# dimforge/wgsparkl

Measured on AMD Instinct MI355X. Metric: particle-steps/sec, higher is better.
Workload: dtype f32; 1 GPU; wgsparkl3d neo-Hookean elastic cube, 1000000 particles, 128^3-cell domain, h=1, dt=1/1200, 8 particles/cell, floor cuboid (CPIC passes on), free fall; config=c2, particles_per_gpu=1000000, global_particles=1000000, active_blocks_rank0=2700, parallelism=1 GPU

## Files before the change

wgsparkl_amd/csrc/capi_debug.inc:

```

extern "C" {

wgs_status wgs_enqueue_diagnostics(wgs_data *d, uint32_t what, wgs_diagnostics *device_out) {
    WGS_TRY(enter(d, device_out != nullptr));
    return diag_enqueue(d, what, device_out);
}

wgs_status wgs_read_diagnostics(wgs_data *d, uint32_t what, wgs_diagnostics *out) {
    WGS_TRY(enter(d, out != nullptr));
    if (!d->diag_out) WGS_TRY(dev_alloc(d, &d->diag_out, 1));
    if (!d->diag_host) WGS_TRY(d->diag_host.alloc(1));
    WGS_TRY(diag_enqueue(d, what, d->diag_out));
    WGS_TRY(download(d, d->diag_host.get(), d->diag_out, sizeof(wgs_diagnostics)));
    memcpy(out, d->diag_host.get(), sizeof(wgs_diagnostics));
    return WGS_OK;
}

wgs_status wgs_debug_scan(wgs_pipeline *pipeline, const uint32_t *values, uint32_t n, uint32_t *out, uint32_t *total) {
    if (!pipeline || (!values && n) || (!out && n)) return fail(WGS_ERR_INVALID_ARGUMENT, "NULL argument");
    if (n > (1u << 25)) return fail(WGS_ERR_INVALID_ARGUMENT, "n out of range");
    HIP_TRY(hipSetDevice(pipeline->device));
    Dev dev{};
    dev.cap = std::max(1u, n);
    const uint32_t nscan = (dev.cap + SCAN_CHUNK - 1) / SCAN_CHUNK, epoch = 1u;
    Scratch<uint32_t> counters, stamp, acc, active, start;
    Scratch<unsigned long long> chunk_a, chunk_b, group_a, group_b;
    const size_t ngroup = (size_t)nscan * SORT_THREADS;
    if (counters.alloc(CTR_COUNT, true) != WGS_OK || stamp.alloc(dev.cap, true) != WGS_OK || acc.alloc(dev.cap, true) != WGS_OK ||
        active.alloc(dev.cap, true) != WGS_OK || start.alloc(dev.cap, true) != WGS_OK || chunk_a.alloc(nscan, true) != WGS_OK ||
        chunk_b.alloc(nscan, true) != WGS_OK || group_a.alloc(ngroup, true) != WGS_OK || group_b.alloc(ngroup, true) != WGS_OK)
        return fail(WGS_ERR_HIP, "out of device memory");
    dev.counters = counters.ptr; dev.block_stamp = stamp.ptr; dev.block_acc = acc.ptr; dev.active = active.ptr; dev.block_start = start.ptr;
    dev.chunk_a = chunk_a.ptr; dev.chunk_b = chunk_b.ptr; dev.group_a = group_a.ptr; dev.group_b = group_b.ptr;
    std::vector<uint32_t> ones(dev.cap, epoch);
    uint32_t ctr[CTR_COUNT] = {0};
    ctr[CTR_NPHYS] = n;
    hipError_t e = hipMemcpy(dev.counters, ctr, sizeof(ctr), hipMemcpyHostToDevice);
    if (e == hipSuccess) e = hipMemcpy(dev.block_stamp, ones.data(), sizeof(uint32_t) * dev.cap, hipMemcpyHostToDevice);
    if (e == hipSuccess && n) e = hipMemcpy(dev.block_acc, values, sizeof(uint32_t) * n, hipMemcpyHostToDevice);
    if (e == hipSuccess) {
        hipLaunchKernelGGL(k_scan_only, dim3(nscan + std::min((n + 3u) / 4u + 1u, 2048u)), dim3(SORT_THREADS), 0, 0, dev, epoch, nscan);
        e = hipDeviceSynchronize();
    }
    if (e == hipSuccess && n) e = hipMemcpy(out, dev.block_start, sizeof(uint32_t) * n, hipMemcpyDeviceToHost);
    if (e == hipSuccess && total) {
        unsigned long long t = 0;
        std::vector<unsigned long long> ct(nscan);
        e = hipMemcpy(ct.data(), dev.chunk_b, sizeof(unsigned long long) * nscan, hipMemcpyDeviceToHost);
        for (auto v : ct) t += v & 0xffffffffull;
        *total = (uint32_t)t;
    }
    if (e != hipSuccess) return fail(WGS_ERR_HIP, hipGetErrorString(e));
    return WGS_OK;
}

#ifdef WGS_ABLATE
static wgs_status read_and_reset_prof(const void *symbol, unsigned long long *out, size_t rows) {
    const std::vector<unsigned long long> zero(rows * 8, 0ull);
    HIP_TRY(hipDeviceSynchronize());
    HIP_TRY(hipMemcpyFromSymbol(out, symbol, sizeof(unsigned long long) * zero.size()));
    HIP_TRY(hipMemcpyToSymbol(symbol, zero.data(), sizeof(unsigned long long) * zero.size()));
    return WGS_OK;
}
wgs_status wgs_debug_g2p_prof(unsigned long long *out) { return read_and_reset_prof(HIP_SYMBOL(g_g2p_prof), out, WGS_G2P_ROWS); }
wgs_status wgs_debug_p2g_prof(unsigned long long *out) { return read_and_reset_prof(HIP_SYMBOL(g_p2g_prof), out, WGS_P2G_ROWS); }
wgs_status wgs_debug_prof(unsigned long long *out) { return read_and_reset_prof(HIP_SYMBOL(g_prof), out, WGS_PROF_ROWS); }
#endif

}
```

wgsparkl_amd/csrc/host_grid.inc:

```

namespace {

wgs_status alloc_grid(wgs_data *d, bool missing_only = false) {
    Dev &dev = d->dev;
    const size_t hcap = (size_t)dev.hmask + 1, cap = dev.cap, nchunk = (cap + SCAN_CHUNK - 1) / SCAN_CHUNK;
    auto grid_array = [&](auto **ptr, size_t count) {
        return missing_only && *ptr ? WGS_OK : dev_alloc(d, ptr, count, MemGroup::grid);
    };
    WGS_TRY(grid_array(&dev.hkeys, hcap));
    WGS_TRY(grid_array(&dev.hvals, hcap));
    WGS_TRY(grid_array(&dev.block_key, cap));
    if (!(dev.dbg & DBG_NO_EVICTION)) {
        WGS_TRY(grid_array(&dev.block_slot, cap));
        WGS_TRY(grid_array(&dev.free_ids, cap));
    }
    WGS_TRY(grid_array(&dev.block_count, cap));
    WGS_TRY(grid_array(&dev.block_stamp, cap));
    WGS_TRY(grid_array(&dev.links_epoch, cap));
    WGS_TRY(grid_array(&dev.block_acc, cap));
    WGS_TRY(grid_array(&dev.block_dirty, cap));
    WGS_TRY(grid_array(&dev.blk_narr, cap));
    WGS_TRY(grid_array(&dev.block_ident, cap));
    WGS_TRY(grid_array(&dev.blk_arr, cap * BLK_ARR));
    WGS_TRY(grid_array(&dev.active, cap));
    WGS_TRY(grid_array(&dev.block_start, cap));
    WGS_TRY(grid_array(&dev.act_info, cap));
    WGS_TRY(grid_array(&dev.act_cells, cap * NPB));
    WGS_TRY(grid_array(&dev.nbr_plus, cap * 8));
    WGS_TRY(grid_array(&dev.nbr_minus, cap * 8));
    WGS_TRY(grid_array(&dev.nbr_known, cap * 16));
    WGS_TRY(grid_array(&dev.act_src, cap * 8));
    WGS_TRY(grid_array(&dev.cell_head, cap * NPB));
    WGS_TRY(grid_array(&dev.chunk_a, nchunk));
    WGS_TRY(grid_array(&dev.chunk_b, nchunk));
    WGS_TRY(grid_array(&dev.group_a, nchunk * SORT_THREADS));
    WGS_TRY(grid_array(&dev.group_b, nchunk * SORT_THREADS));
    WGS_TRY(grid_array(&dev.cell_start, cap * NPB));
    WGS_TRY(grid_array(&dev.cell_cursor, cap * NPB));
    WGS_TRY(grid_array(&dev.nodes, cap * NPB));
    WGS_TRY(grid_array(&dev.node_cdf, cap * NPB));
    WGS_TRY(grid_array(&dev.slab, cap * Dim<D>::TILE));
    WGS_TRY(grid_array(&dev.slab_epoch, cap));
    WGS_TRY(grid_array(&dev.block_cdf_gen, cap));
    WGS_TRY(grid_array(&dev.block_cpic, cap));
    WGS_TRY(grid_array(&dev.block_cdf_summ, cap));
    WGS_TRY(grid_array(&dev.pcdf_done, cap));
    WGS_TRY(grid_array(&dev.cpic_list, cap * 8));
    dev.visit_cap = dev.npad / 512u + 2u * dev.cap + 16u;
    WGS_TRY(grid_array(&dev.visit_list, (size_t)dev.visit_cap * 8));
    if (dev.sharded) WGS_TRY(grid_array(&dev.halo_list, cap * HALO_ENT));
    if (d->two_way) WGS_TRY(grid_array(&dev.imp_slab, cap * Dim<D>::TILE * (D == 3 ? 2 : 1)));
    if (d->mesh_cdf) {
        WGS_TRY(grid_array(&dev.mesh_min, cap * NPB));
        WGS_TRY(grid_array(&dev.mesh_aff, cap * NPB));
    }
    return WGS_OK;
}

wgs_status enable_impulses(wgs_data *d) {
    if (d->two_way) return WGS_OK;
    d->two_way = true;
    const wgs_status st = alloc_grid(d, true);
    if (st != WGS_OK) d->two_way = false;
    return st;
}

wgs_status clear_table(wgs_data *d, bool ids_too) {
    const Dev &dev = d->dev;
    HIP_TRY(hipMemsetAsync(dev.hkeys, 0xff, sizeof(uint32_t) * ((size_t)dev.hmask + 1), d->stream));
    HIP_TRY(hipMemsetAsync(dev.hvals, 0xff, sizeof(uint32_t) * ((size_t)dev.hmask + 1), d->stream));
    if (!ids_too) return WGS_OK;
    HIP_TRY(hipMemsetAsync(dev.counters + CTR_NPHYS, 0, sizeof(uint32_t), d->stream));
    HIP_TRY(hipMemsetAsync(dev.counters + CTR_NFREE, 0, 3 * sizeof(uint32_t), d->stream));
    return WGS_OK;
}

wgs_status grow_grid(wgs_data *d, uint32_t new_cap) {
    Dev &dev = d->dev;
    HIP_TRY(hipStreamSynchronize(d->stream));
    const Dev old = dev;
    d->mem.regroup(MemGroup::grid, MemGroup::old_grid);
    dev.cap = new_cap;
    dev.hmask = new_cap * 2u - 1u;
    if (alloc_grid(d) != WGS_OK) {
        d->mem.release_group(MemGroup::grid);
        d->mem.regroup(MemGroup::old_grid, MemGroup::grid);
        dev = old;
        d->auto_grow = false;
        hipGetLastError();
        return WGS_OK;
    }
    d->mem.release_group(MemGroup::old_grid);
    WGS_TRY(clear_table(d, true));
    d->sub.prev_sorted = false;
    d->sub.prebinned = false;
    d->cdf_generation++;
    d->seen.ncpic = UINT32_MAX;
    d->seen.nvisit = UINT32_MAX;
    d->stats.grid_grown++;
    return WGS_OK;
}

wgs_status maintain_grid(wgs_data *d) {
    if (!d->seen.watch || !d->seen.watch_pending) return WGS_OK;
    if (hipEventQuery(d->seen.watch_event) != hipSuccess) {
        if (++d->seen.watch_skips < 2u) return WGS_OK;
        HIP_TRY(hipEventSynchronize(d->seen.watch_event));
    }
    d->seen.watch_skips = 0;
    d->seen.watch_pending = false;
    const uint32_t nblocks = d->seen.watch[CTR_NBLOCKS], nphys = d->seen.watch[CTR_NPHYS], cap = d->dev.cap;
    if (d->dev.sharded) d->seen.nv_hint = std::max(d->seen.watch[CTR_NV], d->seen.watch[CTR_NV + CTR_SET]);
    const uint32_t rate = nblocks > d->seen.nblocks && d->seen.nblocks != 0u ? nblocks - d->seen.nblocks : 0u;
    d->seen.nblocks = std::min(nblocks, cap);
    const uint64_t ahead = (uint64_t)nblocks + 3ull * rate;
    if (d->auto_grow && (nblocks > cap / 2u || ahead > cap / 4u * 3u) && cap < (1u << 24)) {
        uint32_t new_cap = cap * 2u;
        while (ahead > new_cap / 4u * 3u && new_cap < (1u << 24)) new_cap *= 2u;
        return grow_grid(d, new_cap);
    }
    if (nphys > cap / 4u * 3u) d->seen.force_rehash = true;
    if (d->seen.watch[CTR_NTOMB] > cap / 2u) d->seen.force_refresh = true;
    return WGS_OK;
}

wgs_status watch_counters(wgs_data *d) {
    if (!d->seen.watch) {
        Pinned<uint32_t> watch;
        Event copied;
        WGS_TRY(watch.alloc(CTR_COUNT));
        WGS_TRY(copied.create(hipEventDisableTiming));
        d->seen.watch = std::move(watch);
        d->seen.watch_event = std::move(copied);
    }
    HIP_TRY(hipMemcpyAsync(d->seen.watch.get(), d->dev.counters, sizeof(uint32_t) * CTR_COUNT, hipMemcpyDeviceToHost, d->stream));
    HIP_TRY(hipEventRecord(d->seen.watch_event, d->stream));
    d->seen.watch_pending = true;
    return WGS_OK;
}

wgs_status fetch_counters(wgs_data *d) {
    uint32_t host[CTR_COUNT];
    HIP_TRY(hipMemcpyAsync(host, d->dev.counters, sizeof(host), hipMemcpyDeviceToHost, d->stream));
    HIP_TRY(hipStreamSynchronize(d->stream));
    d->seen.sync_nblocks = host[CTR_NBLOCKS] < d->dev.cap ? host[CTR_NBLOCKS] : d->dev.cap;
    d->seen.nblocks = d->seen.sync_nblocks;
    const uint32_t last_epoch = (uint32_t)d->substeps;
    d->seen.ncpic = 0;
    for (uint32_t k = 0; k < 8; k++) d->seen.ncpic += std::min(host[ctr_ncpic(k, last_epoch)], d->dev.cap);
    d->seen.ncpic = std::min(d->seen.ncpic, d->dev.cap);
    d->seen.nvisit = 0;
    for (uint32_t k = 0; k < 8; k++) d->seen.nvisit = std::max(d->seen.nvisit, std::min(host[ctr_nvisit(k, last_epoch)], d->dev.visit_cap));
    uint32_t movers = 0u;
    for (int k = 0; k < 16; k++) movers += host[CTR_MOVERS + 32 * k];
    d->stats.movers_total += (uint32_t)(movers - d->seen.movers);
    d->seen.movers = movers;
    d->seen.nphys = host[CTR_NPHYS];
    d->seen.nfree = host[CTR_NFREE];
    d->seen.ntomb = host[CTR_NTOMB];
    d->seen.errors |= host[CTR_ERRORS];
    if (host[CTR_NBLOCKS] > d->dev.cap) d->seen.errors |= ERRBIT_OVERFLOW;
    if (host[CTR_NPHYS] > d->dev.cap / 4u * 3u) d->seen.force_rehash = true;
    if (host[CTR_NTOMB] > d->dev.cap / 2u) d->seen.force_refresh = true;
    return WGS_OK;
}

wgs_status sticky_status(wgs_data *d) {
    if (d->seen.errors & ERRBIT_OVERFLOW)
        return fail(WGS_ERR_GRID_OVERFLOW, "sparse grid overflow: more active blocks than grid_capacity");
    if (d->seen.errors & ERRBIT_SHARD)
        return fail(WGS_ERR_INVALID_ARGUMENT, "sharded run: a message buffer or the particle capacity overflowed, a particle left the decomposition, or the ranks disagree on the uniform-material mode");
    if (d->seen.errors & ERRBIT_KEYRANGE)
        return fail(WGS_ERR_KEY_RANGE, "a particle left the packed block-key range (grid.wgsl:88-95)");
    if (d->seen.errors & ERRBIT_HANDOVER)
        return fail(WGS_ERR_HIP, "internal: a grid-update wave gave up waiting for a block's P2G slab (the sort's block totals and cell runs disagree)");
    if (d->seen.errors & ERRBIT_PCDF)
        return fail(WGS_ERR_HIP, "internal: a near-collider workgroup of P2G gave up waiting for the prologue waves of its launch and computed the particle cdf itself (results intact; the launch lost 0.2 s)");
    if (d->seen.errors & ERRBIT_MATERIAL)
        return fail(WGS_ERR_INVALID_ARGUMENT, "wgs_set_uniform_material: a particle of this wgs_data carries other constants (mass, init_volume, lambda, mu)");
    return WGS_OK;
}

void resolve_timings(wgs_data *d) {
    if (!d->timing.pending) return;
    hipStreamSynchronize(d->stream);
    for (int p = 0; p < WGS_NUM_PASSES; p++) d->timing.ms[p] = 0.f;
    const int pass_of_mark[8] = {WGS_PASS_GRID_SORT,   WGS_PASS_GRID_UPDATE_CDF, WGS_PASS_G2P_CDF,          WGS_PASS_P2G,
                                 WGS_PASS_GRID_UPDATE, WGS_PASS_G2P,             WGS_PASS_PARTICLES_UPDATE, WGS_PASS_INTEGRATE_BODIES};
    d->timing.mark_overhead_ms = 0.f;
    for (int s = 0; s < d->timing.events.used; s++) {
        float ms = 0.f;
        if (hipEventElapsedTime(&ms, d->timing.events.ev[s][9], d->timing.events.ev[s][10]) == hipSuccess) d->timing.mark_overhead_ms += ms;
    }
    if (d->timing.events.used > 0) d->timing.mark_overhead_ms /= (float)d->timing.events.used;
    for (int s = 0; s < d->timing.events.used; s++)
        for (int m = 0; m < 8; m++) {
            if (m == 6 && !d->cpic) continue;
            float ms = 0.f;
            if (hipEventElapsedTime(&ms, d->timing.events.ev[s][m], d->timing.events.ev[s][m + 1]) == hipSuccess)
                d->timing.ms[pass_of_mark[m]] += ms;
        }
    d->timing.pending = false;
}

}
```

wgsparkl_amd/csrc/host_state.h:

```cpp
#pragma once

namespace {

constexpr int D = WGS_DIM;
constexpr int DD = D * D;
using P = Pl<D>;

#define WGS_STR2(x) #x
#define WGS_STR(x) WGS_STR2(x)

thread_local std::string g_last_error;

wgs_status fail(wgs_status code, const std::string &msg) {
    g_last_error = msg;
    return code;
}

#define HIP_TRY(expr)                                                                                   \
    do {                                                                                                \
        hipError_t _e = (expr);                                                                         \
        if (_e != hipSuccess)                                                                           \
            return fail(WGS_ERR_HIP, std::string(#expr) + ": " + hipGetErrorString(_e));                \
    } while (0)
#define WGS_TRY(expr)                          \
// ... 79 lines not shown
        for (int k = 0; k < count; k++) hipEventDestroy(*(&ev[0][0] + k));
        created = false;
    }
};

class DataStream {
    hipStream_t s = nullptr;
    bool owned = false;

public:
    DataStream() = default;
    DataStream(const DataStream &) = delete;
    DataStream &operator=(const DataStream &) = delete;
    ~DataStream() {
        if (s && owned) hipStreamDestroy(s);
    }
    wgs_status create() {
        if (hipStreamCreateWithFlags(&s, hipStreamNonBlocking) != hipSuccess) return fail(WGS_ERR_HIP, "hipStreamCreate failed");
        owned = true;
        return WGS_OK;
    }
    wgs_status borrow(hipStream_t callers) {
        if (s && owned) HIP_TRY(hipStreamDestroy(s));
        s = callers;
        owned = false;
        return WGS_OK;
    }
    hipStream_t exchange(hipStream_t other) { return std::exchange(s, other); }
    operator hipStream_t() const { return s; }
};

enum class MemGroup : uint8_t { fixed, grid, old_grid, rigid, models };
class DeviceMemory {
    struct Block { void *ptr; size_t bytes; MemGroup group; };
    std::vector<Block> blocks;
    uint64_t total = 0;

public:
    wgs_status alloc(void **out, size_t bytes, MemGroup group, hipStream_t zero_on, bool zero) {
        void *p = nullptr;
        HIP_TRY(hipMalloc(&p, bytes));
        blocks.push_back({p, bytes, group});
        total += bytes;
        *out = p;
        if (zero) HIP_TRY(hipMemsetAsync(p, 0, bytes, zero_on));
        return WGS_OK;
    }
    void release(void *p) {
        if (!p) return;
        for (size_t i = 0; i < blocks.size(); i++)
            if (blocks[i].ptr == p) {
                total -= blocks[i].bytes;
                blocks.erase(blocks.begin() + (long)i);
                break;
            }
        hipFree(p);
    }
    void release_group(MemGroup group) {
        for (size_t i = blocks.size(); i-- > 0;)
            if (blocks[i].group == group) release(blocks[i].ptr);
    }
    void release_all() {
        while (!blocks.empty()) release(blocks.back().ptr);
    }
    void regroup(MemGroup from, MemGroup to) {
        for (Block &b : blocks) b.group = b.group == from ? to : b.group;
    }
    uint64_t bytes() const { return total; }
};

template <typename T> struct Scratch {
    T *ptr = nullptr;
    Scratch() = default;
    Scratch(const Scratch &) = delete;
    Scratch &operator=(const Scratch &) = delete;
    ~Scratch() { hipFree(ptr); }
    wgs_status alloc(size_t count, bool zeroed = false) {
        HIP_TRY(hipMalloc((void **)&ptr, sizeof(T) * (count ? count : 1)));
        if (zeroed) HIP_TRY(hipMemset(ptr, 0, sizeof(T) * (count ? count : 1)));
        return WGS_OK;
    }
};

}

namespace { struct DiagAcc; }

struct wgs_pipeline {
    int device = 0;
    int num_cus = 256;
    hipDeviceProp_t props;
};

struct wgs_comm {
    void *comm = nullptr;
    int rank = 0, world = 1;
    int lower = -1, upper = -1;
    int device = 0;
};
struct ShardLink {
    bool attached = false;
    wgs_comm *comm = nullptr;
    bool has_lower = false, has_upper = false;
    uint32_t halo_cap = 0, mig_cap = 0;
    size_t msg_floats = 0;
    float *msg_out[2] = {nullptr, nullptr}, *msg_in[2] = {nullptr, nullptr};
};

struct wgs_data {
    wgs_pipeline *pipeline = nullptr;
    DataStream stream;
    Dev dev{};
    int side = 0;
    bool plastic = false;
    bool cpic = false;
    uint64_t substeps = 0;
    uint32_t capacity = 0;
    uint32_t *shard_counts = nullptr;
    float *static_radius = nullptr;
    float *static_dp = nullptr;
    float *static_phase = nullptr;
    uint32_t *static_flags = nullptr;
    SimParamsDev *sp = nullptr;
    ColliderDev *colliders = nullptr;
    std::vector<ColliderDev> host_colliders;
    std::vector<BodyDev> host_bodies;
    bool bodies_move = false;
    uint32_t moving_mask = 0;
    bool two_way = false;
    bool mesh_cdf = false;
    SimParamsDev host_sp{};
    bool auto_grow = true;
    uint32_t cdf_generation = 1;
    uint32_t rehash_period = REHASH_PERIOD;
    ShardLink *link = nullptr;
    int reduce_impulses = 0;
    int32_t **lockstep_imp_ptrs = nullptr;
    uint32_t lockstep_imp_n = 0;
    DiagAcc *diag_acc = nullptr;
    wgs_diagnostics *diag_out = nullptr;
    Pinned<wgs_diagnostics> diag_host;
    uint32_t *probe_mark = nullptr;
    uint32_t probe_mark_cap = 0, probe_ticket = 0;

    DeviceMemory mem;

    struct Seen {
        Pinned<uint32_t> watch;
        Event watch_event;
        bool watch_pending = false;
        uint32_t watch_skips = 0;
        uint32_t errors = 0;
        uint32_t nblocks = 0;
        uint32_t sync_nblocks = 0;
        uint32_t nv_hint = 0;
        uint32_t ncpic = UINT32_MAX;
        uint32_t nvisit = UINT32_MAX;
        uint32_t movers = 0;
        uint32_t nphys = 0, nfree = 0, ntomb = 0;
        bool force_rehash = false;
        bool force_refresh = false;
    } seen;

    struct Substep {
        bool prev_sorted = false;
        bool needs_compact = false;
        bool prebinned = false;
        bool bodies_pending = false;
        bool in_sharded_step = false;
        int ts_slot = -1;
        uint32_t epoch = 0;
        bool rehash = false;
        bool use_rebin = false;
        bool binned = false;
        bool fused_cdf = false;
        bool gu_fused = false;
        bool shard_fused = false;
        bool arrivals = false;
    } sub;

    struct Stats {
        uint64_t movers_total = 0;
        uint64_t table_rebuilds = 0;
        uint64_t table_refreshes = 0;
        uint32_t grid_grown = 0;
    } stats;

    struct Timing {
        Events events;
        float ms[WGS_NUM_PASSES] = {0};
        float mark_overhead_ms = 0.f;
        bool pending = false;
    } timing;
};

namespace {

template <typename T> wgs_status dev_alloc(wgs_data *d, T **out, size_t count, MemGroup group = MemGroup::fixed, bool zero = true) {
    return d->mem.alloc(reinterpret_cast<void **>(out), sizeof(T) * (count ? count : 1), group, d->stream, zero);
}

wgs_status download(wgs_data *d, void *dst, const void *src, size_t bytes) {
    HIP_TRY(hipMemcpyAsync(dst, src, bytes, hipMemcpyDeviceToHost, d->stream));
    HIP_TRY(hipStreamSynchronize(d->stream));
    return WGS_OK;
}

wgs_status enter(wgs_data *d, bool args_ok = true, const char *what = "NULL argument") {
    if (!d || !args_ok) return fail(WGS_ERR_INVALID_ARGUMENT, what);
    HIP_TRY(hipSetDevice(d->pipeline->device));
    return WGS_OK;
}

int grid_for(const wgs_data *d, int blocks_per_cu) { return d->pipeline->num_cus * blocks_per_cu; }

}
```

wgsparkl_amd/csrc/host_substep.inc:

```

namespace {

wgs_status allreduce_impulses(wgs_data *d);
void launch_bodies_integrate(wgs_data *d);

#ifndef WGS_PCDF_WAVES_MAX_VISITS
#define WGS_PCDF_WAVES_MAX_VISITS 256
#endif
constexpr uint32_t PCDF_WAVES_MAX_VISITS = WGS_PCDF_WAVES_MAX_VISITS;
constexpr uint32_t P2G_SMALL_BUDGET_MIN_PARTICLES = 600000;
#ifndef WGS_REGROUP_ROUNDS
#define WGS_REGROUP_ROUNDS 4u
#endif
#ifndef WGS_GU_WG_PER_CU
#define WGS_GU_WG_PER_CU 8
#endif
#ifndef WGS_PLASTIC_WPE_DENSE
#define WGS_PLASTIC_WPE_DENSE 2
#endif
#ifndef WGS_PLASTIC_WPE
#define WGS_PLASTIC_WPE G2P_WAVES_PER_EU
#endif
constexpr uint32_t P2G_PAIR_MIN_BLOCKS = 8;


struct PackWaves {
    uint32_t blocks, guests;
};
PackWaves pack_waves(const wgs_data *d) {
    return {std::max(64u, std::min(2048u, d->seen.nblocks ? d->seen.nblocks : 2048u)), std::max(1u, std::min(64u, (2u * d->link->mig_cap + 63u) / 64u))};
}

template <int DIM> void launch_regroup(const Dev &dev, hipStream_t s, dim3 g, int side, uint32_t epoch, uint32_t nscan, int have_old, bool cdf, bool summ) {
    const dim3 b(SORT_THREADS);
    if (cdf && dev.sharded && summ) hipLaunchKernelGGL((k_regroup<DIM, true, true, true>), g, b, 0, s, dev, side, epoch, nscan, have_old);
    else if (cdf && dev.sharded) hipLaunchKernelGGL((k_regroup<DIM, true, true>), g, b, 0, s, dev, side, epoch, nscan, have_old);
    else if (cdf && summ) hipLaunchKernelGGL((k_regroup<DIM, true, false, true>), g, b, 0, s, dev, side, epoch, nscan, have_old);
    else if (cdf) hipLaunchKernelGGL((k_regroup<DIM, true, false>), g, b, 0, s, dev, side, epoch, nscan, have_old);
    else if (dev.sharded) hipLaunchKernelGGL((k_regroup<DIM, false, true>), g, b, 0, s, dev, side, epoch, nscan, have_old);
    else hipLaunchKernelGGL((k_regroup<DIM, false, false>), g, b, 0, s, dev, side, epoch, nscan, have_old);
}

enum class P2gShape {
    plain,
    separate,
    cpic_first,
    pair,
};
struct P2gLaunch {
    P2gShape shape;
    bool two_way;
    bool small_budget;
    int gu;
    uint32_t wgs;
    uint32_t ride;
    uint32_t npack, npack_blk, layer_sel;
    uint32_t npro;
};

template <int DIM, bool TW, int WPE> void launch_p2g_pair(Dev &dev, hipStream_t s, int side, uint32_t epoch, const P2gLaunch &p) {
    const dim3 g(p.npro + 2u * p.wgs + p.ride), b(P2GCfg<DIM>::NW * 64);
    dev.pcdf_waves = p.npro;
    if (p.gu == 2) hipLaunchKernelGGL((k_p2g_pair<DIM, TW, WPE, 2>), g, b, 0, s, dev, side, epoch, p.wgs, p.npack, p.npack_blk, p.layer_sel, p.npro);
    else if (p.gu == 3) hipLaunchKernelGGL((k_p2g_pair<DIM, TW, WPE, 3>), g, b, 0, s, dev, side, epoch, p.wgs, p.npack, p.npack_blk, p.layer_sel, p.npro);
    else hipLaunchKernelGGL((k_p2g_pair<DIM, TW, WPE, 0>), g, b, 0, s, dev, side, epoch, p.wgs, p.npack, p.npack_blk, p.layer_sel, p.npro);
    dev.pcdf_waves = 0u;
}

template <int DIM, bool CP, bool TW, bool PC> void launch_p2g_last(Dev &dev, hipStream_t s, int side, int filter, uint32_t epoch, const P2gLaunch &p) {
    const uint32_t npro = PC ? p.npro : 0u;
    const dim3 g(npro + p.wgs + p.ride), b(P2GCfg<DIM>::NW * 64);
    dev.pcdf_waves = npro;
    if (p.gu == 2) hipLaunchKernelGGL((k_p2g<DIM, CP, TW, PC, 2>), g, b, 0, s, dev, side, filter, epoch, p.wgs, p.npack, p.npack_blk, p.layer_sel, npro);
    else if (p.gu == 3) hipLaunchKernelGGL((k_p2g<DIM, CP, TW, PC, 3>), g, b, 0, s, dev, side, filter, epoch, p.wgs, p.npack, p.npack_blk, p.layer_sel, npro);
    else hipLaunchKernelGGL((k_p2g<DIM, CP, TW, PC, 0>), g, b, 0, s, dev, side, filter, epoch, p.wgs, p.npack, p.npack_blk, p.layer_sel, npro);
    dev.pcdf_waves = 0u;
}

template <int DIM> void launch_p2g(Dev &dev, hipStream_t s, int side, uint32_t epoch, const P2gLaunch &p) {
    const dim3 g(p.wgs), b(P2GCfg<DIM>::NW * 64);
    switch (p.shape) {
        case P2gShape::pair:
            if (p.two_way) launch_p2g_pair<DIM, true, 1>(dev, s, side, epoch, p);
            else if (p.small_budget) launch_p2g_pair<DIM, false, 3>(dev, s, side, epoch, p);
            else launch_p2g_pair<DIM, false, 1>(dev, s, side, epoch, p);
            break;
        case P2gShape::cpic_first:
            dev.pcdf_waves = p.npro;
            hipLaunchKernelGGL((k_p2g<DIM, true, true, true, 1>), dim3(p.npro + p.wgs), b, 0, s, dev, side, 2, epoch, p.wgs, 0u, 0u, p.layer_sel, p.npro);
            dev.pcdf_waves = 0u;
            hipLaunchKernelGGL((k_p2g<DIM, false, false, false, 2, true>), dim3(p.wgs + p.ride), b, 0, s, dev, side, 1, epoch, p.wgs, p.npack, p.npack_blk, p.layer_sel, 0u);
            break;
        case P2gShape::separate:
            if (p.gu != 0) hipLaunchKernelGGL((k_p2g<DIM, false, false, false, 1>), g, b, 0, s, dev, side, 1, epoch, p.wgs, 0u, 0u, p.layer_sel, 0u);
            else hipLaunchKernelGGL((k_p2g<DIM, false>), g, b, 0, s, dev, side, 1, epoch, p.wgs, 0u, 0u, p.layer_sel, 0u);
            if (p.two_way) launch_p2g_last<DIM, true, true, true>(dev, s, side, 2, epoch, p);
            else launch_p2g_last<DIM, true, false, true>(dev, s, side, 2, epoch, p);
            break;
        case P2gShape::plain:
            launch_p2g_last<DIM, false, false, false>(dev, s, side, 0, epoch, p);
            break;
    }
}

template <int DIM> void launch_grid_update(const Dev &dev, hipStream_t s, dim3 g, uint32_t epoch, bool slab, bool two_way, uint32_t iface_only) {
    if (!slab && two_way) hipLaunchKernelGGL((k_grid_update<DIM, 0, true>), g, dim3(256), 0, s, dev, epoch, 0u);
    else if (!slab) hipLaunchKernelGGL((k_grid_update<DIM, 0>), g, dim3(256), 0, s, dev, epoch, 0u);
    else if (two_way) hipLaunchKernelGGL((k_grid_update<DIM, 3, true>), g, dim3(256), 0, s, dev, epoch, iface_only);
    else hipLaunchKernelGGL((k_grid_update<DIM, 3>), g, dim3(256), 0, s, dev, epoch, iface_only);
}

enum class G2pShape {
    single,
    two_launches,
    pair,
    pair_dense,
};
struct G2pLaunch {
    G2pShape shape;
    bool shard;
    uint32_t g;
    uint32_t nlist;
};

template <int DIM, int MODEL, bool PL, int NP, class Mark>
void launch_g2p_shape(const Dev &dev, hipStream_t s, int side, uint32_t epoch, const G2pLaunch &p, const Mark &mark) {
    constexpr int WPE = PL ? WGS_PLASTIC_WPE : G2P_WAVES_PER_EU, WPE_DENSE = PL ? WGS_PLASTIC_WPE_DENSE : G2P_WAVES_PER_EU;
    constexpr bool SH = MODEL != 3;
    const dim3 g(p.g), pg(p.g + 8u * p.nlist), t(G2P_THREADS);
    switch (p.shape) {
        case G2pShape::pair_dense:
            if (p.shard) hipLaunchKernelGGL((k_g2p_pair<DIM, MODEL, PL, WPE_DENSE, NP, SH, !PL>), pg, t, 0, s, dev, side, epoch, p.g, p.nlist);
            else hipLaunchKernelGGL((k_g2p_pair<DIM, MODEL, PL, WPE_DENSE, NP, false, !PL>), pg, t, 0, s, dev, side, epoch, p.g, p.nlist);
            break;
        case G2pShape::pair:
            if (p.shard) hipLaunchKernelGGL((k_g2p_pair<DIM, MODEL, PL, WPE, NP, SH, !PL>), pg, t, 0, s, dev, side, epoch, p.g, p.nlist);
            else hipLaunchKernelGGL((k_g2p_pair<DIM, MODEL, PL, WPE, NP, false, !PL>), pg, t, 0, s, dev, side, epoch, p.g, p.nlist);
            break;
        case G2pShape::two_launches:
            hipLaunchKernelGGL((k_g2p_update<DIM, MODEL, PL, 1, NP, false, !PL>), g, t, 0, s, dev, side, epoch);
            mark(6);
            hipLaunchKernelGGL((k_g2p_update<DIM, MODEL, PL, 2, 1, false, !PL>), dim3(8u * p.nlist), t, 0, s, dev, side, epoch);
            break;
        case G2pShape::single:
            if (p.shard) hipLaunchKernelGGL((k_g2p_update<DIM, MODEL, PL, 0, NP, SH, !PL>), g, t, 0, s, dev, side, epoch);
            else hipLaunchKernelGGL((k_g2p_update<DIM, MODEL, PL, 0, NP, false, !PL>), g, t, 0, s, dev, side, epoch);
            break;
    }
}

template <int DIM, int MODEL, bool PL, class Mark>
void launch_g2p_model(const Dev &dev, hipStream_t s, int side, uint32_t epoch, const G2pLaunch &p, const Mark &mark) {
    if (dev.g2p_npass == (uint32_t)G2P_MANY_PASSES) launch_g2p_shape<DIM, MODEL, PL, G2P_MANY_PASSES>(dev, s, side, epoch, p, mark);
    else if (dev.g2p_npass == 2u) launch_g2p_shape<DIM, MODEL, PL, 2>(dev, s, side, epoch, p, mark);
    else launch_g2p_shape<DIM, MODEL, PL, 1>(dev, s, side, epoch, p, mark);
}

enum class G2pVariant { corotated, corotated_plastic, neo_hookean, neo_hookean_plastic, fluid, per_particle };
G2pVariant g2p_variant(const Dev &dev, bool plastic) {
    if (dev.pmodel[0]) return G2pVariant::per_particle;
    if (dev.model == WGS_MODEL_FLUID) return G2pVariant::fluid;
    if (dev.model == WGS_MODEL_NEO_HOOKEAN) return plastic ? G2pVariant::neo_hookean_plastic : G2pVariant::neo_hookean;
    return plastic ? G2pVariant::corotated_plastic : G2pVariant::corotated;
}

template <int DIM, class Mark> void launch_g2p(const Dev &dev, hipStream_t s, int side, uint32_t epoch, bool plastic, const G2pLaunch &p, const Mark &mark) {
    switch (g2p_variant(dev, plastic)) {
        case G2pVariant::corotated: launch_g2p_model<DIM, 0, false>(dev, s, side, epoch, p, mark); break;
        case G2pVariant::corotated_plastic: launch_g2p_model<DIM, 0, true>(dev, s, side, epoch, p, mark); break;
        case G2pVariant::neo_hookean: launch_g2p_model<DIM, 1, false>(dev, s, side, epoch, p, mark); break;
        case G2pVariant::neo_hookean_plastic: launch_g2p_model<DIM, 1, true>(dev, s, side, epoch, p, mark); break;
        case G2pVariant::fluid: launch_g2p_model<DIM, 2, false>(dev, s, side, epoch, p, mark); break;
        case G2pVariant::per_particle: launch_g2p_model<DIM, 3, false>(dev, s, side, epoch, p, mark); break;
    }
}

template <int DIM> void launch_arrivals(const Dev &dev, hipStream_t s, dim3 g, int side, uint32_t epoch, bool plastic) {
    switch (g2p_variant(dev, plastic)) {
        case G2pVariant::corotated: hipLaunchKernelGGL((k_g2p_arrivals<DIM, 0, false>), g, dim3(256), 0, s, dev, side, epoch); break;
        case G2pVariant::corotated_plastic: hipLaunchKernelGGL((k_g2p_arrivals<DIM, 0, true>), g, dim3(256), 0, s, dev, side, epoch); break;
        case G2pVariant::neo_hookean: hipLaunchKernelGGL((k_g2p_arrivals<DIM, 1, false>), g, dim3(256), 0, s, dev, side, epoch); break;
        case G2pVariant::neo_hookean_plastic: hipLaunchKernelGGL((k_g2p_arrivals<DIM, 1, true>), g, dim3(256), 0, s, dev, side, epoch); break;
        default: hipLaunchKernelGGL((k_g2p_arrivals<DIM, 2, false>), g, dim3(256), 0, s, dev, side, epoch); break;
    }
}


enum class SortBin { full, rebin, by_last_g2p };
struct SortLaunch {
    bool refresh, reset_table;
    SortBin bin;
    uint32_t do_bodies;
    uint32_t nscan, nreg;
    int have_old;
    bool cdf, summ;
    uint32_t refresh_wgs, mesh_wgs, p2g_cdf_wgs;
};
SortLaunch plan_sort(const wgs_data *d) {
    const Dev &dev = d->dev;
    SortLaunch p{};
    p.refresh = d->seen.force_refresh && !d->sub.rehash && dev.free_ids != nullptr;
    p.refresh_wgs = std::max(1u, std::min((dev.cap + 255u) / 256u, (uint32_t)grid_for(d, 4)));
    p.reset_table = d->sub.rehash;
    p.bin = d->sub.binned ? SortBin::by_last_g2p : d->sub.use_rebin ? SortBin::rebin : SortBin::full;
    p.do_bodies = d->sub.bodies_pending ? 1u : 0u;
    p.mesh_wgs = (uint32_t)grid_for(d, 1);
    p.nscan = (dev.cap + SCAN_CHUNK - 1) / SCAN_CHUNK;
    p.nreg = std::max(1u, std::min((dev.cap + 3u) / 4u, WGS_REGROUP_ROUNDS * ((uint32_t)grid_for(d, 4) - std::min(p.nscan, (uint32_t)grid_for(d, 2)))));
    p.have_old = d->sub.use_rebin ? 1 : 0;
    p.cdf = d->sub.fused_cdf;
    p.summ = (dev.cdf_moving != 0u || dev.cdf_gen == 0u) && !(dev.dbg & DBG_NO_CDF_SUMM);
    p.p2g_cdf_wgs = std::min((dev.n_rigid * 32u + 255u) / 256u, (uint32_t)grid_for(d, 32));
    return p;
}

enum class P2gLayers { all, boundary, others };

P2gLaunch plan_p2g(const wgs_data *d, P2gLayers layers) {
    const Dev &dev = d->dev;
    const uint32_t n = dev.n;
    const uint32_t NW = (uint32_t)P2GCfg<D>::NW;
    P2gLaunch p{};
    p.two_way = d->two_way;
    p.layer_sel = layers == P2gLayers::boundary ? 1u : layers == P2gLayers::others ? 2u : 0u;
    p.wgs = std::min((uint32_t)grid_for(d, 32), std::max((uint32_t)grid_for(d, 8), (d->seen.nblocks / 2u + 255u) & ~255u));
    p.gu = d->sub.gu_fused ? 2 : d->sub.shard_fused ? 3 : 0;
    const uint32_t gu_wgs = (p.gu == 0 || layers == P2gLayers::boundary) ? 0u : std::min((uint32_t)grid_for(d, 8), std::max((uint32_t)grid_for(d, 1), ((d->seen.nblocks + NW - 1u) / NW + 7u) & ~7u));
    if (d->sub.shard_fused && (d->link->has_lower || d->link->has_upper) && layers != P2gLayers::others) {
        const PackWaves pw = pack_waves(d);
        p.npack_blk = pw.blocks;
        p.npack = (pw.blocks + pw.guests + NW - 1u) / NW;
    }
    p.ride = p.npack + gu_wgs;
    if (d->cpic && !dev.sharded && d->seen.nvisit != UINT32_MAX && d->seen.nvisit != 0u && d->seen.nvisit <= PCDF_WAVES_MAX_VISITS && !(dev.dbg & DBG_NO_PCDF_WAVES))
        p.npro = 8u * ((std::min(d->seen.nvisit + 8u, dev.visit_cap) + NW - 1u) / NW);
    if (d->cpic && !dev.sharded && (dev.dbg & DBG_PCDF_WAVES_UNSIZED)) p.npro = 8u;
    if (!d->cpic) {
        p.shape = P2gShape::plain;
        return p;
    }
    p.small_budget = !d->two_way && n >= P2G_SMALL_BUDGET_MIN_PARTICLES && !(dev.dbg & DBG_NO_P2G_SMALL_BUDGET);
    const bool big_two_way = d->two_way && n >= P2G_SMALL_BUDGET_MIN_PARTICLES;
    const bool small_two_way = d->two_way && n < P2G_SMALL_BUDGET_MIN_PARTICLES;
    const bool many_listed = d->seen.ncpic != UINT32_MAX && d->seen.ncpic >= P2G_PAIR_MIN_BLOCKS;
    if (!big_two_way && (p.small_budget || small_two_way || many_listed) && !(dev.dbg & DBG_P2G_TWO_LAUNCHES))
        p.shape = P2gShape::pair;
    else if (big_two_way && p.gu == 2 && !(dev.dbg & DBG_PLAIN_P2G_FIRST))
        p.shape = P2gShape::cpic_first;
    else
        p.shape = P2gShape::separate;
    return p;
}

G2pLaunch plan_g2p(const wgs_data *d) {
    const Dev &dev = d->dev;
    const uint32_t npass = dev.g2p_npass;
    const uint32_t full = (uint32_t)grid_for(d, 1) * 3u / 2u;
    G2pLaunch p{G2pShape::single, dev.sharded != 0u, ((dev.nv + G2P_THREADS * npass - 1) / (G2P_THREADS * npass) + 7) / 8 * 8, full};
    if (d->cpic && (p.shard || !(dev.dbg & DBG_G2P_TWO_LAUNCHES))) {
        const uint32_t per_run = std::min<uint32_t>(npass, WGS_G2P_LIST_PASSES);
        if (d->seen.nvisit != UINT32_MAX) p.nlist = std::min(full, std::max(8u, 2u * ((d->seen.nvisit + per_run - 1u) / per_run)));
        const bool dense = d->plastic && d->seen.ncpic != UINT32_MAX && d->seen.ncpic * 2u >= std::max(1u, d->seen.sync_nblocks) && !(dev.dbg & DBG_NO_G2P_DENSE);
        p.shape = dense ? G2pShape::pair_dense : G2pShape::pair;
    } else if (d->cpic) {
        p.shape = G2pShape::two_launches;
    }
    return p;
}


struct Mark {
    wgs_data *d;
    void operator()(int m) const {
        static const bool trace = getenv("WGS_TRACE") != nullptr;
        if (d->sub.ts_slot >= 0) hipEventRecord(d->timing.events.ev[d->sub.ts_slot][m], d->stream);
        if (trace) {
            const hipError_t te = hipStreamSynchronize(d->stream);
            fprintf(stderr, "[wgs trace] substep %llu mark %d: %s\n", (unsigned long long)d->substeps, m, hipGetErrorString(te));
        }
    }
};

void catch_up_counters(wgs_data *d) {
    d->dev.ctr_set = (uint32_t)(d->substeps & 1u);
    if (!d->sub.needs_compact) return;
    hipLaunchKernelGGL(k_shard_compacted, dim3(1), dim3(64), 0, d->stream, d->dev);
    d->sub.needs_compact = false;
}

wgs_status begin_substep(wgs_data *d, bool in_sharded_step, int ts_slot = -1) {
    Dev &dev = d->dev;
    wgs_data::Substep &sub = d->sub;
    hipStream_t s = d->stream;
    sub.in_sharded_step = in_sharded_step;
    sub.ts_slot = ts_slot;
    sub.epoch = (uint32_t)(d->substeps + 1);
    const uint32_t nv_now = dev.sharded && d->seen.nv_hint != 0u ? std::min(d->seen.nv_hint, dev.nv) : dev.nv;
    dev.g2p_npass = (D == 3 && nv_now >= G2P_MANY_PASS_MIN_PARTICLES) ? (uint32_t)G2P_MANY_PASSES
                    : (nv_now >= G2P_TWO_PASS_MIN_PARTICLES || (dev.dbg & DBG_G2P_TWO_PASSES)) ? 2u : 1u;
    sub.rehash = d->substeps == 0 || (d->rehash_period != 0u && d->substeps % d->rehash_period == 0) || d->seen.force_rehash;
    if (sub.rehash) {
        d->stats.table_rebuilds++;
        d->seen.force_rehash = false;
        d->cdf_generation++;
    }
    dev.cdf_gen = d->cpic ? d->cdf_generation : 0u;
    dev.cdf_moving = d->moving_mask;
    sub.fused_cdf = d->cpic && dev.n_rigid == 0;
    dev.listed_in_perm = sub.fused_cdf ? 1u : 0u;
    sub.use_rebin = sub.prev_sorted && !sub.rehash && !(dev.dbg & DBG_NO_REBIN);
    sub.binned = sub.use_rebin && sub.prebinned;
    if (sub.prebinned && !sub.binned) {
        HIP_TRY(hipMemsetAsync(dev.block_acc, 0, sizeof(uint32_t) * (size_t)dev.cap, s));
        HIP_TRY(hipMemsetAsync(dev.cell_head, 0, sizeof(uint32_t) * (size_t)dev.cap * NPB, s));
        HIP_TRY(hipMemsetAsync(dev.blk_narr, 0, sizeof(uint32_t) * (size_t)dev.cap, s));
    }
    sub.prebinned = false;
    dev.bin_next = (!d->plastic && !(dev.dbg & (DBG_NO_REBIN | DBG_REBIN_LAUNCH)) && (d->rehash_period == 0u || (d->substeps + 1) % d->rehash_period != 0)) ? 1u : 0u;
    dev.skip_guests = (in_sharded_step && dev.sharded) ? 1u : 0u;
    sub.gu_fused = !in_sharded_step && !dev.sharded && !(dev.dbg & DBG_GU_OWN_LAUNCH);
    const bool attached = in_sharded_step && d->link && d->link->attached;
    sub.shard_fused = attached && dev.n > 0 && !(dev.dbg & DBG_GU_OWN_LAUNCH);
    sub.arrivals = attached;
    catch_up_counters(d);
    return WGS_OK;
}

template <int DIM> wgs_status enqueue_sort(wgs_data *d) {
    Dev &dev = d->dev;
    hipStream_t s = d->stream;
    const Mark mark{d};
    const int side = d->side;
    const uint32_t n = dev.n, epoch = d->sub.epoch;
    const int pgrid = (int)((n + SORT_THREADS - 1) / SORT_THREADS);
    const SortLaunch p = plan_sort(d);
    if (d->sub.ts_slot >= 0) {
        mark(9);
        mark(10);
    }
    mark(0);
    if (p.refresh) {
        WGS_TRY(clear_table(d, false));
        hipLaunchKernelGGL(k_table_refresh, dim3(p.refresh_wgs), dim3(256), 0, s, dev);
        d->stats.table_refreshes++;
    }
    d->seen.force_refresh = false;
    if (p.reset_table) WGS_TRY(clear_table(d, true));
    if (dev.n_rigid > 0)
        hipLaunchKernelGGL(k_rigid_transform<DIM>, dim3(p.mesh_wgs), dim3(256), 0, s, dev);
    if (n > 0) {
        d->sub.bodies_pending = false;
        switch (p.bin) {
            case SortBin::by_last_g2p: if (p.do_bodies) launch_bodies_integrate(d); break;
            case SortBin::rebin: hipLaunchKernelGGL(k_rebin<DIM>, dim3((pgrid + REBIN_K - 1) / REBIN_K), dim3(SORT_THREADS), 0, s, dev, side, epoch, p.do_bodies); break;
            case SortBin::full: hipLaunchKernelGGL(k_bin<DIM>, dim3(pgrid), dim3(SORT_THREADS), 0, s, dev, side, epoch, p.do_bodies); break;
        }
        if (dev.n_rigid > 0) {
            hipLaunchKernelGGL(k_rigid_mark<DIM>, dim3(p.mesh_wgs), dim3(256), 0, s, dev, epoch);
            hipLaunchKernelGGL(k_rigid_touch<DIM>, dim3(p.mesh_wgs), dim3(256), 0, s, dev, epoch);
        }
        launch_regroup<DIM>(dev, s, dim3(p.nscan + p.nreg), side, epoch, p.nscan, p.have_old, p.cdf, p.summ);
    } else {
        HIP_TRY(hipMemsetAsync(dev.counters + CTR_NBLOCKS, 0, sizeof(uint32_t), s));
    }
    mark(1);
    if (dev.n_rigid > 0 && n > 0)
        hipLaunchKernelGGL(k_p2g_cdf<DIM>, dim3(p.p2g_cdf_wgs), dim3(256), 0, s, dev, epoch);
    if (d->cpic && n > 0 && !p.cdf)
        hipLaunchKernelGGL(k_cdf<DIM>, dim3(grid_for(d, 16)), dim3(CDF_THREADS), 0, s, dev, side, epoch);
    mark(2);
    mark(3);
    HIP_TRY(hipGetLastError());
    return WGS_OK;
}

template <int DIM> wgs_status enqueue_p2g(wgs_data *d, P2gLayers layers) {
    if (d->dev.n > 0) launch_p2g<DIM>(d->dev, d->stream, d->side, d->sub.epoch, plan_p2g(d, layers));
    Mark{d}(4);
    HIP_TRY(hipGetLastError());
    return WGS_OK;
}

template <int DIM> wgs_status enqueue_finish(wgs_data *d) {
    Dev &dev = d->dev;
    const wgs_data::Substep &sub = d->sub;
    hipStream_t s = d->stream;
    const Mark mark{d};
    const int side = d->side;
    const uint32_t n = dev.n, epoch = sub.epoch;
    if (n > 0 && !sub.gu_fused)
        launch_grid_update<DIM>(dev, s, dim3(grid_for(d, WGS_GU_WG_PER_CU)), epoch, sub.in_sharded_step, d->two_way, sub.shard_fused ? 1u : 0u);
    mark(5);
    const G2pLaunch g2p = plan_g2p(d);
    if (dev.nv > 0) launch_g2p<DIM>(dev, s, side, epoch, d->plastic, g2p, mark);
    if (!(dev.nv > 0 && g2p.shape == G2pShape::two_launches)) mark(6);
    if (sub.arrivals) {
        const uint32_t arr_most = ((d->link->has_lower ? 1u : 0u) + (d->link->has_upper ? 1u : 0u)) * d->link->mig_cap;
        launch_arrivals<DIM>(dev, s, dim3(std::max(1u, std::min((arr_most + ARR_PER_WG - 1u) / ARR_PER_WG, 1024u))), side, epoch, d->plastic);
    }
    mark(7);
    if (d->bodies_move && dev.n_colliders > 0 && !(sub.in_sharded_step && d->reduce_impulses == 2)) {
        if (sub.in_sharded_step && d->reduce_impulses == 1) WGS_TRY(allreduce_impulses(d));
        if (!sub.in_sharded_step && !dev.sharded && dev.n_rigid == 0 && n > 0 && !(dev.dbg & DBG_BODIES_OWN_LAUNCH) && !dev.bin_next) d->sub.bodies_pending = true;
        else launch_bodies_integrate(d);
    }
    mark(8);
    d->side ^= 1;
    d->substeps++;
    d->sub.prev_sorted = true;
    d->sub.prebinned = dev.bin_next != 0u && dev.nv > 0;
    dev.n = dev.nv;
    if (dev.sharded && !sub.arrivals) d->sub.needs_compact = true;
    HIP_TRY(hipGetLastError());
    return WGS_OK;
}

void launch_bodies_integrate(wgs_data *d) { hipLaunchKernelGGL(k_bodies_integrate<D>, dim3(1), dim3(16), 0, d->stream, d->dev); }

wgs_status enqueue_bodies(wgs_data *d) {
    if (d->bodies_move && d->dev.n_colliders > 0) launch_bodies_integrate(d);
    HIP_TRY(hipGetLastError());
    return WGS_OK;
}

}
```

wgsparkl_amd/csrc/kernels_sort.h:

```cpp
#pragma once
#include "kernels_shard.h"

namespace wgs {

constexpr int SORT_THREADS = 256;
constexpr int TOUCH_SET = 32;

template <int D> __device__ inline void load_cell(const Dev &d, const float *in, uint32_t i, int *cell) {
    const float4 xm = ldq(in, d.npad, Pl<D>::XM, i);
    const bool p2 = d.h_pow2 != 0u;
    cell[0] = assoc_cell(xm.x, d.h, d.inv_h, p2);
    cell[1] = assoc_cell(xm.y, d.h, d.inv_h, p2);
    if constexpr (D == 3) cell[2] = assoc_cell(xm.z, d.h, d.inv_h, p2);
}

__device__ inline void push_mover(const Dev &d, uint32_t cid, uint32_t i) { d.mv_next[i] = atomicExch(&d.cell_head[cid], i + 1u); }
__device__ inline void push_arrival(const Dev &d, uint32_t cid, uint32_t i) {
    const uint32_t pos = atomicAdd(&d.blk_narr[cid >> 6], 1u);
    if (pos < BLK_ARR) d.blk_arr[(size_t)(cid >> 6) * BLK_ARR + pos] = i;
    else push_mover(d, cid, i);
}

__device__ inline void count_blocks(const Dev &d, int lane, uint32_t myid) {
    unsigned long long todo = __ballot(myid != NONE);
// ... 71 lines not shown
        const int slot = tid >> 3, o = tid & 7;
        const uint32_t k0 = s_keys[slot];
        if (k0 != NONE && o < NN) {
            int lb[3] = {0, 0, 0};
            unpack_key<D>(k0, lb);
            int nb[3] = {lb[0] + (o & 1), lb[1] + ((o >> 1) & 1), lb[2] + ((o >> 2) & 1)};
            const uint32_t id = activate_block(d, pack_key<D>(nb), epoch);
            if (o == 0) s_ids[slot] = id;
        }
    }
    __syncthreads();
    uint32_t myid = !valid ? NONE : (myslot != NONE ? s_ids[myslot] : mydirect);
    if (myid >= d.cap) myid = NONE;
    count_blocks(d, lane, myid);
    if (i < slots_end) {
        const uint32_t cid = myid == NONE ? NONE : myid * NPB + local;
        d.cellid[i] = cid;
        if (cid != NONE) push_mover(d, cid, i);
    }
}
template <int D> __global__ __launch_bounds__(SORT_THREADS) void k_bin(Dev d, int side, uint32_t epoch, uint32_t do_bodies) {
    if (do_bodies && blockIdx.x == 0 && threadIdx.x < 16) bodies_integrate_one<D>(d, threadIdx.x);
    bin_body<D>(d, side, epoch, blockIdx.x);
}

#ifndef WGS_REBIN_K
#define WGS_REBIN_K 2
#endif
constexpr int REBIN_K = WGS_REBIN_K;
template <int D> __device__ __forceinline__ void rebin_body(const Dev &d, int side, uint32_t epoch, uint32_t bid) {
    constexpr int BS = Dim<D>::BSHIFT, BW = Dim<D>::BW, NN = Dim<D>::NNBR, K = REBIN_K;
    const float *in = d.buf[side];
    const int tid = threadIdx.x, lane = tid & 63;
    const uint32_t nslots = num_slots(d);
    const uint32_t nprev = d.sharded ? ctr_cur(d, CTR_NPREV) : 0u;
    uint32_t idx[K], old[K];
    bool in_range[K], valid[K];
    float4 xm[K];
#pragma unroll
    for (int k = 0; k < K; k++) {
        idx[k] = (bid * (uint32_t)K + (uint32_t)k) * SORT_THREADS + (uint32_t)tid;
        in_range[k] = idx[k] < nslots;
        valid[k] = in_range[k];
        old[k] = NONE;
        xm[k] = make_float4(0.f, 0.f, 0.f, 0.f);
        if (in_range[k]) {
            if (!d.sharded || idx[k] < nprev) old[k] = d.perm_cell[idx[k]];
            xm[k] = ldq(in, d.npad, Pl<D>::XM, idx[k]);
            if (d.sharded) valid[k] = ldpid<D>(in, d.npad, idx[k]) != 0xffffffffu;
        }
    }
    uint32_t okey[K];
#pragma unroll
    for (int k = 0; k < K; k++) {
        if (old[k] != NONE) old[k] &= ~CELL_LISTED;
        okey[k] = (valid[k] && old[k] != NONE) ? d.block_key[old[k] >> 6] : 0u;
    }
    const bool p2 = d.h_pow2 != 0u;
    uint32_t last_b1 = NONE;
#pragma unroll
    for (int k = 0; k < K; k++) {
        uint32_t myid = NONE, local = 0u, mykey = 0u;
        if (valid[k]) {
            const uint32_t ob = old[k] >> 6;
            int c[3] = {assoc_cell(xm[k].x, d.h, d.inv_h, p2), assoc_cell(xm[k].y, d.h, d.inv_h, p2), D == 3 ? assoc_cell(xm[k].z, d.h, d.inv_h, p2) : 0};
            int nb[3] = {0, 0, 0};
            uint32_t shift = 0;
#pragma unroll
            for (int a = 0; a < D; a++) {
                nb[a] = c[a] >> BS;
                local |= (uint32_t)(c[a] & (BW - 1)) << shift;
                shift += BS;
            }
            int hi[3] = {nb[0] + 1, nb[1] + 1, nb[2] + 1};
            if (!block_in_key_range<D>(nb) || !block_in_key_range<D>(hi)) {
                atomicOr(&d.counters[CTR_ERRORS], ERRBIT_KEYRANGE);
            } else {
                const uint32_t key = pack_key<D>(nb);
                mykey = key;
                myid = (old[k] != NONE && key == okey[k]) ? ob : activate_block(d, key, epoch);
                if (myid >= d.cap) myid = NONE;
            }
        }
        unsigned long long todo = __ballot(myid != NONE);
        while (todo) {
            const int leader = __ffsll((long long)todo) - 1;
            const uint32_t b1 = __shfl(myid, leader);
            const uint32_t k1 = __shfl(mykey, leader);
            const unsigned long long same = __ballot(myid == b1);
            todo &= ~same;
            if (lane == leader) atomicAdd(&d.block_acc[b1], (uint32_t)__popcll(same));
            if (b1 == last_b1) continue;
            last_b1 = b1;
            if (lane < NN) {
                const uint32_t le = d.links_epoch[b1], link = d.nbr_plus[b1 * 8u + lane];
                const uint32_t t1 = le == epoch - 1u ? link : NONE;
                if (t1 != NONE) {
                    d.block_stamp[t1] = epoch;
                } else {
                    int kb[3] = {0, 0, 0};
                    unpack_key<D>(k1, kb);
                    int nb[3] = {kb[0] + (lane & 1), kb[1] + ((lane >> 1) & 1), kb[2] + ((lane >> 2) & 1)};
                    if (block_in_key_range<D>(nb)) activate_block(d, pack_key<D>(nb), epoch);
                }
            }
        }
        if (in_range[k]) {
            const uint32_t cid = myid == NONE ? NONE : myid * NPB + local;
            d.cellid[idx[k]] = (cid != NONE && old[k] != NONE && cid != old[k]) ? (cid | CELL_MOVED) : cid;
            if (old[k] != NONE && cid != old[k]) d.block_dirty[old[k] >> 6] = epoch;
            if (cid != NONE && (old[k] == NONE || (cid >> 6) != (old[k] >> 6))) push_arrival(d, cid, idx[k]);
        }
    }
}
template <int D> __global__ __launch_bounds__(SORT_THREADS) void k_rebin(Dev d, int side, uint32_t epoch, uint32_t do_bodies) {
    if (do_bodies && blockIdx.x == 0 && threadIdx.x < 16) bodies_integrate_one<D>(d, threadIdx.x);
    rebin_body<D>(d, side, epoch, blockIdx.x);
}
#ifdef WGS_ABLATE
constexpr int WGS_PROF_ROWS = 8192;
__device__ unsigned long long g_prof[WGS_PROF_ROWS][8];
#define WGS_PROF_START() if (lane == 0 && id < WGS_PROF_ROWS - 1) g_prof[id][0] = wall_clock64();
#define WGS_PROF(k) if (lane == 0 && id < WGS_PROF_ROWS - 1) g_prof[id][1 + (k)] = wall_clock64();
#define WGS_PROF_END()
#else
#define WGS_PROF_START()
#define WGS_PROF(k)
#define WGS_PROF_END()
#endif
constexpr int SCAN_ITEMS = 16;
constexpr int SCAN_CHUNK = SORT_THREADS * SCAN_ITEMS;
constexpr int RUNCAP = 768;

__device__ inline uint32_t wait_tagged(const unsigned long long *word, uint32_t epoch) {
    unsigned long long v = __hip_atomic_load(word, __ATOMIC_RELAXED, __HIP_MEMORY_SCOPE_AGENT);
    while ((uint32_t)(v >> 32) != epoch) {
        __builtin_amdgcn_s_sleep(8);
        v = __hip_atomic_load(word, __ATOMIC_RELAXED, __HIP_MEMORY_SCOPE_AGENT);
    }
    return (uint32_t)v;
}
__device__ inline void publish_tagged(unsigned long long *word, uint32_t epoch, uint32_t value) {
    __hip_atomic_store(word, ((unsigned long long)epoch << 32) | value, __ATOMIC_RELAXED, __HIP_MEMORY_SCOPE_AGENT);
}

template <bool SHARD = false>
__device__ __forceinline__ void scan_chunk(const Dev &d, uint32_t epoch, uint32_t k, uint32_t nchunks, unsigned long long *s_wave, unsigned long long *s_bcast) {
    const uint32_t nphys = min(d.counters[CTR_NPHYS], d.cap);
    const int tid = threadIdx.x, lane = tid & 63, wave = tid >> 6;
#ifdef WGS_ABLATE
    if (tid == 0 && k == 0) g_prof[WGS_PROF_ROWS - 1][1] = wall_clock64();
#endif
    unsigned long long sum = 0ull;
    const uint32_t first = k * SCAN_CHUNK + (uint32_t)tid * SCAN_ITEMS;
    uint32_t stamp[SCAN_ITEMS], acc[SCAN_ITEMS];
#pragma unroll
    for (int j = 0; j < SCAN_ITEMS; j++) {
        const uint32_t idc = min(first + j, nphys ? nphys - 1u : 0u);
        stamp[j] = d.block_stamp[idc];
        acc[j] = d.block_acc[idc];
    }
#pragma unroll
    for (int j = 0; j < SCAN_ITEMS; j++) {
        const bool act = first + j < nphys && stamp[j] == epoch;
        sum += act ? ((1ull << 32) | (unsigned long long)acc[j]) : 0ull;
    }
    const unsigned long long inc = ((unsigned long long)wave_scan_incl_u32((uint32_t)(sum >> 32)) << 32) | (unsigned long long)wave_scan_incl_u32((uint32_t)sum);
    if (lane == 63) s_wave[wave] = inc;
    __syncthreads();
    unsigned long long wave_off = 0ull, total = 0ull;
#pragma unroll
    for (int w = 0; w < SORT_THREADS / 64; w++) {
        const unsigned long long t = s_wave[w];
        if (w < wave) wave_off += t;
        total += t;
    }
#ifdef WGS_ABLATE
    if (tid == 0 && k == 0) g_prof[WGS_PROF_ROWS - 1][2] = wall_clock64();
#endif
    if (tid == 0) {
        publish_tagged(&d.chunk_a[k], epoch, (uint32_t)(total >> 32));
        publish_tagged(&d.chunk_b[k], epoch, (uint32_t)total);
    }
    unsigned long long part = 0ull;
    for (uint32_t p = (uint32_t)tid; p < k; p += SORT_THREADS)
        part += ((unsigned long long)wait_tagged(&d.chunk_a[p], epoch) << 32) + wait_tagged(&d.chunk_b[p], epoch);
    part = ((unsigned long long)wave_sum_u32((uint32_t)(part >> 32)) << 32) + (unsigned long long)wave_sum_u32((uint32_t)part);
    __syncthreads();
    if (lane == 0) s_wave[wave] = part;
    __syncthreads();
    if (tid == 0) {
        unsigned long long b = 0ull;
        for (int w = 0; w < SORT_THREADS / 64; w++) b += s_wave[w];
        *s_bcast = b;
    }
    __syncthreads();
    const unsigned long long base = *s_bcast;
    const unsigned long long run = base + wave_off + inc - sum;
    publish_tagged(&d.group_a[k * SORT_THREADS + tid], epoch, (uint32_t)(run >> 32));
    publish_tagged(&d.group_b[k * SORT_THREADS + tid], epoch, (uint32_t)run);
    if (tid == 0 && k + 1 == nchunks) {
        d.counters[CTR_NBLOCKS] = (uint32_t)((base + total) >> 32);
        d.counters[CTR_NSORTED] = (uint32_t)(base + total);
    }
#ifdef WGS_ABLATE
    if (tid == 0) g_prof[WGS_PROF_ROWS - 1][0] = wall_clock64();
#endif
    if (k == 0 && tid == 0) d.counters[CTR_NPHYS_SEEN + (epoch & 1u)] = d.counters[CTR_NINSERT];
    if (k == 0 && tid < 16) d.counters[tid < 8 ? ctr_ncpic((uint32_t)tid, epoch + 1u) : ctr_nvisit((uint32_t)tid - 8u, epoch + 1u)] = 0u;
    if (k == 0 && tid == 16) d.counters[ctr_nhalo(epoch + 1u)] = 0u;
    if constexpr (SHARD) {
        if (k == 0 && tid < 4 && d.msg.out[tid >> 1]) reinterpret_cast<uint32_t *>(d.msg.out[tid >> 1])[tid & 1] = 0u;
    }
}

struct GroupLoads {
    uint32_t stamp, acc;
};
__device__ inline GroupLoads block_prefix_loads(const Dev &d, uint32_t id, int lane) {
    GroupLoads g = {0u, 0u};
    if (lane < SCAN_ITEMS) {
        const uint32_t j = min((id & ~(uint32_t)(SCAN_ITEMS - 1)) + (uint32_t)lane, d.cap - 1u);
        g.stamp = d.block_stamp[j];
        g.acc = d.block_acc[j];
    }
    return g;
}
__device__ inline void block_prefix(const Dev &d, uint32_t epoch, uint32_t id, int lane, const GroupLoads &g, uint32_t nphys, uint32_t &start, uint32_t &aidx) {
    const uint32_t gbase = id & ~(uint32_t)(SCAN_ITEMS - 1), j = id & (uint32_t)(SCAN_ITEMS - 1);
    const bool before = lane < (int)j && gbase + (uint32_t)lane < nphys && g.stamp == epoch;
    const uint32_t cnt = (uint32_t)__popcll(__ballot(before));
    uint32_t psum = before ? g.acc : 0u;
    psum = wave_sum_u32(psum);
    const uint32_t grp = id / SCAN_ITEMS;
    aidx = wait_tagged(&d.group_a[grp], epoch) + cnt;
    start = wait_tagged(&d.group_b[grp], epoch) + psum;
}

constexpr uint32_t OUT_CELL_SHIFT = 26, OUT_SRC_MASK = 0x03ffffffu;

constexpr int ARRC = 4;
constexpr int PAR_R = (RUNCAP + 63) / 64;
struct WaveStage {
    uint32_t *s_in;
    uint32_t *s_out;
    uint32_t *s_pid;
    __device__ uint32_t *cnt_stay() const { return s_out + RUNCAP - 64; }
    __device__ uint32_t *cnt_new() const { return s_out + RUNCAP - 128; }
    __device__ uint32_t *place_stay() const { return s_in; }
    __device__ uint32_t *arr_slot() const { return s_in + 64; }
    __device__ uint32_t *place_new() const { return s_in + 128; }
    __device__ uint32_t *hand_cnt() const { return s_out; }
    __device__ uint32_t *hand_slot() const { return s_out + 64; }
    __device__ uint32_t *hand_pid() const { return s_out + 64 + 64 * ARRC; }
};
static_assert(PAR_R % 2 == 0 && RUNCAP <= 1023, "two 16-bit (cell | place << 6) per register; 0xffff = none");
static_assert(RUNCAP >= 64 + 2 * 64 * ARRC, "the hand-over arrays alias the output stage");

template <int D, bool CDF, bool SHARD, bool SUMM>
__device__ __forceinline__ uint32_t regroup_block(const Dev &d, int side, uint32_t epoch_of_launch, uint32_t id, uint32_t nphys, bool have_old, bool no_new_blocks, bool check_keys,
                                              uint32_t *s_in, uint32_t *s_out, uint32_t *s_pid, ColliderDev *cols, bool &cols_staged) {
    constexpr int NN = Dim<D>::NNBR;
    int lane = threadIdx.x & 63;
    asm volatile("" : "+v"(lane));
    uint32_t epoch = epoch_of_launch;
    if constexpr (SUMM) asm volatile("" : "+s"(epoch));
    const float *in = d.buf[side];
    const WaveStage st = {s_in, s_out, s_pid};
    const uint32_t lane_p = (uint32_t)lane;
    const uint32_t idx = id * NPB + lane_p;
    WGS_PROF_START()
    const uint32_t stamp = d.block_stamp[id];
    const uint32_t le = d.links_epoch[id];
    uint32_t cs_old = d.cell_start[idx], ce_old = d.cell_cursor[idx];
    const uint32_t head = d.cell_head[idx];
    const uint32_t bkey = d.block_key[id];
    const uint32_t dirty_at = d.block_dirty[id];
    const uint32_t bstart_old = d.block_start[id], ident = d.block_ident[id];
    const uint32_t narr = d.blk_narr[id];
    uint32_t a_ent = NONE;
    uint32_t cdf_seen = 0u, cdf_class = 0u, cdf_summ = 0u;
    if constexpr (CDF) {
        cdf_seen = d.block_cdf_gen[id];
        cdf_class = d.block_cpic[id];
        if constexpr (SUMM) cdf_summ = d.block_cdf_summ[id];
    }
    uint32_t link = NONE;
    if (lane < 16) link = d.nbr_known[id * 16u + lane_p];
    const GroupLoads grp = block_prefix_loads(d, id, lane);
    if (stamp != epoch) {
        {
            if (d.free_ids != nullptr && lane == 0 && (epoch & (EVICT_AGE - 1u)) == 0u && stamp != 0u && epoch - stamp > EVICT_AGE && bkey != NONE &&
                d.counters[CTR_NTOMB] <= d.cap / 2u) {
                const uint32_t hs = d.block_slot[id];
                d.hkeys[hs] = KEY_TOMB;
                d.hvals[hs] = NONE;
                d.block_key[id] = NONE;
                if constexpr (CDF) d.block_cdf_gen[id] = 0u;
                d.free_ids[atomicAdd(&d.counters[CTR_NFREE], 1u)] = id;
                atomicAdd(&d.counters[CTR_NTOMB], 1u);
            }
        }
        return 0u;
    }
    const bool old_ok = have_old && le == epoch - 1u;
    if (!old_ok) {
        cs_old = ce_old = 0u;
        link = NONE;
    }
    uint32_t link_stamp = 0u, link_cnt = 0u, link_key = NONE;
    if (link != NONE) {
        link_stamp = d.block_stamp[link];
        link_cnt = d.block_acc[link];
        if (check_keys) link_key = d.block_key[link];
    }
    const bool links_valid = old_ok;
    const uint32_t run0 = lane_value(cs_old, 0), run1 = lane_value(ce_old, 63);
    const uint32_t runlen = run1 - run0;
    const bool in_lds = runlen <= (uint32_t)RUNCAP;
    const uint32_t narr_in = min(narr, BLK_ARR);
    const bool any_arr = __ballot(head != 0u) != 0ull || narr != 0u;
    uint32_t a_cell = NONE, a_epid = 0u;
    if ((uint32_t)lane < narr_in) {
        a_ent = d.blk_arr[(size_t)id * BLK_ARR + (uint32_t)lane];
        a_cell = cell_of(d.cellid[a_ent]);
        a_epid = ldpid<D>(in, d.npad, a_ent);
        if ((a_cell >> 6) != id) a_cell = NONE;
    } else {
        a_ent = NONE;
    }
    const bool clean = dirty_at != epoch;
    const bool need_ids = !clean || any_arr;
    uint32_t n_moved = 0u;
    const bool par = old_ok && need_ids && in_lds && __ballot(head != 0u) == 0ull && runlen + narr_in <= (uint32_t)RUNCAP;
    if (in_lds && need_ids) {
        const bool want_cells = !clean || par;
#pragma unroll
        for (int half = 0; half < 2; half++) {
            if (half == 1 && runlen <= 64u * (uint32_t)(PAR_R / 2)) break;
            uint32_t ce[PAR_R / 2], pe[PAR_R / 2];
#pragma unroll
            for (int r = 0; r < PAR_R / 2; r++) {
                const uint32_t t = (uint32_t)lane + 64u * (uint32_t)(half * (PAR_R / 2) + r);
                ce[r] = NONE;
                pe[r] = 0u;
                if (t < runlen) {
                    if (want_cells) ce[r] = d.cellid[run0 + t];
                    pe[r] = ldpid<D>(in, d.npad, run0 + t);
                }
            }
#pragma unroll
            for (int r = 0; r < PAR_R / 2; r++) {
                const uint32_t t = (uint32_t)lane + 64u * (uint32_t)(half * (PAR_R / 2) + r);
                if (t < runlen) {
                    if (want_cells) {
                        s_in[t] = ce[r];
                        n_moved += (ce[r] != NONE && (ce[r] & CELL_MOVED) != 0u && (cell_of(ce[r]) >> 6) == id) ? 1u : 0u;
                    }
                    s_pid[t] = pe[r];
                }
            }
        }
    }
    uint32_t res = NONE;
    int b[3] = {0, 0, 0};
    unpack_key<D>(bkey, b);
    if (lane < 16) {
        const uint32_t o = lane & 7u;
        const bool minus = lane >= 8;
        uint32_t known = NONE;
        if ((int)o < NN) {
            const int sgn = minus ? -1 : 1;
            int nb[3] = {b[0] + sgn * (int)(o & 1u), b[1] + sgn * (int)((o >> 1) & 1u), b[2] + sgn * (int)((o >> 2) & 1u)};
            if (check_keys && link != NONE && link_key != pack_key<D>(nb)) link = NONE;
            if (link != NONE) {
                known = link;
                res = link_stamp == epoch ? link : NONE;
            } else if (!(links_valid && no_new_blocks)) {
                if (block_in_key_range<D>(nb)) known = hmap_lookup(d, pack_key<D>(nb));
                if (known != NONE && d.block_stamp[known] == epoch) res = known;
                if (res != NONE) link_cnt = d.block_acc[res];
            }
        }
        if (res == NONE) link_cnt = 0u;
        (minus ? d.nbr_minus : d.nbr_plus)[id * 8u + o] = res;
        d.nbr_known[id * 16u + lane] = known;
    }
    WGS_PROF(0)
    auto new_cell_of = [&](uint32_t i) {
// ... 110 lines not shown
                uint32_t parts = 1u;
                uint32_t mine = 0u;
#pragma unroll 1
                for (int it = 0; it <= ROUNDS; it++) {
                    if (it == 1) {
                        uint32_t bits = 0u;
                        const int t0[3] = {lane & (BW - 1), (lane >> BS) & (BW - 1), D == 3 ? (lane >> (2 * BS)) : 0};
#pragma unroll
                        for (int o = 0; o < NN; o++) {
                            bool in = mine != 0u;
#pragma unroll
                            for (int k = 0; k < D; k++)
                                if ((o >> k) & 1) in = in && t0[k] < TW - BW;
                            bits |= __ballot(in) != 0ull ? (1u << o) : 0u;
                        }
                        publish_summ(bits);
                        any = (bits & 1u) != 0u;
                        parts = 0u;
                        if (!any && bcount > 0u) {
                            const uint32_t nb = lane >= 1 && lane < NN ? res : NONE;
                            const unsigned long long t_start = wall_clock64();
                            for (;;) {
                                uint32_t w = 0u;
                                if (nb != NONE) w = __hip_atomic_load(&d.block_cdf_summ[nb], __ATOMIC_RELAXED, __HIP_MEMORY_SCOPE_AGENT);
                                const bool have = nb != NONE && (w >> 8) == (epoch & SUMM_TAG);
                                any = __ballot(have && ((w >> lane) & 1u) != 0u) != 0ull;
                                parts = (uint32_t)__ballot(nb != NONE && !have);
                                if (any || parts == 0u || (d.dbg & DBG_CDF_SUMM_NO_WAIT) || wall_clock64() - t_start > 400ull) break;
                                __builtin_amdgcn_s_sleep(8);
                            }
                            if (any) parts = 0u;
                        }
                        if (parts == 0u) break;
                        mine = 0u;
                    }
                    int t[3], o = 0;
                    bool active = true;
                    if (it == 0) {
                        t[0] = lane & (BW - 1); t[1] = (lane >> BS) & (BW - 1); t[2] = D == 3 ? (lane >> (2 * BS)) : 0;
                    } else {
                        const int n = lane + 64 * (it - 1);
                        t[0] = n % TW; t[1] = (n / TW) % TW; t[2] = D == 3 ? n / (TW * TW) : 0;
                        o = (t[0] >= BW ? 1 : 0) | (t[1] >= BW ? 2 : 0) | (t[2] >= BW ? 4 : 0);
                        active = n < TILE && ((parts >> o) & 1u) != 0u;
                    }
                    if (active) {
                        float pt[D];
#pragma unroll
                        for (int k = 0; k < D; k++) pt[k] = (float)(b[k] * BW + t[k]) * d.h;
                        const NodeCdf c = node_cdf_eval<D>(cols, d.n_colliders, d.h, pt, near);
                        if (it == 0) d.node_cdf[(size_t)id * NPB + (uint32_t)lane] = c;
                        mine |= c.affinities;
                    }
                }
                if (parts != 0u) any = __ballot(mine != 0u) != 0ull;
            }
        }
        if (lane == 0) {
            d.block_cpic[id] = any ? 1u : 0u;
            if (d.cdf_gen != 0u) d.block_cdf_gen[id] = (near & d.cdf_moving) == 0u ? (d.cdf_gen | (bcount > 0u ? CDF_FULL : 0u)) : 0u;
            if (any && bcount > 0u) d.cpic_list[(size_t)(id & 7u) * d.cap + atomicAdd(&d.counters[ctr_ncpic(id & 7u, epoch)], 1u)] = id;
        }
        listed = any && bcount > 0u;
        pc_flag = any ? CELL_LISTED : 0u;
    }
    WGS_PROF(3)
    uint32_t a_slot[ARRC], a_pid[ARRC];
#pragma unroll
    for (int k = 0; k < ARRC; k++) { a_slot[k] = NONE; a_pid[k] = NONE; }
    uint32_t n_stay = ce_old - cs_old, n_arr = 0, n_in = 0;
    uint32_t ckp[PAR_R / 2];
    uint32_t a_ck = NONE;
    uint32_t *s_cnt = st.cnt_stay(), *s_cnt2 = st.cnt_new();
    uint32_t par_new = 0u;
    uint32_t par_nst = 0u;
    if (par) {
        __hip_atomic_store(&s_cnt[lane], 0u, __ATOMIC_RELAXED, __HIP_MEMORY_SCOPE_WAVEFRONT);
        __hip_atomic_store(&s_cnt2[lane], 0u, __ATOMIC_RELAXED, __HIP_MEMORY_SCOPE_WAVEFRONT);
#pragma unroll
        for (int r = 0; r < PAR_R; r++) {
            const uint32_t t = (uint32_t)lane + 64u * (uint32_t)r;
            uint32_t ck = 0xffffu;
            if (t < runlen) {
                const uint32_t e = __hip_atomic_load(&s_in[t], __ATOMIC_RELAXED, __HIP_MEMORY_SCOPE_WAVEFRONT);
                const uint32_t c = cell_of(e);
                if ((c >> 6) == id) {
                    const bool came = (e & CELL_MOVED) != 0u;
                    ck = (c & 63u) | (__hip_atomic_fetch_add(came ? &s_cnt2[c & 63u] : &s_cnt[c & 63u], 1u, __ATOMIC_RELAXED, __HIP_MEMORY_SCOPE_WAVEFRONT) << 6);
                    par_new |= came ? (1u << r) : 0u;
                }
            }
            if (r & 1) ckp[r / 2] |= ck << 16;
            else ckp[r / 2] = ck;
        }
        if (a_cell != NONE) a_ck = (a_cell & 63u) | (__hip_atomic_fetch_add(&s_cnt2[a_cell & 63u], 1u, __ATOMIC_RELAXED, __HIP_MEMORY_SCOPE_WAVEFRONT) << 6);
        par_nst = __hip_atomic_load(&s_cnt[lane], __ATOMIC_RELAXED, __HIP_MEMORY_SCOPE_WAVEFRONT);
        n_stay = par_nst + __hip_atomic_load(&s_cnt2[lane], __ATOMIC_RELAXED, __HIP_MEMORY_SCOPE_WAVEFRONT);
        n_arr = 0;
    } else {
        uint32_t *s_acnt = st.hand_cnt(), *s_aslot = st.hand_slot(), *s_apid = st.hand_pid();
        auto hand_over = [&](uint32_t c, uint32_t slot, uint32_t pid) {
            const uint32_t k = __hip_atomic_fetch_add(&s_acnt[c & 63u], 1u, __ATOMIC_RELAXED, __HIP_MEMORY_SCOPE_WAVEFRONT);
            if (k < (uint32_t)ARRC) {
                __hip_atomic_store(&s_aslot[(c & 63u) * ARRC + k], slot, __ATOMIC_RELAXED, __HIP_MEMORY_SCOPE_WAVEFRONT);
                __hip_atomic_store(&s_apid[(c & 63u) * ARRC + k], pid, __ATOMIC_RELAXED, __HIP_MEMORY_SCOPE_WAVEFRONT);
            }
        };
        if (!clean || narr_in != 0u) {
            __hip_atomic_store(&s_acnt[lane], 0u, __ATOMIC_RELAXED, __HIP_MEMORY_SCOPE_WAVEFRONT);
            if (!clean) {
                n_stay = 0;
                for (uint32_t i = cs_old; i < ce_old; i++) {
                    const uint32_t c = new_cell_of(i);
                    if (c == idx) n_stay++;
                    else if ((c >> 6) == id) hand_over(c, i, pid_of_old(i));
                }
            }
            if (a_cell != NONE) hand_over(a_cell, a_ent, a_epid);
            n_in = __hip_atomic_load(&s_acnt[lane], __ATOMIC_RELAXED, __HIP_MEMORY_SCOPE_WAVEFRONT);
#pragma unroll
            for (int k = 0; k < ARRC; k++)
                if ((uint32_t)k < n_in) {
                    a_slot[k] = __hip_atomic_load(&s_aslot[lane * ARRC + k], __ATOMIC_RELAXED, __HIP_MEMORY_SCOPE_WAVEFRONT);
                    a_pid[k] = __hip_atomic_load(&s_apid[lane * ARRC + k], __ATOMIC_RELAXED, __HIP_MEMORY_SCOPE_WAVEFRONT);
                }
            n_arr = n_in;
        }
        for (uint32_t a = head; a != 0u;) {
            const uint32_t nxt = d.mv_next[a - 1u], p = ldpid<D>(in, d.npad, a - 1u);
#pragma unroll
            for (int k = 0; k < ARRC; k++)
                if (n_arr == (uint32_t)k) { a_slot[k] = a - 1u; a_pid[k] = p; }
            n_arr++;
            a = nxt;
        }
    }
    if (n_arr > 1u && n_arr <= (uint32_t)ARRC) {
#pragma unroll
        for (int pass = 0; pass < ARRC; pass++)
#pragma unroll
            for (int k = pass & 1; k + 1 < ARRC; k += 2)
                if (a_pid[k] > a_pid[k + 1]) {
                    const uint32_t tp = a_pid[k], ts = a_slot[k];
                    a_pid[k] = a_pid[k + 1]; a_slot[k] = a_slot[k + 1];
                    a_pid[k + 1] = tp; a_slot[k + 1] = ts;
                }
    }
    const uint32_t total = n_stay + n_arr;
    const uint32_t inc = wave_scan_incl_u32(total);
    const uint32_t btotal = lane_value(inc, 63);
    const uint32_t lstart = inc - total;
    WGS_PROF(2)
    const bool out_lds = btotal <= (uint32_t)RUNCAP;
    uint32_t bstart = 0, aidx = 0;
    auto fetch_bstart = [&]() { block_prefix(d, epoch, id, lane, grp, nphys, bstart, aidx); };
    if (!out_lds) fetch_bstart();
    const bool fast_clean = old_ok && clean && !any_arr;
    bool keep_perm = false;
    if (fast_clean) {
        if (out_lds) fetch_bstart();
        keep_perm = bstart == bstart_old && ident == (((epoch - 1u) << 1) | (pc_flag != 0u ? 1u : 0u));
    }
    uint32_t *s_lst = st.place_stay(), *s_av = st.arr_slot(), *s_new = st.place_new();
    if (par) {
        __hip_atomic_store(&s_lst[lane], lstart, __ATOMIC_RELAXED, __HIP_MEMORY_SCOPE_WAVEFRONT);
        __hip_atomic_store(&s_new[lane], lstart + par_nst, __ATOMIC_RELAXED, __HIP_MEMORY_SCOPE_WAVEFRONT);
        if (a_ck != NONE) {
            __hip_atomic_store(&s_av[lane], a_ent, __ATOMIC_RELAXED, __HIP_MEMORY_SCOPE_WAVEFRONT);
            __hip_atomic_store(&s_pid[runlen + (uint32_t)lane], a_epid, __ATOMIC_RELAXED, __HIP_MEMORY_SCOPE_WAVEFRONT);
        }
#pragma unroll
        for (int r = 0; r < PAR_R; r++) {
            const uint32_t ck = (ckp[r / 2] >> (16 * (r & 1))) & 0xffffu;
            if (ck != 0xffffu) {
                const uint32_t pos = __hip_atomic_load(((par_new >> r) & 1u) ? &s_new[ck & 63u] : &s_lst[ck & 63u], __ATOMIC_RELAXED, __HIP_MEMORY_SCOPE_WAVEFRONT) + (ck >> 6);
                __hip_atomic_store(&s_out[pos], ((ck & 63u) << OUT_CELL_SHIFT) | ((uint32_t)lane + 64u * (uint32_t)r), __ATOMIC_RELAXED, __HIP_MEMORY_SCOPE_WAVEFRONT);
            }
        }
        if (a_ck != NONE) {
            const uint32_t pos = __hip_atomic_load(&s_new[a_ck & 63u], __ATOMIC_RELAXED, __HIP_MEMORY_SCOPE_WAVEFRONT) + (a_ck >> 6);
            __hip_atomic_store(&s_out[pos], ((a_ck & 63u) << OUT_CELL_SHIFT) | (runlen + (uint32_t)lane), __ATOMIC_RELAXED, __HIP_MEMORY_SCOPE_WAVEFRONT);
        }
        constexpr int NEWC = 4;
        auto lds = [&](const uint32_t *ptr) { return *ptr; };
        bool ordered = true;
        {
            uint32_t pk = 0u, pv = 0u;
#pragma unroll 4
            for (uint32_t m = 0; m < par_nst; m++) {
                const uint32_t v = lds(&s_out[lstart + m]) & OUT_SRC_MASK, k = lds(&s_pid[v]);
                ordered = ordered && (m == 0u || pk < k || (pk == k && pv < v));
                pk = k;
                pv = v;
            }
        }
        const bool quick = ordered && !(d.dbg & DBG_CELL_INSERTION_SORT);
        for (uint32_t base = par_nst; quick && base < total; base += (uint32_t)NEWC) {
            const uint32_t par_nst = base, n_new = min((uint32_t)NEWC, total - base);
            uint32_t nk[NEWC], nv[NEWC], rk[NEWC];
#pragma unroll
            for (int k = 0; k < NEWC; k++) {
                nk[k] = nv[k] = NONE;
                if ((uint32_t)k < n_new) {
                    nv[k] = lds(&s_out[lstart + par_nst + (uint32_t)k]) & OUT_SRC_MASK;
                    nk[k] = lds(&s_pid[nv[k]]);
                }
            }
#pragma unroll
            for (int pass = 0; pass < NEWC; pass++)
#pragma unroll
                for (int k = pass & 1; k + 1 < NEWC; k += 2)
                    if (nk[k] > nk[k + 1] || (nk[k] == nk[k + 1] && nv[k] > nv[k + 1])) {
                        const uint32_t tk = nk[k], tv = nv[k];
                        nk[k] = nk[k + 1]; nv[k] = nv[k + 1];
                        nk[k + 1] = tk; nv[k + 1] = tv;
                    }
            uint32_t lo[NEWC], hi[NEWC];
#pragma unroll
            for (int k = 0; k < NEWC; k++) { lo[k] = 0u; hi[k] = (uint32_t)k < n_new ? par_nst : 0u; }
            for (;;) {
                bool more = false;
                uint32_t mid[NEWC], mv[NEWC], mk[NEWC];
#pragma unroll
                for (int k = 0; k < NEWC; k++) {
                    mid[k] = (lo[k] + hi[k]) >> 1;
                    mv[k] = lo[k] < hi[k] ? (lds(&s_out[lstart + mid[k]]) & OUT_SRC_MASK) : 0u;
                }
#pragma unroll
                for (int k = 0; k < NEWC; k++) mk[k] = lo[k] < hi[k] ? lds(&s_pid[mv[k]]) : 0u;
#pragma unroll
                for (int k = 0; k < NEWC; k++)
                    if (lo[k] < hi[k]) {
                        if (mk[k] < nk[k] || (mk[k] == nk[k] && mv[k] < nv[k])) lo[k] = mid[k] + 1u;
                        else hi[k] = mid[k];
                        more = more || lo[k] < hi[k];
                    }
                if (!more) break;
            }
#pragma unroll
            for (int k = 0; k < NEWC; k++) rk[k] = lo[k];
            for (uint32_t t = par_nst; t > rk[0]; t--) {
                const uint32_t at = t - 1u;
                uint32_t up = 0u;
#pragma unroll
                for (int k = 0; k < NEWC; k++) up += ((uint32_t)k < n_new && rk[k] <= at) ? 1u : 0u;
                s_out[lstart + at + up] = lds(&s_out[lstart + at]);
            }
#pragma unroll
            for (int k = 0; k < NEWC; k++)
                if ((uint32_t)k < n_new)
                    s_out[lstart + rk[k] + (uint32_t)k] = ((uint32_t)lane << OUT_CELL_SHIFT) | nv[k];
        }
        uint32_t kprev = 0u, vprev = 0u;
        if (!quick && total > 1u) {
            vprev = __hip_atomic_load(&s_out[lstart], __ATOMIC_RELAXED, __HIP_MEMORY_SCOPE_WAVEFRONT) & OUT_SRC_MASK;
            kprev = __hip_atomic_load(&s_pid[vprev], __ATOMIC_RELAXED, __HIP_MEMORY_SCOPE_WAVEFRONT);
        }
        for (uint32_t m = 1; m < (quick ? 0u : total); m++) {
            const uint32_t e = __hip_atomic_load(&s_out[lstart + m], __ATOMIC_RELAXED, __HIP_MEMORY_SCOPE_WAVEFRONT);
            const uint32_t ve = e & OUT_SRC_MASK, ke = __hip_atomic_load(&s_pid[ve], __ATOMIC_RELAXED, __HIP_MEMORY_SCOPE_WAVEFRONT);
            if (kprev < ke || (kprev == ke && vprev < ve)) {
                kprev = ke;
                vprev = ve;
                continue;
            }
            uint32_t j = m;
            while (j > 0u) {
                const uint32_t q = __hip_atomic_load(&s_out[lstart + j - 1u], __ATOMIC_RELAXED, __HIP_MEMORY_SCOPE_WAVEFRONT);
                const uint32_t vq = q & OUT_SRC_MASK, kq = __hip_atomic_load(&s_pid[vq], __ATOMIC_RELAXED, __HIP_MEMORY_SCOPE_WAVEFRONT);
                if (kq < ke || (kq == ke && vq < ve)) break;
                __hip_atomic_store(&s_out[lstart + j], q, __ATOMIC_RELAXED, __HIP_MEMORY_SCOPE_WAVEFRONT);
                j--;
            }
            if (j != m) __hip_atomic_store(&s_out[lstart + j], e, __ATOMIC_RELAXED, __HIP_MEMORY_SCOPE_WAVEFRONT);
        }
    }
    uint32_t out = lstart;
    auto emit = [&](uint32_t src) {
        if (out_lds) {
            __hip_atomic_store(&s_out[out], ((uint32_t)lane << OUT_CELL_SHIFT) | src, __ATOMIC_RELAXED, __HIP_MEMORY_SCOPE_WAVEFRONT);
        } else {
            d.perm[bstart + out] = src;
            d.perm_cell[bstart + out] = idx | pc_flag;
        }
        out++;
    };
    uint32_t arr_slot = NONE, arr_pid = 0, arr_k = 0;
    bool have_last = false;
    uint32_t last_pid = 0, last_slot = 0;
    const bool cached = n_arr <= (uint32_t)ARRC;
    const bool coop_ok = in_lds && out_lds;
    const bool coop_me = !par && !cached && coop_ok && total <= 64u;
    auto next_arrival = [&]() {
        arr_slot = NONE;
        if (cached) {
#pragma unroll
            for (int k = 0; k < ARRC; k++)
                if (arr_k == (uint32_t)k && (uint32_t)k < n_arr) { arr_slot = a_slot[k]; arr_pid = a_pid[k]; }
            arr_k++;
            return;
        }
        unsigned long long best = ~0ull;
        const unsigned long long last_key = ((unsigned long long)last_pid << 32) | last_slot;
        for (uint32_t a = head; a != 0u; a = d.mv_next[a - 1u]) {
            const unsigned long long key = ((unsigned long long)ldpid<D>(in, d.npad, a - 1u) << 32) | (a - 1u);
            if (have_last && key <= last_key) continue;
            if (key < best) best = key;
        }
        if (n_in != 0u) {
            if (!clean)
                for (uint32_t i = run0; i < run1; i++) {
                    if ((i >= cs_old && i < ce_old) || new_cell_of(i) != idx) continue;
                    const unsigned long long key = ((unsigned long long)pid_of_old(i) << 32) | i;
                    if (have_last && key <= last_key) continue;
                    if (key < best) best = key;
                }
            for (uint32_t t = 0; t < narr_in; t++) {
                const uint32_t sl = d.blk_arr[(size_t)id * BLK_ARR + t];
                if (cell_of(d.cellid[sl]) != idx) continue;
                const unsigned long long key = ((unsigned long long)ldpid<D>(in, d.npad, sl) << 32) | sl;
                if (have_last && key <= last_key) continue;
                if (key < best) best = key;
            }
        }
        if (best != ~0ull) {
            arr_slot = (uint32_t)best;
            arr_pid = (uint32_t)(best >> 32);
        }
    };
    if (n_arr && !coop_me) next_arrival();
    for (uint32_t i = cs_old; i < ((coop_me || par || keep_perm) ? cs_old : ce_old); i++) {
        if (!stays_here(i)) continue;
        if (arr_slot != NONE) {
            const uint32_t ps = pid_of_old(i);
            while (arr_slot != NONE && arr_pid < ps) {
                emit(arr_slot);
                have_last = true;
                last_pid = arr_pid;
                last_slot = arr_slot;
                next_arrival();
            }
        }
        emit(i);
    }
    while (arr_slot != NONE) {
        emit(arr_slot);
        have_last = true;
        last_pid = arr_pid;
        last_slot = arr_slot;
        next_arrival();
    }
    for (unsigned long long slow = __ballot(coop_me); slow != 0ull; slow &= slow - 1ull) {
        const int c = __ffsll((long long)slow) - 1;
        const uint32_t c_idx = id * NPB + (uint32_t)c;
        const uint32_t c_cs = __shfl(cs_old, c), c_ce = __shfl(ce_old, c), c_head = __shfl(head, c), c_lstart = __shfl(lstart, c), c_total = __shfl(total, c);
        uint32_t cnt = 0u;
        for (uint32_t t0 = 0; t0 < runlen; t0 += 64u) {
            const uint32_t t = t0 + (uint32_t)lane, i = run0 + t;
            const bool m = t < runlen && (clean ? (i >= c_cs && i < c_ce) : new_cell_of(i) == c_idx);
            const unsigned long long mm = __ballot(m);
            if (m) {
                const uint32_t at = c_lstart + cnt + (uint32_t)__popcll(mm & ((1ull << lane) - 1ull));
                if (at < c_lstart + c_total) __hip_atomic_store(&s_out[at], i, __ATOMIC_RELAXED, __HIP_MEMORY_SCOPE_WAVEFRONT);
            }
            cnt += (uint32_t)__popcll(mm);
        }
        {
            const bool m = a_cell == c_idx;
            const unsigned long long mm = __ballot(m);
            if (m) {
                const uint32_t at = c_lstart + cnt + (uint32_t)__popcll(mm & ((1ull << lane) - 1ull));
                if (at < c_lstart + c_total) __hip_atomic_store(&s_out[at], a_ent, __ATOMIC_RELAXED, __HIP_MEMORY_SCOPE_WAVEFRONT);
            }
            cnt += (uint32_t)__popcll(mm);
        }
        if (lane == 0)
            for (uint32_t a = c_head; a != 0u && cnt < c_total; a = d.mv_next[a - 1u]) {
                __hip_atomic_store(&s_out[c_lstart + cnt], a - 1u, __ATOMIC_RELAXED, __HIP_MEMORY_SCOPE_WAVEFRONT);
                cnt++;
            }
        unsigned long long key = ~0ull;
        if ((uint32_t)lane < c_total) {
            const uint32_t sl = __hip_atomic_load(&s_out[c_lstart + (uint32_t)lane], __ATOMIC_RELAXED, __HIP_MEMORY_SCOPE_WAVEFRONT);
            const uint32_t pd = (sl >= run0 && sl < run1) ? pid_of_old(sl) : ldpid<D>(in, d.npad, sl);
            key = ((unsigned long long)pd << 32) | sl;
        }
        uint32_t rank = 0u;
        for (uint32_t m = 0; m < c_total; m++) rank += __shfl(key, (int)m) < key ? 1u : 0u;
        if ((uint32_t)lane < c_total)
            __hip_atomic_store(&s_out[c_lstart + rank], ((uint32_t)c << OUT_CELL_SHIFT) | (uint32_t)key, __ATOMIC_RELAXED, __HIP_MEMORY_SCOPE_WAVEFRONT);
    }
    WGS_PROF(4)
    if (out_lds && !fast_clean) fetch_bstart();
    WGS_PROF(5)
    if (out_lds && !keep_perm)
        for (uint32_t t = lane; t < btotal; t += 64) {
            const uint32_t v = __hip_atomic_load(&s_out[t], __ATOMIC_RELAXED, __HIP_MEMORY_SCOPE_WAVEFRONT);
            uint32_t src = v & OUT_SRC_MASK;
            if (par) src = src < runlen ? run0 + src : __hip_atomic_load(&s_av[src - runlen], __ATOMIC_RELAXED, __HIP_MEMORY_SCOPE_WAVEFRONT);
            d.perm[bstart + t] = src;
            d.perm_cell[bstart + t] = (id * NPB + (v >> OUT_CELL_SHIFT)) | pc_flag;
        }
    d.cell_start[idx] = bstart + lstart;
    d.cell_cursor[idx] = bstart + lstart + total;
    const bool direct = fast_clean && !(d.dbg & DBG_NO_DIRECT_RUNS);
    d.act_cells[(size_t)aidx * NPB + lane] = direct ? make_uint2(cs_old, ce_old) : make_uint2(bstart + lstart, bstart + lstart + total);
    if (head != 0u) d.cell_head[idx] = 0u;
    if (lane == 0 && narr != 0u) d.blk_narr[id] = 0u;
    if (d.n_rigid != 0u) {
        d.mesh_min[idx] = ~0ull;
        d.mesh_aff[idx] = 0u;
    }
    if (lane >= 8 && lane < 16) d.act_src[aidx * 8u + (uint32_t)(lane & 7)] = link_cnt > 0u ? res : NONE;
    if (lane == 63) {
        d.active[aidx] = id;
        d.act_info[aidx] = make_uint4(id, bkey, btotal, pc_flag | (direct ? CELL_DIRECT : 0u));
        d.block_start[id] = bstart;
        d.block_count[id] = btotal;
        d.links_epoch[id] = epoch;
        d.block_ident[id] = (fast_clean && bstart == bstart_old) ? ((epoch << 1) | (pc_flag != 0u ? 1u : 0u)) : 0u;
    }
    if (listed) {
        append_visits(d, id, bstart, btotal, lane, epoch);
        if (lane == 0) d.pcdf_done[id] = 0u;
    }
    if constexpr (SHARD) {
        const IfaceMasks im = iface_masks<D>(d, b[0]);
        if ((im.send_lo | im.send_hi) != 0u) {
            uint32_t e = 0u;
            if (lane == 0) e = atomicAdd(&d.counters[ctr_nhalo(epoch)], 1u);
            e = __shfl(e, 0);
            if (e < d.cap) {
                uint32_t *ent = d.halo_list + (size_t)e * HALO_ENT;
                if (lane == 0) { ent[0] = id; ent[1] = bkey; }
                if (lane >= 8 && lane < 16) ent[2 + (lane & 7)] = link_cnt > 0u ? res : NONE;
            }
        }
    }
    WGS_PROF(6)
    WGS_PROF_END()
    uint32_t movers = 0u;
    if (have_old) {
        if (par) {
            movers = wave_sum_u32(n_moved) + narr_in;
        } else {
            movers = wave_sum_u32(n_arr);
        }
    }
    return movers;
}

#ifndef WGS_REGROUP_WPE
#define WGS_REGROUP_WPE 4
#endif
template <int D, bool CDF, bool SHARD = false, bool SUMM = false> __global__ __launch_bounds__(SORT_THREADS, WGS_REGROUP_WPE) void k_regroup(Dev d, int side, uint32_t epoch, uint32_t nscan, int have_old) {
    __shared__ unsigned long long s_wave[SORT_THREADS / 64];
    __shared__ unsigned long long s_bcast;
    __shared__ uint32_t s_in[SORT_THREADS / 64][RUNCAP], s_out[SORT_THREADS / 64][RUNCAP], s_pid[SORT_THREADS / 64][RUNCAP];
    if (blockIdx.x < nscan) {
        __builtin_amdgcn_s_setprio(3);
        scan_chunk<SHARD>(d, epoch, blockIdx.x, nscan, s_wave, &s_bcast);
        return;
    }
    __shared__ ColliderDev s_cols[SUMM ? 16 : 1];
    bool cols_staged = false;
    const uint32_t nphys = min(d.counters[CTR_NPHYS], d.cap);
    const uint32_t wave = ((blockIdx.x - nscan) * SORT_THREADS + threadIdx.x) >> 6;
    const uint32_t nwaves = ((gridDim.x - nscan) * SORT_THREADS) >> 6;
    const int w = SUMM ? __builtin_amdgcn_readfirstlane((int)(threadIdx.x >> 6)) : (int)(threadIdx.x >> 6);
    const bool no_new_blocks = d.counters[CTR_NINSERT] == d.counters[CTR_NPHYS_SEEN + ((epoch - 1u) & 1u)];
    const bool check_keys = ((epoch - 1u) & (EVICT_AGE - 1u)) == 0u;
    uint32_t movers = 0u;
    for (uint32_t id = wave; id < nphys; id += nwaves)
        movers += regroup_block<D, CDF, SHARD, SUMM>(d, side, epoch, id, nphys, have_old != 0, no_new_blocks, check_keys, s_in[w], s_out[w], s_pid[w], s_cols, cols_staged);
    if ((threadIdx.x & 63u) == 0u) s_wave[w] = movers;
    __syncthreads();
    if (threadIdx.x == 0) {
        const unsigned long long m = s_wave[0] + s_wave[1] + s_wave[2] + s_wave[3];
        if (m != 0ull) atomicAdd(&d.counters[CTR_MOVERS + 32u * (blockIdx.x & 15u)], (uint32_t)m);
    }
}

__global__ __launch_bounds__(256) void k_table_refresh(Dev d) {
    const uint32_t nphys = min(d.counters[CTR_NPHYS], d.cap);
    if (blockIdx.x == 0 && threadIdx.x == 0) d.counters[CTR_NTOMB] = 0u;
    for (uint32_t id = blockIdx.x * 256u + threadIdx.x; id < nphys; id += gridDim.x * 256u) {
        const uint32_t key = d.block_key[id];
        if (key == NONE) continue;
        uint32_t slot = hash_key(key) & d.hmask;
        for (uint32_t probe = 0; probe <= d.hmask; ++probe) {
            if (atomicCAS(&d.hkeys[slot], NONE, key) == NONE) {
                d.hvals[slot] = id;
                d.block_slot[id] = slot;
                break;
            }
            slot = (slot + 1u) & d.hmask;
        }
    }
}

__global__ __launch_bounds__(SORT_THREADS) void k_scan_only(Dev d, uint32_t epoch, uint32_t nscan) {
    __shared__ unsigned long long s_wave[SORT_THREADS / 64];
    __shared__ unsigned long long s_bcast;
    if (blockIdx.x < nscan) {
        scan_chunk(d, epoch, blockIdx.x, nscan, s_wave, &s_bcast);
        return;
    }
    const uint32_t nphys = min(d.counters[CTR_NPHYS], d.cap);
    const int lane = threadIdx.x & 63;
    const uint32_t wave = ((blockIdx.x - nscan) * SORT_THREADS + threadIdx.x) >> 6;
    const uint32_t nwaves = ((gridDim.x - nscan) * SORT_THREADS) >> 6;
    for (uint32_t id = wave; id < nphys; id += nwaves) {
        const GroupLoads g = block_prefix_loads(d, id, lane);
        uint32_t start = 0, aidx = 0;
        block_prefix(d, epoch, id, lane, g, nphys, start, aidx);
        if (lane == 0) {
            d.block_start[id] = start;
            d.active[aidx] = id;
        }
    }
}

}
```

wgsparkl_amd/csrc/kernels_transfer.h:

```cpp
#pragma once
#include "kernels_bodies.h"
#include "kernels_shard.h"

namespace wgs {

constexpr int P2G_J = 4;
#ifndef WGS_P2G_ROW_PAD
#define WGS_P2G_ROW_PAD 2
#endif
#ifdef WGS_ABLATE
constexpr int WGS_P2G_ROWS = 8192;
__device__ unsigned long long g_p2g_prof[WGS_P2G_ROWS][8];
#define P2G_PROF(k)                                                                                               \
    if (threadIdx.x == 0) {                                                                                       \
        if (filter != 2 && a < WGS_P2G_ROWS / 2) g_p2g_prof[a][k] = wall_clock64();                               \
        if (filter == 2 && a < WGS_P2G_ROWS / 16) g_p2g_prof[WGS_P2G_ROWS / 2 + (P2G_BLK & 7u) * (WGS_P2G_ROWS / 16) + a][k] = wall_clock64(); \
    }
#else
#define P2G_PROF(k)
#endif
template <int D> struct P2GCfg;
template <> struct P2GCfg<3> {
    static constexpr int NW = 3;
    static constexpr int NSXY = 9;
// ... 57 lines not shown
        for (int o = 0; o < NN; o++) {
            const uint32_t src = (uint32_t)__builtin_amdgcn_readlane((int)mysrc, o);
            const int tt[3] = {l[0] + BW * (o & 1), l[1] + BW * ((o >> 1) & 1), l[2] + BW * ((o >> 2) & 1)};
            const bool in_tile = tt[0] < TW && tt[1] < TW && (D == 2 || tt[2] < TW);
            rs[o] = slab_rsrc(&d.slab[(size_t)(src != NONE ? src : 0u) * TILE], src != NONE ? TILE * 16u : 0u);
            off[o] = in_tile ? slab_pos<D>(o, l) * 16u : 0x7ffffff0u;
            part[o] = ld_agent(rs[o], off[o]);
        }
        float4 sum = make_float4(0.f, 0.f, 0.f, 0.f);
#pragma unroll
        for (int o = 0; o < NN; o++) {
            sum.x += part[o].x; sum.y += part[o].y; sum.z += part[o].z; sum.w += part[o].w;
        }
        if constexpr (TWOWAY) {
            constexpr int IMPQ = D == 3 ? 2 : 1;
            float isum[6] = {0.f, 0.f, 0.f, 0.f, 0.f, 0.f};
#pragma unroll
            for (int o = 0; o < NN; o++) {
                const uint32_t src = (uint32_t)__builtin_amdgcn_readlane((int)mysrc, o);
                if (src == NONE || d.block_cpic[src] == 0u) continue;
                const __amdgpu_buffer_rsrc_t ri = slab_rsrc(&d.imp_slab[(size_t)src * TILE * IMPQ], TILE * IMPQ * 16u);
                const uint32_t io = off[o] < TILE * 16u ? off[o] * IMPQ : 0x7ffffff0u;
                const float4 a = ld_agent(ri, io);
                isum[0] += a.x; isum[1] += a.y; isum[2] += a.z;
                if constexpr (D == 3) {
                    const float4 bq = ld_agent(ri, io + 16u);
                    isum[3] += bq.x; isum[4] += bq.y; isum[5] += bq.z;
                }
            }
            const uint32_t cl = d.node_cdf[(size_t)b * NPB + (uint32_t)lane].closest_id;
            if (cl < 16u) {
                constexpr int NI = D == 3 ? 6 : 3;
#pragma unroll
                for (int k = 0; k < NI; k++) {
                    const int32_t v = flt2int(isum[k]);
                    if (v != 0) atomicAdd(&s_body_imp[cl * 8u + k], v);
                }
            }
        }
        const float4 nv = node_velocity<D>(sum, g, dt, lim);
#pragma unroll
        for (int o = 0; o < NN; o++) st_plain(rs[o], off[o], nv);
        d.nodes[b * NPB + (uint32_t)lane] = nv;
        if (lane == 0 && !d.bin_next) d.block_acc[b] = 0u;
    }
    if constexpr (TWOWAY) {
        __syncthreads();
        for (uint32_t i = threadIdx.x; i < 128u; i += blockDim.x) {
            const int32_t v = s_body_imp[i];
            if (v != 0) atomicAdd(&d.impulses[i], v);
        }
    }
}

template <int D> __device__ __forceinline__ void pcdf_waves(const Dev &d, int side, uint32_t epoch, uint32_t wave_of_list, uint32_t waves_per_list, uint32_t k, int lane, NodeCdf *tile) {
    if (!pcdf_waves_on(d, epoch, (uint32_t)P2GCfg<D>::NW)) return;
    const uint32_t nvis = min(d.counters[ctr_nvisit(k, epoch)], d.visit_cap);
    const uint2 *vl = d.visit_list + (size_t)k * d.visit_cap;
    const uint32_t nsorted = min(d.nv, d.counters[CTR_NSORTED]);
    float *buf = d.buf[side];
    uint32_t staged = NONE;
    for (uint32_t v = wave_of_list; v < nvis; v += waves_per_list) {
        const uint2 e = vl[v];
        const uint32_t b = (uint32_t)__builtin_amdgcn_readfirstlane((int)e.x);
        const uint32_t j = e.y * 64u + (uint32_t)lane;
        uint32_t cid = NONE, src = 0u;
        if (j < nsorted) {
            cid = d.perm_cell[j];
            src = d.perm[j];
        }
        const uint32_t bkey = d.block_key[b];
        const ParticleCdfIn in = particle_cdf_fetch<D>(d, buf, src);
        if (b != staged) {
            __builtin_amdgcn_fence(__ATOMIC_RELEASE, "wavefront");
            __builtin_amdgcn_wave_barrier();
            stage_node_cdf_tile<D, 64>(d, b, tile, lane);
            __builtin_amdgcn_fence(__ATOMIC_RELEASE, "wavefront");
            __builtin_amdgcn_wave_barrier();
            __builtin_amdgcn_fence(__ATOMIC_ACQUIRE, "wavefront");
            staged = b;
        }
        int bc[3] = {0, 0, 0};
        unpack_key<D>(bkey, bc);
        const bool mine = cid != NONE && ((cid & ~CELL_LISTED) >> 6) == b;
        if (mine) particle_cdf_update<D, true>(d, buf, src, in, tile, bc, epoch);
        const uint32_t done = (uint32_t)__popcll(__ballot(mine));
        asm volatile("s_waitcnt vmcnt(0)" ::: "memory");
        if (lane == 0 && done != 0u) __hip_atomic_fetch_add(&d.pcdf_done[b], done, __ATOMIC_RELAXED, __HIP_MEMORY_SCOPE_AGENT);
    }
}

template <int D, bool CPIC, bool TWOWAY = false, bool PCDF = false, int GU = 0, bool GUTW = TWOWAY>
__global__ __launch_bounds__(P2GCfg<D>::NW * 64) void k_p2g(Dev d, int side, int filter, uint32_t epoch, uint32_t nblk, uint32_t npack, uint32_t npack_blk, uint32_t layer_sel, uint32_t npro) {
    using Cfg = P2GCfg<D>;
    constexpr int TILE = Dim<D>::TILE;
    __shared__ float4 s_tile[Cfg::NW][TILE];
    if constexpr (PCDF) {
        if (blockIdx.x < npro) {
            const uint32_t w = threadIdx.x >> 6;
            pcdf_waves<D>(d, side, epoch, (blockIdx.x >> 3) * (uint32_t)Cfg::NW + w, (npro >> 3) * (uint32_t)Cfg::NW, blockIdx.x & 7u, (int)(threadIdx.x & 63u),
                          reinterpret_cast<NodeCdf *>(s_tile[w]));
            return;
        }
    }
    const uint32_t wg = blockIdx.x - (PCDF ? npro : 0u), nwg = gridDim.x - (PCDF ? npro : 0u);
    if constexpr (GU == 2) {
        if (wg >= nblk) {
            gu_waves<D, GUTW>(d, epoch, (wg - nblk) * Cfg::NW + (threadIdx.x >> 6), (nwg - nblk) * Cfg::NW, (int)(threadIdx.x & 63u));
            return;
        }
    }
    if constexpr (GU == 3) {
        if (wg >= nblk) {
            const uint32_t t = wg - nblk, w = threadIdx.x >> 6;
            const int lane = (int)(threadIdx.x & 63u);
            if (t < npack) pack_face_body<D, true>(d, side, epoch, t * Cfg::NW + w, npack_blk, npack * Cfg::NW, lane);
            else gu_waves<D, GUTW, true>(d, epoch, (t - npack) * Cfg::NW + w, (nwg - nblk - npack) * Cfg::NW, lane);
            return;
        }
    }
    constexpr int BW = Dim<D>::BW, BS = Dim<D>::BSHIFT, TW = Dim<D>::TW;
    constexpr int NT = Cfg::NW * 64;
    constexpr int SLOTS = P2G_J * NPB;
    constexpr int ROW = NPB + WGS_P2G_ROW_PAD;
    constexpr int KS = (SLOTS + NT - 1) / NT;
    constexpr int NQ = Cfg::NQ;
    __shared__ float4 s_q[NQ][P2G_J * ROW];
    __shared__ uint32_t s_aff[CPIC ? P2G_J * ROW : 1];
    __shared__ uint32_t s_cs[NPB], s_cn[NPB];
    constexpr int IMPQ = D == 3 ? 2 : 1;
    __shared__ float4 s_nrm[TWOWAY ? P2G_J * ROW : 1];
    __shared__ NodeCdf s_ncdf[PCDF ? TILE : 1];
    __shared__ float4 s_imp[TWOWAY ? Cfg::NW : 1][TWOWAY ? IMPQ : 1][TWOWAY ? TILE : 1];
    __shared__ ColliderMotion s_colm[TWOWAY ? 16 : 1];

#define P2G_CPIC CPIC
#define P2G_TWOWAY TWOWAY
#define P2G_PCDF PCDF
#define P2G_HANDOVER (GU != 0)
#define P2G_GUESTS_INLAUNCH (GU == 3)
#define P2G_BLK wg
#define P2G_NBLK nblk
#include "p2g_body.inc"
#undef P2G_CPIC
#undef P2G_TWOWAY
#undef P2G_PCDF
#undef P2G_BLK
#undef P2G_NBLK
#undef P2G_HANDOVER
#undef P2G_GUESTS_INLAUNCH
}

template <int D, bool TWOWAY, int WPE = 1, int GU = 0>
__global__ __launch_bounds__(P2GCfg<D>::NW * 64, WPE) void k_p2g_pair(Dev d, int side, uint32_t epoch, uint32_t half, uint32_t npack, uint32_t npack_blk, uint32_t layer_sel, uint32_t npro) {
    using Cfg = P2GCfg<D>;
    constexpr int TILE = Dim<D>::TILE;
    __shared__ float4 s_tile[Cfg::NW][TILE];
    if (blockIdx.x < npro) {
        static_assert(sizeof(NodeCdf) == sizeof(float4), "a wave's accumulation tile doubles as its node-cdf tile");
        const uint32_t w = threadIdx.x >> 6;
        pcdf_waves<D>(d, side, epoch, (blockIdx.x >> 3) * (uint32_t)Cfg::NW + w, (npro >> 3) * (uint32_t)Cfg::NW, blockIdx.x & 7u, (int)(threadIdx.x & 63u),
                      reinterpret_cast<NodeCdf *>(s_tile[w]));
        return;
    }
    const uint32_t wg = blockIdx.x - npro, nwg = gridDim.x - npro;
    if constexpr (GU == 2) {
        if (wg >= 2u * half) {
            gu_waves<D, TWOWAY>(d, epoch, (wg - 2u * half) * Cfg::NW + (threadIdx.x >> 6), (nwg - 2u * half) * Cfg::NW, (int)(threadIdx.x & 63u));
            return;
        }
    }
    if constexpr (GU == 3) {
        if (wg >= 2u * half) {
            const uint32_t t = wg - 2u * half, w = threadIdx.x >> 6;
            const int lane = (int)(threadIdx.x & 63u);
            if (t < npack) pack_face_body<D, true>(d, side, epoch, t * Cfg::NW + w, npack_blk, npack * Cfg::NW, lane);
            else gu_waves<D, TWOWAY, true>(d, epoch, (t - npack) * Cfg::NW + w, (nwg - 2u * half - npack) * Cfg::NW, lane);
            return;
        }
    }
    constexpr int BW = Dim<D>::BW, BS = Dim<D>::BSHIFT, TW = Dim<D>::TW;
    constexpr int NT = Cfg::NW * 64;
    constexpr int SLOTS = P2G_J * NPB;
    constexpr int ROW = NPB + WGS_P2G_ROW_PAD;
    constexpr int KS = (SLOTS + NT - 1) / NT;
    constexpr int NQ = Cfg::NQ;
    __shared__ float4 s_q[NQ][P2G_J * ROW];
    __shared__ uint32_t s_aff[P2G_J * ROW];
    __shared__ uint32_t s_cs[NPB], s_cn[NPB];
    constexpr int IMPQ = D == 3 ? 2 : 1;
    __shared__ float4 s_nrm[TWOWAY ? P2G_J * ROW : 1];
    __shared__ NodeCdf s_ncdf[TILE];
    __shared__ float4 s_imp[TWOWAY ? Cfg::NW : 1][TWOWAY ? IMPQ : 1][TWOWAY ? TILE : 1];
    __shared__ ColliderMotion s_colm[TWOWAY ? 16 : 1];
#define P2G_HANDOVER (GU != 0)
#define P2G_GUESTS_INLAUNCH (GU == 3)
#define P2G_NBLK half
    if (wg >= half) {
        const int filter = 1;
#define P2G_CPIC false
#define P2G_TWOWAY false
#define P2G_PCDF false
#define P2G_BLK (wg - half)
#include "p2g_body.inc"
#undef P2G_CPIC
#undef P2G_TWOWAY
#undef P2G_PCDF
#undef P2G_BLK
    } else {
        const int filter = 2;
#define P2G_CPIC true
#define P2G_TWOWAY TWOWAY
#define P2G_PCDF true
#define P2G_BLK wg
#include "p2g_body.inc"
#undef P2G_CPIC
#undef P2G_TWOWAY
#undef P2G_PCDF
#undef P2G_BLK
    }
#undef P2G_NBLK
#undef P2G_HANDOVER
#undef P2G_GUESTS_INLAUNCH
}


template <int D> __device__ inline float4 gather_slabs(const Dev &d, uint32_t b, uint32_t ln) {
    constexpr int BW = Dim<D>::BW, BS = Dim<D>::BSHIFT, TW = Dim<D>::TW, TILE = Dim<D>::TILE, NN = Dim<D>::NNBR;
    const int l[3] = {(int)(ln & (BW - 1)), (int)((ln >> BS) & (BW - 1)), D == 3 ? (int)(ln >> (2 * BS)) : 0};
    float4 sum = make_float4(0.f, 0.f, 0.f, 0.f);
#pragma unroll
    for (int o = 0; o < NN; o++) {
        const int tt[3] = {l[0] + BW * (o & 1), l[1] + BW * ((o >> 1) & 1), l[2] + BW * ((o >> 2) & 1)};
        const bool in_tile = tt[0] < TW && tt[1] < TW && (D == 2 || tt[2] < TW);
        if (!in_tile) continue;
        const uint32_t src = d.nbr_minus[b * 8u + o];
        if (src == NONE || d.block_count[src] == 0) continue;
        const float4 p = d.slab[(size_t)src * TILE + slab_pos<D>(o, l)];
        sum.x += p.x; sum.y += p.y; sum.z += p.z; sum.w += p.w;
    }
    return sum;
}

template <int D, int PHASE, bool TWOWAY = false> __global__ __launch_bounds__(256) void k_grid_update(Dev d, uint32_t epoch, uint32_t iface_only) {
    constexpr int BW = Dim<D>::BW, BS = Dim<D>::BSHIFT, TW = Dim<D>::TW, TILE = Dim<D>::TILE, NN = Dim<D>::NNBR;
    const uint32_t B = min(d.counters[CTR_NBLOCKS], d.cap);
    const uint32_t total = B * NPB;
    const float dt = d.sp->dt;
    const float lim = d.h / dt;
    float g[3] = {d.sp->gravity[0], d.sp->gravity[1], d.sp->gravity[2]};
    if (d.sharded && blockIdx.x == 0 && threadIdx.x == 0) d.counters[CTR_NLEAVE] = 0;
    __shared__ int32_t s_body_imp[TWOWAY ? 128 : 1];
    if constexpr (TWOWAY) {
        if (threadIdx.x < 128) s_body_imp[threadIdx.x] = 0;
        __syncthreads();
    }
    for (uint32_t t = blockIdx.x * 256 + threadIdx.x; t < total; t += gridDim.x * 256) {
        const uint32_t b = d.active[t >> 6], ln = t & 63u;
        const uint32_t node = b * NPB + ln;
        if constexpr (PHASE == 3) {
            if (iface_only) {
                int kc[3] = {0, 0, 0};
                unpack_key<D>(d.block_key[b], kc);
                const IfaceMasks im = iface_masks<D>(d, kc[0]);
                if ((im.recv | im.send_lo | im.send_hi) == 0u) continue;
            }
        }
        if (ln == 0u && !d.bin_next) d.block_acc[b] = 0u;
        int l[3];
        l[0] = ln & (BW - 1);
        l[1] = (ln >> BS) & (BW - 1);
        l[2] = D == 3 ? (ln >> (2 * BS)) : 0;
        float4 sum = make_float4(0.f, 0.f, 0.f, 0.f);
        float4 recv = make_float4(0.f, 0.f, 0.f, 0.f);
        if constexpr (PHASE == 3) {
            int bc[3] = {0, 0, 0};
            unpack_key<D>(d.block_key[b], bc);
            const uint32_t rmask = iface_masks<D>(d, bc[0]).recv;
            if (rmask != 0u) {
                int tag, q;
                halo_slot<D>(ln, tag, q);
                const int face = iface_recv_face(d, bc[0]);
                uint32_t mine = NONE;
#pragma unroll
                for (int tt = 0; tt < HaloCfg<D>::NTAG; tt++) {
                    if (!((rmask >> tt) & 1u)) continue;
                    const uint32_t slot = rec_find_wave<D>(d, face, d.block_key[b], (uint32_t)tt, epoch, (int)(threadIdx.x & 63u));
                    if (tt == tag) mine = slot;
                }
                if (mine != NONE) recv = msg_halo<D>(d.msg.in[face])[(size_t)mine * HaloCfg<D>::REC_F4 + 1 + q];
            }
        }
        float isum[6] = {0.f, 0.f, 0.f, 0.f, 0.f, 0.f};
        uint32_t srcs[NN];
        int tis[NN];
#pragma unroll
        for (int o = 0; o < NN; o++) {
            srcs[o] = NONE;
            int tt[3] = {l[0] + BW * (o & 1), l[1] + BW * ((o >> 1) & 1), l[2] + BW * ((o >> 2) & 1)};
            bool in_tile = tt[0] < TW && tt[1] < TW && (D == 2 || tt[2] < TW);
            if (!in_tile) continue;
            const uint32_t src = d.act_src[(t >> 6) * 8u + o];
            if (src == NONE) continue;
            int ti = (int)slab_pos<D>(o, l);
            srcs[o] = src;
            tis[o] = ti;
            {
                float4 p = d.slab[(size_t)src * TILE + ti];
                sum.x += p.x; sum.y += p.y; sum.z += p.z; sum.w += p.w;
            }
            if constexpr (TWOWAY) {
                if (d.block_cpic[src] != 0u) {
                    constexpr int IMPQ = D == 3 ? 2 : 1;
                    const float4 a = d.imp_slab[((size_t)src * TILE + ti) * IMPQ];
                    isum[0] += a.x; isum[1] += a.y; isum[2] += a.z;
                    if constexpr (D == 3) {
                        const float4 bq = d.imp_slab[((size_t)src * TILE + ti) * IMPQ + 1];
                        isum[3] += bq.x; isum[4] += bq.y; isum[5] += bq.z;
                    }
                }
            }
        }
        if constexpr (TWOWAY) {
            const uint32_t cl = d.node_cdf[node].closest_id;
            if (cl < 16u) {
                constexpr int NI = D == 3 ? 6 : 3;
#pragma unroll
                for (int k = 0; k < NI; k++) {
                    const int32_t v = flt2int(isum[k]);
                    if (v != 0) atomicAdd(&s_body_imp[cl * 8u + k], v);
                }
            }
        }
        if constexpr (PHASE == 3) {
            sum.x += recv.x; sum.y += recv.y; sum.z += recv.z; sum.w += recv.w;
        }
        const float4 nv = node_velocity<D>(sum, g, dt, lim);
#pragma unroll
        for (int o = 0; o < NN; o++)
            if (srcs[o] != NONE) d.slab[(size_t)srcs[o] * TILE + tis[o]] = nv;
        d.nodes[node] = nv;
    }
    if constexpr (TWOWAY) {
        __syncthreads();
        if (threadIdx.x < 128) {
            const int32_t v = s_body_imp[threadIdx.x];
            if (v != 0) atomicAdd(&d.impulses[threadIdx.x], v);
        }
    }
}

constexpr int G2P_THREADS = 64;
#ifdef WGS_ABLATE
constexpr int WGS_G2P_ROWS = 16384;
__device__ unsigned long long g_g2p_prof[WGS_G2P_ROWS][8];
#define G2P_PROF(k)                                                                                                   \
    if (threadIdx.x == 0) {                                                                                           \
        if (G2P_CMODE != 2 && chunk < WGS_G2P_ROWS / 2) g_g2p_prof[chunk][k] = wall_clock64();                        \
        if (G2P_CMODE == 2 && run * npass + (uint32_t)pass < WGS_G2P_ROWS / 4)                                        \
            g_g2p_prof[WGS_G2P_ROWS / 2 + run * npass + (uint32_t)pass][k] = wall_clock64();                          \
    }
#define G2P_PROF_LIST(k, v) if (threadIdx.x == 0 && G2P_CMODE == 2 && blockIdx.x < WGS_G2P_ROWS / 4) g_g2p_prof[WGS_G2P_ROWS * 3 / 4 + blockIdx.x][k] = (v);
#else
#define G2P_PROF(k)
#define G2P_PROF_LIST(k, v)
#endif
#ifndef G2P_WAVES_PER_EU
#define G2P_WAVES_PER_EU 3
#endif

#define G2P_DONE continue;
#define G2P_BIN BIN
#ifndef WGS_G2P_TWO_PASS_MIN
#define WGS_G2P_TWO_PASS_MIN 1500000
// ... 61 lines not shown
```

wgsparkl_amd/csrc/layout.h:

```cpp
#pragma once
#include <hip/hip_runtime.h>
#include <stdint.h>

#include <initializer_list>

#ifndef WGS_DIM
#define WGS_DIM 3
#endif

#ifdef WGS_ABLATE
#define WGS_ABLATE_AND(cond) &&(cond)
#else
#define WGS_ABLATE_AND(cond)
#endif

namespace wgs {

constexpr uint32_t NONE = 0xffffffffu;
constexpr uint32_t PID_DEAD = 0xffffffffu;
constexpr int NPB = 64;
constexpr uint32_t BLK_ARR = 64;

template <int D> struct Dim;
template <> struct Dim<3> {
    static constexpr int BW = 4, BSHIFT = 2, TW = 6, TILE = 216, NBH = 27, DD = 9, NNBR = 8, ANG = 3;
};
template <> struct Dim<2> {
    static constexpr int BW = 8, BSHIFT = 3, TW = 10, TILE = 100, NBH = 9, DD = 4, NNBR = 4, ANG = 1;
};

template <int D> struct Pl;
template <> struct Pl<3> {
    static constexpr int XM = 0;
    static constexpr int CV0 = 1;
    static constexpr int CV1 = 2;
    static constexpr int CV2 = 3;
    static constexpr int F0 = 4;
    static constexpr int F1 = 5;
    static constexpr int F2 = 6;
    static constexpr int NBASE = 7;
    static constexpr int DP0 = 7;
    static constexpr int DP1 = 8;
    static constexpr int DP2 = 9;
    static constexpr int CDF0 = 10;
    static constexpr int CDF1 = 11;
    static constexpr int NQ = 12;
};
template <> struct Pl<2> {
    static constexpr int XM = 0;
    static constexpr int CV0 = 1;
    static constexpr int CV2 = 2;
    static constexpr int F0 = 3;
    static constexpr int NBASE = 4;
    static constexpr int DP0 = 4;
    static constexpr int DP1 = 5;
    static constexpr int DP2 = 6;
    static constexpr int CDF0 = 7;
    static constexpr int CDF1 = 8;
    static constexpr int NQ = 9;
};
template <int D> constexpr size_t buffer_floats(uint32_t npad) { return ((size_t)Pl<D>::NQ * 4 + 2) * npad; }

struct SimParamsDev {
    float gravity[3];
    float dt;
};

struct ColliderDev {
    uint32_t shape_type;
    float shape[4];
    float rot[4];
    float trans[3];
    float scale;
    float linvel[3];
    float angvel[3];
    float com[3];
};

struct ColliderMotion {
    float linvel[3];
    float angvel[3];
    float com[3];
};

struct BodyDev {
    float inv_mass[3];
    float inv_inertia_local[9];
    float local_com[3];
    float inv_inertia_world[9];
};

struct NodeCdf {
    float distance;
    uint32_t affinities;
    uint32_t closest_id;
    uint32_t pad;
};

enum { CTR_NBLOCKS = 0, CTR_ERRORS = 1, CTR_NPHYS = 2,
       CTR_NSORTED = 3,
       CTR_N = 4, CTR_NV = 5,
       CTR_NPREV = 6,
       CTR_NLEAVE = 7,
       CTR_TICKET = 10,
       CTR_NFREE = 11,
       CTR_NINSERT = 12,
       CTR_NTOMB = 13,
       CTR_NPHYS_SEEN = 8,
       CTR_NVISIT = 64,
       CTR_NCPIC = 320,
       CTR_NHALO = 576,
       CTR_MOVERS = 640,
       CTR_COUNT = 1152 };
constexpr uint32_t CTR_PARITY = 16;
__host__ __device__ inline uint32_t ctr_ncpic(uint32_t k, uint32_t epoch) { return (uint32_t)CTR_NCPIC + 32u * k + CTR_PARITY * (epoch & 1u); }
__host__ __device__ inline uint32_t ctr_nvisit(uint32_t k, uint32_t epoch) { return (uint32_t)CTR_NVISIT + 32u * k + CTR_PARITY * (epoch & 1u); }
__host__ __device__ inline uint32_t ctr_nhalo(uint32_t epoch) { return (uint32_t)CTR_NHALO + CTR_PARITY * (epoch & 1u); }
enum { ERRBIT_OVERFLOW = 1u, ERRBIT_KEYRANGE = 2u, ERRBIT_SHARD = 4u, ERRBIT_MATERIAL = 8u, ERRBIT_HANDOVER = 16u,
       ERRBIT_PCDF = 32u };
constexpr uint32_t CELL_LISTED = 0x80000000u;
constexpr uint32_t CELL_DIRECT = 0x40000000u;
constexpr uint32_t CELL_MOVED = 0x80000000u;
__device__ inline uint32_t cell_of(uint32_t entry) { return entry == NONE ? NONE : (entry & ~CELL_MOVED); }
constexpr uint32_t HALO_ENT = 12;

struct ShardMsg {
    float *out[2];
    const float *in[2];
    uint32_t halo_cap, mig_cap;
};

struct Dev {
    uint32_t n;
    uint32_t nv;
    uint32_t sharded;
    int shard_lo, shard_hi;
    uint32_t shard_has_lo, shard_has_hi;
    uint32_t ctr_set;
    uint32_t skip_guests;
    ShardMsg msg;
    uint32_t npad;
    float *buf[2];
    uint32_t *perm;
    uint32_t *perm_cell;
    uint32_t *cellid;
    uint32_t *mv_next;
    uint32_t *hkeys;
    uint32_t *hvals;
    uint32_t hmask;
    uint32_t cap;
    uint32_t *block_key;
    uint32_t *block_slot;
    uint32_t *free_ids;
    uint32_t *block_stamp;
    uint32_t *links_epoch;
    uint32_t *block_acc;
    uint32_t *block_ident;
    uint32_t *blk_narr;
    uint32_t *blk_arr;
    uint32_t *block_dirty;
    uint32_t *block_count;
    uint32_t *block_start;
    uint32_t *active;
    uint4 *act_info;
    uint2 *act_cells;
    uint32_t *nbr_plus;
    uint32_t *nbr_minus;
    uint32_t *act_src;
    uint32_t *nbr_known;
    uint32_t *cell_head;
    uint32_t *cell_start;
    uint32_t *cell_cursor;
    unsigned long long *chunk_a, *chunk_b;
    unsigned long long *group_a, *group_b;
    float4 *nodes;
    NodeCdf *node_cdf;
    float4 *slab;
    uint32_t *slab_epoch;
    uint32_t *block_cdf_gen;
    uint32_t *block_cpic;
    uint32_t *block_cdf_summ;
    uint32_t *cpic_list;
    uint2 *visit_list;
    uint32_t *halo_list;
    uint32_t *pcdf_done;
    uint32_t pcdf_waves;
    uint32_t visit_cap;
    uint32_t cdf_gen;
    uint32_t cdf_moving;
    uint32_t listed_in_perm;
    uint32_t g2p_npass;
    uint32_t bin_next;
    uint32_t *counters;
    const SimParamsDev *sp;
    ColliderDev *colliders;
    uint32_t n_colliders;
    BodyDev *bodies;
    int32_t *impulses;
    float4 *imp_slab;
    uint32_t *leavers;
    uint32_t leavers_cap;
    uint32_t n_rigid, n_rvtx;
    float *rp_local, *rp_world;
    uint4 *rp_ids;
    float *rv_local, *rv_world;
    uint32_t *rv_collider;
    uint32_t *rp_needs;
    unsigned long long *mesh_min;
    uint32_t *mesh_aff;
    float h;
    float inv_h;
    uint32_t h_pow2;
    uint32_t uniform;
    float uni_mass, uni_vol, uni_lambda, uni_mu;
    uint32_t uni_dp;
    float uni_dpv[6], uni_max_stretch;
    int model;
    uint32_t dbg;
    float fluid_gamma;
    uint8_t *pmodel[2];
};

enum DebugSwitch : uint32_t {
    DBG_CDF_SUMM_NO_WAIT = 1u << 1,
    DBG_NO_PCDF_WAVES = 1u << 2,
    DBG_PCDF_WAVES_UNSIZED = 1u << 3,
    DBG_ABLATE_G2P_BYTES_ONLY = 1u << 6,
    DBG_NO_REBIN = 1u << 7,
    DBG_ABLATE_P2G_NO_ACCUM = 1u << 8,
    DBG_ABLATE_P2G_NO_LOADS = 1u << 9,
    DBG_NO_EVICTION = 1u << 10,
    DBG_NO_CDF_SUMM = 1u << 11,
    DBG_G2P_TWO_LAUNCHES = 1u << 12,
    DBG_P2G_TWO_LAUNCHES = 1u << 13,
    DBG_NO_G2P_DENSE = 1u << 14,
    DBG_NO_P2G_SMALL_BUDGET = 1u << 15,
    DBG_NO_UNIFORM = 1u << 16,
    DBG_G2P_TWO_PASSES = 1u << 17,
    DBG_GU_OWN_LAUNCH = 1u << 18,
    DBG_BODIES_OWN_LAUNCH = 1u << 19,
    DBG_REBIN_LAUNCH = 1u << 20,
    DBG_ABLATE_NO_BLOCK_CDF = 1u << 21,
    DBG_SHARD_SPLIT_LAYERS = 1u << 22,
    DBG_CELL_INSERTION_SORT = 1u << 24,
    DBG_NO_DIRECT_RUNS = 1u << 25,
    DBG_PLAIN_P2G_FIRST = 1u << 26,
};

constexpr uint32_t or_of_distinct_bits(std::initializer_list<uint32_t> bits) {
    uint32_t all = 0u;
    for (const uint32_t b : bits) {
        if (b == 0u || (b & (b - 1u)) != 0u || (all & b) != 0u) return 0u;
        all |= b;
    }
    return all;
}
constexpr uint32_t WGS_LAUNCH_SHAPE_SWITCHES = or_of_distinct_bits({
    DBG_CDF_SUMM_NO_WAIT, DBG_NO_PCDF_WAVES, DBG_PCDF_WAVES_UNSIZED, DBG_NO_REBIN, DBG_NO_EVICTION, DBG_NO_CDF_SUMM,
    DBG_G2P_TWO_LAUNCHES, DBG_P2G_TWO_LAUNCHES, DBG_NO_G2P_DENSE, DBG_NO_P2G_SMALL_BUDGET, DBG_NO_UNIFORM, DBG_G2P_TWO_PASSES,
    DBG_GU_OWN_LAUNCH, DBG_BODIES_OWN_LAUNCH, DBG_REBIN_LAUNCH, DBG_SHARD_SPLIT_LAYERS, DBG_CELL_INSERTION_SORT,
    DBG_NO_DIRECT_RUNS, DBG_PLAIN_P2G_FIRST});
constexpr uint32_t WGS_ABLATION_SWITCHES = or_of_distinct_bits({
    DBG_ABLATE_G2P_BYTES_ONLY, DBG_ABLATE_P2G_NO_ACCUM, DBG_ABLATE_P2G_NO_LOADS, DBG_ABLATE_NO_BLOCK_CDF});
static_assert(WGS_LAUNCH_SHAPE_SWITCHES != 0u && WGS_ABLATION_SWITCHES != 0u && (WGS_LAUNCH_SHAPE_SWITCHES & WGS_ABLATION_SWITCHES) == 0u,
              "WGS_DEBUG switches must be distinct single bits");

constexpr uint32_t CTR_SET = 16;
__device__ inline uint32_t &ctr_cur(const Dev &d, uint32_t which) { return d.counters[which + CTR_SET * d.ctr_set]; }
__device__ inline uint32_t &ctr_next(const Dev &d, uint32_t which) { return d.counters[which + CTR_SET * (d.ctr_set ^ 1u)]; }
__device__ inline uint32_t num_slots(const Dev &d) { return d.sharded ? ctr_cur(d, CTR_N) : d.n; }
__device__ inline uint32_t num_valid(const Dev &d) { return d.sharded ? ctr_cur(d, CTR_NV) : d.nv; }
__device__ inline uint32_t g2p_waves_per_xcd(const Dev &d, uint32_t npass) {
    const uint32_t span = 64u * npass;
    return ((num_valid(d) + span - 1u) / span + 7u) >> 3;
}

template <int D> __host__ __device__ constexpr int slab_region_base(int o) {
    int base = 0;
    for (int r = 0; r < o; r++) {
        int sz = 1;
        for (int k = 0; k < D; k++) sz *= ((r >> k) & 1) ? 2 : Dim<D>::BW;
        base += sz;
    }
    return base;
}
template <int D> __device__ inline uint32_t slab_pos(int o, const int *l) {
    constexpr int BW = Dim<D>::BW;
    const int ex = (o & 1) ? 2 : BW, ey = (o & 2) ? 2 : BW;
    int base = 0;
#pragma unroll
    for (int r = 0; r < (1 << D); r++)
        if (r == o) base = slab_region_base<D>(r);
    return (uint32_t)(base + l[0] + ex * (l[1] + (D == 3 ? ey * l[2] : 0)));
}
template <int D> __host__ __device__ constexpr uint32_t slab_tile_of(uint32_t p) {
    constexpr int BW = Dim<D>::BW, TW = Dim<D>::TW;
    int o = 0;
    for (int r = 1; r < (1 << D); r++)
        if (p >= (uint32_t)slab_region_base<D>(r)) o = r;
    const uint32_t q = p - (uint32_t)slab_region_base<D>(o);
    const uint32_t sx = (o & 1) ? 1u : (uint32_t)Dim<D>::BSHIFT, sy = (o & 2) ? 1u : (uint32_t)Dim<D>::BSHIFT;
    const uint32_t lx = q & ((1u << sx) - 1u), ly = (q >> sx) & ((1u << sy) - 1u), lz = D == 3 ? q >> (sx + sy) : 0u;
    const uint32_t tx = lx + ((o & 1) ? BW : 0), ty = ly + ((o & 2) ? BW : 0), tz = lz + ((o & 4) ? BW : 0);
    return tx + TW * ty + (D == 3 ? TW * TW * tz : 0u);
}
template <int D> struct SlabTileMap {
    uint8_t t[Dim<D>::TILE];
    constexpr SlabTileMap() : t{} {
        for (int p = 0; p < Dim<D>::TILE; p++) t[p] = (uint8_t)slab_tile_of<D>((uint32_t)p);
    }
};
__constant__ SlabTileMap<WGS_DIM> g_slab_tile_map = SlabTileMap<WGS_DIM>();
template <int D> __host__ __device__ constexpr uint32_t slab_pos_of_tile(uint32_t t) {
    constexpr uint32_t BW = Dim<D>::BW, TW = Dim<D>::TW, BS = Dim<D>::BSHIFT;
    const uint32_t tz = D == 3 ? t / (TW * TW) : 0u, r = D == 3 ? t - tz * (TW * TW) : t, ty = r / TW, tx = r - ty * TW;
    const uint32_t ox = tx >= BW ? 1u : 0u, oy = ty >= BW ? 1u : 0u, oz = tz >= BW ? 1u : 0u;
    const uint32_t o = ox | (oy << 1) | (oz << 2);
    unsigned long long bases = 0ull;
    for (int q = 0; q < (1 << D); q++) bases |= (unsigned long long)slab_region_base<D>(q) << (8 * q);
    const uint32_t sx = ox ? 1u : BS, sy = oy ? 1u : BS;
    return (uint32_t)((bases >> (8u * o)) & 0xffull) + (tx - ox * BW) + (((ty - oy * BW) + ((tz - oz * BW) << sy)) << sx);
}
template <int D> constexpr bool slab_pos_of_tile_inverts_the_map() {
    static_assert(slab_region_base<D>((1 << D) - 1) < 256, "the region bases are packed a byte each");
    for (int p = 0; p < Dim<D>::TILE; p++)
        if (slab_pos_of_tile<D>(slab_tile_of<D>((uint32_t)p)) != (uint32_t)p) return false;
    return true;
}
static_assert(slab_pos_of_tile_inverts_the_map<2>() && slab_pos_of_tile_inverts_the_map<3>(), "slab_pos_of_tile is the inverse of slab_tile_of at every node");

__device__ inline float4 ldq(const float *base, uint32_t npad, int q, uint32_t i) {
    uint32_t off = ((uint32_t)q * npad + i) * 16u;
    asm volatile("" : "+v"(off));
    return *reinterpret_cast<const float4 *>(reinterpret_cast<const char *>(base) + off);
}
__device__ inline void stq(float *base, uint32_t npad, int q, uint32_t i, float4 v) {
    uint32_t off = ((uint32_t)q * npad + i) * 16u;
    asm volatile("" : "+v"(off));
    *reinterpret_cast<float4 *>(reinterpret_cast<char *>(base) + off) = v;
}
__device__ inline float4 ldq_stream(const float *base, uint32_t npad, int q, uint32_t i) {
    typedef float v4f __attribute__((ext_vector_type(4)));
    uint32_t off = ((uint32_t)q * npad + i) * 16u;
    asm volatile("" : "+v"(off));
    const v4f nv = __builtin_nontemporal_load(reinterpret_cast<const v4f *>(reinterpret_cast<const char *>(base) + off));
    return make_float4(nv.x, nv.y, nv.z, nv.w);
}
typedef uint32_t wgs_v4u __attribute__((ext_vector_type(4)));
constexpr int WGS_CPOL_SC1 = 16;
__device__ inline __amdgpu_buffer_rsrc_t slab_rsrc(float4 *slab_of_block, uint32_t bytes) {
    return __builtin_amdgcn_make_buffer_rsrc(slab_of_block, 0, bytes, 0x00020000);
}
__device__ inline void st_agent(__amdgpu_buffer_rsrc_t r, uint32_t byte_off, const float4 v) {
    const wgs_v4u u = {__float_as_uint(v.x), __float_as_uint(v.y), __float_as_uint(v.z), __float_as_uint(v.w)};
    __builtin_amdgcn_raw_buffer_store_b128(u, r, byte_off, 0, WGS_CPOL_SC1);
}
__device__ inline void st_plain(__amdgpu_buffer_rsrc_t r, uint32_t byte_off, const float4 v) {
    const wgs_v4u u = {__float_as_uint(v.x), __float_as_uint(v.y), __float_as_uint(v.z), __float_as_uint(v.w)};
    __builtin_amdgcn_raw_buffer_store_b128(u, r, byte_off, 0, 0);
}
__device__ inline float4 ld_agent(__amdgpu_buffer_rsrc_t r, uint32_t byte_off) {
    const wgs_v4u u = __builtin_amdgcn_raw_buffer_load_b128(r, byte_off, 0, WGS_CPOL_SC1);
    return make_float4(__uint_as_float(u.x), __uint_as_float(u.y), __uint_as_float(u.z), __uint_as_float(u.w));
}
__device__ __forceinline__ uint32_t wave_max_u32(uint32_t v) {
    v = max(v, (uint32_t)__builtin_amdgcn_update_dpp(0, (int)v, 0x111, 0xf, 0xf, true));
    v = max(v, (uint32_t)__builtin_amdgcn_update_dpp(0, (int)v, 0x112, 0xf, 0xf, true));
    v = max(v, (uint32_t)__builtin_amdgcn_update_dpp(0, (int)v, 0x114, 0xf, 0xf, true));
    v = max(v, (uint32_t)__builtin_amdgcn_update_dpp(0, (int)v, 0x118, 0xf, 0xf, true));
    v = max(v, (uint32_t)__builtin_amdgcn_update_dpp(0, (int)v, 0x142, 0xa, 0xf, false));
    v = max(v, (uint32_t)__builtin_amdgcn_update_dpp(0, (int)v, 0x143, 0xc, 0xf, false));
    return (uint32_t)__builtin_amdgcn_readlane((int)v, 63);
}
__device__ __forceinline__ uint32_t wave_scan_incl_u32(uint32_t v) {
    v += (uint32_t)__builtin_amdgcn_update_dpp(0, (int)v, 0x111, 0xf, 0xf, true);
    v += (uint32_t)__builtin_amdgcn_update_dpp(0, (int)v, 0x112, 0xf, 0xf, true);
    v += (uint32_t)__builtin_amdgcn_update_dpp(0, (int)v, 0x114, 0xf, 0xf, true);
    v += (uint32_t)__builtin_amdgcn_update_dpp(0, (int)v, 0x118, 0xf, 0xf, true);
    v += (uint32_t)__builtin_amdgcn_update_dpp(0, (int)v, 0x142, 0xa, 0xf, false);
    v += (uint32_t)__builtin_amdgcn_update_dpp(0, (int)v, 0x143, 0xc, 0xf, false);
    return v;
}
__device__ __forceinline__ uint32_t wave_sum_u32(uint32_t v) { return (uint32_t)__builtin_amdgcn_readlane((int)wave_scan_incl_u32(v), 63); }
__device__ __forceinline__ uint32_t lane_value(uint32_t v, int uniform_lane) { return (uint32_t)__builtin_amdgcn_readlane((int)v, uniform_lane); }
template <int D> __device__ inline uint32_t ldpid(const float *base, uint32_t npad, uint32_t i) {
    uint32_t off = ((uint32_t)Pl<D>::NQ * 4u * npad + i) * 4u;
    asm volatile("" : "+v"(off));
    return *reinterpret_cast<const uint32_t *>(reinterpret_cast<const char *>(base) + off);
}
template <int D> __host__ __device__ inline const uint32_t *pid_plane(const float *base, uint32_t npad) {
    return reinterpret_cast<const uint32_t *>(base + (size_t)Pl<D>::NQ * 4 * npad);
}
template <int D> __host__ __device__ inline uint32_t *pid_plane(float *base, uint32_t npad) {
    return const_cast<uint32_t *>(pid_plane<D>(static_cast<const float *>(base), npad));
}
template <int D> __device__ inline uint32_t ldstamp(const float *base, uint32_t npad, uint32_t i) {
    uint32_t off = (((uint32_t)Pl<D>::NQ * 4u + 1u) * npad + i) * 4u;
    asm volatile("" : "+v"(off));
    return *reinterpret_cast<const uint32_t *>(reinterpret_cast<const char *>(base) + off);
}
template <int D> __device__ inline void ststamp(float *base, uint32_t npad, uint32_t i, uint32_t e) {
    uint32_t off = (((uint32_t)Pl<D>::NQ * 4u + 1u) * npad + i) * 4u;
    asm volatile("" : "+v"(off));
    *reinterpret_cast<uint32_t *>(reinterpret_cast<char *>(base) + off) = e;
}
template <int D> __device__ inline __amdgpu_buffer_rsrc_t particle_rsrc(float *base, uint32_t npad) {
    return __builtin_amdgcn_make_buffer_rsrc(base, 0, ((uint32_t)Pl<D>::NQ * 4u + 2u) * npad * 4u, 0x00020000);
}
__device__ inline uint32_t quad_off(uint32_t npad, int q, uint32_t i) { return ((uint32_t)q * npad + i) * 16u; }
template <int D> __device__ inline uint32_t *stamp_ptr(float *base, uint32_t npad, uint32_t i) {
    return reinterpret_cast<uint32_t *>(base) + ((size_t)((uint32_t)Pl<D>::NQ * 4u + 1u) * npad + i);
}
template <int D> __device__ inline void stpid(float *base, uint32_t npad, uint32_t i, uint32_t pid) {
    uint32_t off = ((uint32_t)Pl<D>::NQ * 4u * npad + i) * 4u;
// ... 17 lines not shown
```

wgsparkl_amd/csrc/p2g_body.inc:

```
    const float *in = d.buf[side];
    const uint32_t npad = d.npad;
    const float h = d.h, inv_h = d.inv_h;
    const int tid0 = threadIdx.x;
    const int sz = D == 3 ? (tid0 >> 6) : 0;

    const bool pcdf_thru = P2G_PCDF && pcdf_waves_on(d, epoch, (uint32_t)Cfg::NW);
    bool s_pcdf_timed_out = false;
    if constexpr (P2G_TWOWAY) {
        for (uint32_t i = (uint32_t)tid0; i < min(d.n_colliders, 16u) * 9u; i += (uint32_t)NT)
            reinterpret_cast<float *>(s_colm)[i] = reinterpret_cast<const float *>(&d.colliders[i / 9u].linvel)[i % 9u];
        __syncthreads();
    }
    int tmap[(TILE + NT - 1) / NT];
#pragma unroll
    for (int kk = 0; kk < (TILE + NT - 1) / NT; kk++) tmap[kk] = tid0 + kk * NT < TILE ? (int)g_slab_tile_map.t[tid0 + kk * NT] : 0;
    uint32_t pending = NONE;
    const uint32_t B = min(d.counters[filter == 2 ? ctr_ncpic(P2G_BLK & 7u, epoch) : (uint32_t)CTR_NBLOCKS], d.cap);
    for (uint32_t a = filter == 2 ? P2G_BLK >> 3 : P2G_BLK; a < B; a += filter == 2 ? P2G_NBLK >> 3 : P2G_NBLK) {
        int tid = tid0;
        asm volatile("" : "+v"(tid));
        const int cell = tid & 63;
        int lc[3];
        lc[0] = cell & (BW - 1);
        lc[1] = (cell >> BS) & (BW - 1);
        lc[2] = D == 3 ? (cell >> (2 * BS)) : 0;
        const int tnode0 = lc[0] + TW * lc[1] + (D == 3 ? TW * TW * (lc[2] + sz) : 0);
        P2G_PROF(0)
        uint32_t b = 0u, cnt = 0u, cs = 0u, cn = 0u, key = 0u;
        bool skip = false;
        bool direct = false;
        if (filter == 2) {
            b = d.cpic_list[(size_t)(P2G_BLK & 7u) * d.cap + a];
            cnt = d.block_count[b];
            key = d.block_key[b];
            cs = d.cell_start[b * NPB + cell];
            cn = d.cell_cursor[b * NPB + cell] - cs;
        } else {
            const uint4 info = d.act_info[a];
            const uint2 cr = d.act_cells[(size_t)a * NPB + cell];
            b = info.x;
            key = info.y;
            cnt = info.z;
            cs = cr.x;
            cn = cr.y - cr.x;
            direct = (info.w & CELL_DIRECT) != 0u;
            if (filter == 1) skip = d.listed_in_perm ? (info.w & CELL_LISTED) != 0u : d.block_cpic[b] != 0u;
        }
        if (layer_sel != 0u) {
            int kb[3] = {0, 0, 0};
            unpack_key<D>(key, kb);
            if (shard_boundary_layer(d, kb[0]) != (layer_sel == 1u)) skip = true;
        }
        if constexpr (P2G_HANDOVER) {
            if (cnt == 0 && filter != 2 && tid == 0) __hip_atomic_store(&d.slab_epoch[b], epoch, __ATOMIC_RELAXED, __HIP_MEMORY_SCOPE_AGENT);
        }
        if (cnt == 0 || skip) continue;
#ifdef WGS_ABLATE
        if (!P2G_CPIC) { P2G_PROF(6) }
#endif
        int bc[3] = {0, 0, 0};
        unpack_key<D>(key, bc);
        __syncthreads();
        if constexpr (P2G_PCDF) {
          stage_node_cdf_tile<D, NT>(d, b, s_ncdf, tid);
          bool own_prologue = !pcdf_thru;
          if (pcdf_thru) {
            if (tid == 0) {
                const unsigned long long t_start = wall_clock64();
                uint32_t gave_up = 0u;
                while (__hip_atomic_load(&d.pcdf_done[b], __ATOMIC_RELAXED, __HIP_MEMORY_SCOPE_AGENT) != cnt) {
                    if (s_pcdf_timed_out || wall_clock64() - t_start > 20000000ull) {
                        atomicOr(&d.counters[CTR_ERRORS], ERRBIT_PCDF);
                        gave_up = 1u;
                        s_pcdf_timed_out = true;
                        break;
                    }
                    __builtin_amdgcn_s_sleep(4);
                }
                s_cs[0] = gave_up;
            }
            __syncthreads();
            own_prologue = s_cs[0] != 0u;
            __syncthreads();
          }
          if (own_prologue) {
            __syncthreads();
            const uint32_t bstart = d.block_start[b];
            {
                const uint32_t jend = bstart + cnt;
                uint32_t j = bstart + (uint32_t)tid;
                uint32_t src0 = j < jend ? d.perm[j] : NONE;
                uint32_t src1 = j + (uint32_t)NT < jend ? d.perm[j + (uint32_t)NT] : NONE;
                ParticleCdfIn in0 = {make_float4(0.f, 0.f, 0.f, 0.f), 0u, 0u};
                if (src0 != NONE) in0 = particle_cdf_fetch<D>(d, d.buf[side], src0);
#pragma unroll 1
                while (src0 != NONE) {
                    const uint32_t src2 = j + 2u * (uint32_t)NT < jend ? d.perm[j + 2u * (uint32_t)NT] : NONE;
                    ParticleCdfIn in1 = {make_float4(0.f, 0.f, 0.f, 0.f), 0u, 0u};
                    if (src1 != NONE) in1 = particle_cdf_fetch<D>(d, d.buf[side], src1);
                    particle_cdf_update<D, P2G_GUESTS_INLAUNCH>(d, d.buf[side], src0, in0, s_ncdf, bc, epoch);
                    src0 = src1;
                    in0 = in1;
                    src1 = src2;
                    j += (uint32_t)NT;
                }
            }
            __threadfence_block();
            __syncthreads();
          }
        }
        if (P2G_CPIC) { P2G_PROF(6) }
        if (tid < NPB) {
            s_cs[cell] = cs;
            s_cn[cell] = cn;
        }
        for (int n = cell; n < TILE; n += 64) s_tile[sz][n] = make_float4(0.f, 0.f, 0.f, 0.f);
        if constexpr (P2G_TWOWAY) {
            for (int n = cell; n < TILE; n += 64)
                for (int q = 0; q < IMPQ; q++) s_imp[sz][q][n] = make_float4(0.f, 0.f, 0.f, 0.f);
        }
        const uint32_t maxc = wave_max_u32(cn);
#ifdef WGS_ABLATE
        if (!P2G_CPIC && maxc != 0xfffffffeu) { P2G_PROF(7) }
#endif
        float cpos[D];
#pragma unroll
        for (int k = 0; k < D; k++) cpos[k] = (float)(bc[k] * BW + lc[k]) * h;
        uint32_t naff[Cfg::NSXY];
        unsigned long long ncol = 0ull;
        if constexpr (P2G_CPIC) {
#pragma unroll
            for (int s = 0; s < 9; s++) {
                int t[3] = {lc[0] + s % 3, lc[1] + s / 3, lc[2] + sz};
                int o = (t[0] >= BW ? 1 : 0) | (t[1] >= BW ? 2 : 0) | (t[2] >= BW ? 4 : 0);
                int ln = (t[0] & (BW - 1)) + ((t[1] & (BW - 1)) << BS) + (D == 3 ? ((t[2] & (BW - 1)) << (2 * BS)) : 0);
                if constexpr (P2G_PCDF) {
                    const NodeCdf nc = s_ncdf[tnode0 + (s % 3) + TW * (s / 3)];
                    naff[s] = nc.affinities;
                    if constexpr (P2G_TWOWAY) {
                        if (nc.closest_id < 16u) ncol |= ((unsigned long long)nc.closest_id << (4 * s)) | (1ull << (36 + s));
                    }
                } else {
                    uint32_t nb = d.nbr_plus[b * 8u + o];
                    naff[s] = nb != NONE ? d.node_cdf[(size_t)nb * NPB + ln].affinities : 0u;
                    if constexpr (P2G_TWOWAY) {
                        const uint32_t cl = nb != NONE ? d.node_cdf[(size_t)nb * NPB + ln].closest_id : NONE;
                        if (cl < 16u) ncol |= ((unsigned long long)cl << (4 * s)) | (1ull << (36 + s));
                    }
                }
            }
        }
        if (P2G_CPIC) { P2G_PROF(7) }
        float acc[Cfg::NSXY][D + 1];
#pragma unroll
        for (int s = 0; s < 9; s++)
#pragma unroll
            for (int k = 0; k <= D; k++) acc[s][k] = 0.f;

        float4 pre[KS][NQ];
        float4 pre_nrm[P2G_TWOWAY ? KS : 1];
        uint32_t pre_aff[KS];
        bool pre_ok[KS];
        __syncthreads();
        P2G_PROF(1)
        auto fetch_round = [&](uint32_t r0) {
#pragma unroll
            for (int k = 0; k < KS; k++) {
                const int sl = tid + k * NT;
                pre_ok[k] = false;
                if (sl < SLOTS) {
// ... 221 lines not shown
```

wgsparkl_amd/pipeline.py:

```python
from __future__ import annotations

import ctypes as C
from dataclasses import dataclass
from typing import Dict, Optional, Sequence

import numpy as np

from . import _ffi
from .models import MODEL_COROTATED
from .solver import Collider, ParticleSet, SimulationParams

F32 = np.float32


@dataclass
class FixedSum:
    fixed: np.ndarray
    exponent: int
    value: np.ndarray

    def __float__(self):
        return float(self.value[0])


# ... 153 lines not shown
    u[:, off("has_plasticity")] = hp.astype(np.uint32)
    o = off("plasticity"); raw[:, o:o + 6] = ps.dp
    u[:, off("has_phase")] = hph.astype(np.uint32)
    o = off("phase"); raw[:, o:o + 2] = ps.phase
    return raw


def _offset_words(struct, path: str) -> int:
    off = 0
    cur = struct
    for name in path.split("."):
        fld = getattr(cur, name)
        off += fld.offset
        cur = dict((f[0], f[1]) for f in cur._fields_)[name]
    return off // 4


def _unpack_particles(T, raw: np.ndarray, D: int, plastic: Optional[np.ndarray]) -> ParticleSet:
    u = raw.view(np.uint32)
    off = lambda path: _offset_words(T.Particle, path)
    sl = lambda path, k: raw[:, off(path):off(path) + k].copy()
    n = raw.shape[0]
    return ParticleSet(
        dim=D, pos=sl("position", D), vel=sl("dynamics.velocity", D), def_grad=sl("dynamics.def_grad", D * D),
        affine=sl("dynamics.affine", D * D), cdf_normal=sl("dynamics.cdf.normal", D),
        cdf_rigid_vel=sl("dynamics.cdf.rigid_vel", D), cdf_dist=raw[:, off("dynamics.cdf.signed_distance")].copy(),
        cdf_affinity=u[:, off("dynamics.cdf.affinity")].copy(), init_volume=raw[:, off("dynamics.init_volume")].copy(),
        init_radius=raw[:, off("dynamics.init_radius")].copy(), mass=raw[:, off("dynamics.mass")].copy(),
        lambda_=raw[:, off("model.lambda_")].copy(), mu=raw[:, off("model.mu")].copy(), dp=sl("plasticity", 6),
        dp_state=plastic if plastic is not None else np.tile(np.array([1, 1, 0], F32), (n, 1)),
        phase=sl("phase", 2), has_plasticity=u[:, off("has_plasticity")] != 0, has_phase=u[:, off("has_phase")] != 0)


def _is_dynamic(c: Collider) -> bool:
    return any(float(v) != 0.0 for v in list(c.inv_mass) + list(c.inv_inertia_local))


def _fill_collider(T, dst, c: Collider, D: int):
    dst.shape_type = int(c.shape_type)
    sh = list(c.shape) + [0.0] * (4 - len(c.shape))
    dst.shape = (C.c_float * 4)(*sh)
    if D == 2:
        ang = F32(c.rotation[0])
        dst.pose.rotation = (C.c_float * 4)(float(np.cos(ang)), float(np.sin(ang)), 0.0, 0.0)
    else:
        dst.pose.rotation = (C.c_float * 4)(*c.rotation)
    t = list(c.translation) + [0.0] * (3 - len(c.translation))
    dst.pose.translation = (C.c_float * 3)(*t)
    dst.pose.scale = c.scale
    dst.velocity.linear = (C.c_float * 3)(*(list(c.linvel)[:D] + [0.0] * (3 - D)))
    dst.velocity.angular = (C.c_float * 3)(*((list(c.angvel) + [0.0, 0.0, 0.0])[:3]))
    com = list(c.com) if c.com is not None else list(c.translation)
    dst.com = (C.c_float * 3)(*(com + [0.0] * (3 - len(com))))


class DataHandle:

    def __init__(self, pipeline: MpmPipeline, colliders: Sequence[Collider]):
        self.pipeline, self.lib, self.T, self.dim = pipeline, pipeline.lib, pipeline.T, pipeline.dim
        self.n_colliders = len(colliders)
        self._h = None

    def _sim_params(self, params: SimulationParams):
        sp = self.T.SimParams()
        sp.gravity = (C.c_float * self.dim)(*params.gravity)
        sp.dt = params.dt
        return sp

    def _collider_array(self, colliders: Sequence[Collider]):
        cols = (self.T.Collider * max(1, len(colliders)))()
        for i, c in enumerate(colliders):
            _fill_collider(self.T, cols[i], c, self.dim)
        return cols

    def set_constitutive_model(self, model: int):
        _ffi.check(self.lib, self.lib.wgs_set_constitutive_model(self._h, int(model)))

    def set_fluid_eos(self, gamma: float):
        _ffi.check(self.lib, self.lib.wgs_set_fluid_eos(self._h, float(gamma)))

    def set_sim_params(self, params: SimulationParams):
        _ffi.check(self.lib, self.lib.wgs_set_sim_params(self._h, C.byref(self._sim_params(params))))

    def set_colliders(self, colliders: Sequence[Collider]):
        n = len(colliders)
        tmp = self._collider_array(colliders)
        poses = (self.T.Pose * max(1, n))()
        vels = (self.T.Velocity * max(1, n))()
        coms = (C.c_float * (3 * max(1, n)))()
        for i in range(n):
            poses[i] = tmp[i].pose
            vels[i] = tmp[i].velocity
            for k in range(3):
                coms[3 * i + k] = tmp[i].com[k]
        _ffi.check(self.lib, self.lib.wgs_set_collider_poses(self._h, poses, coms, n))
        _ffi.check(self.lib, self.lib.wgs_set_body_velocities(self._h, vels, n))
        self.set_body_mass_properties(colliders)

    def set_rigid_particles(self, rb: dict):
        pts = np.ascontiguousarray(rb["local_pts"], F32)
        ids = np.ascontiguousarray(rb["ids"], np.uint32)
        vtx = np.ascontiguousarray(rb["local_vtx"], F32)
        vcol = np.ascontiguousarray(rb["vtx_collider"], np.uint32)
        fp, up = C.POINTER(C.c_float), C.POINTER(C.c_uint32)
        _ffi.check(self.lib, self.lib.wgs_set_rigid_particles(
            self._h, pts.ctypes.data_as(fp), ids.ctypes.data_as(C.c_void_p), len(pts), vtx.ctypes.data_as(fp),
            vcol.ctypes.data_as(up), len(vtx)))

    def _set_mesh_samples(self, colliders: Sequence[Collider], cell_width: float):
        from .sampling import build_rigid_particles
        rb = build_rigid_particles(colliders, self.dim, float(cell_width))
        if rb is not None:
            self.set_rigid_particles(rb)

    def set_body_mass_properties(self, colliders: Sequence[Collider]):
        n = len(colliders)
        mp = (self.T.MassProperties * max(1, n))()
        for i, c in enumerate(colliders):
            im = (list(c.inv_mass) + [0.0] * 3)[:3]
            ii = (list(c.inv_inertia_local) + [0.0] * 9)[:9]
            mp[i].inv_mass = (C.c_float * 3)(*im)
            mp[i].inv_inertia_local = (C.c_float * 9)(*ii)
        _ffi.check(self.lib, self.lib.wgs_set_body_mass_properties(self._h, mp, n))

    def read_body_poses(self):
        n, D = self.n_colliders, self.dim
        poses = (self.T.Pose * max(1, n))()
        vels = (self.T.Velocity * max(1, n))()
        coms = (C.c_float * (3 * max(1, n)))()
        _ffi.check(self.lib, self.lib.wgs_read_body_poses(self._h, poses, vels, coms, n))
        out = []
        for i in range(n):
            out.append(dict(rotation=np.array(list(poses[i].rotation)[:(2 if D == 2 else 4)], np.float64),
                            translation=np.array(list(poses[i].translation)[:D], np.float64),
                            linvel=np.array(list(vels[i].linear)[:D], np.float64),
                            angvel=np.array(list(vels[i].angular)[:(1 if D == 2 else 3)], np.float64),
                            com=np.array([coms[3 * i + k] for k in range(D)], np.float64)))
        return out

    def sync(self):
        _ffi.check(self.lib, self.lib.wgs_sync(self._h))

    def diagnostics(self, what: int = _ffi.DIAG_PARTICLES) -> Diagnostics:
        return read_diagnostics(self.lib, self._h, self.dim, what)

    def enqueue_diagnostics(self, device_ptr: int, what: int = _ffi.DIAG_PARTICLES):
        _ffi.check(self.lib, self.lib.wgs_enqueue_diagnostics(self._h, int(what), C.c_void_p(int(device_ptr))))

    def stats(self):
        s = self.T.Stats()
        _ffi.check(self.lib, self.lib.wgs_get_stats(self._h, C.byref(s)))
        return {k: int(getattr(s, k)) for k, _ in s._fields_}

    def close(self):
        if getattr(self, "_h", None):
            self.lib.wgs_data_destroy(self._h)
            self._h = None

    def __del__(self):
        try:
            self.close()
        except Exception:
            pass


class MpmData(DataHandle):

    def __init__(self, pipeline: MpmPipeline, params: SimulationParams, particles: ParticleSet,
                 colliders: Sequence[Collider], cell_width: float, grid_capacity: int,
                 model: int = MODEL_COROTATED):
        super().__init__(pipeline, colliders)
        if particles.dim != self.dim:
            raise ValueError("particle dimension does not match the pipeline")
        self.n = particles.n
        raw = _pack_particles(self.T, particles)
        h = C.c_void_p()
        _ffi.check(self.lib, self.lib.wgs_data_create(
            pipeline._h, C.byref(self._sim_params(params)), raw.ctypes.data_as(C.POINTER(self.T.Particle)), self.n,
            self._collider_array(colliders), len(colliders), float(cell_width), int(grid_capacity), C.byref(h)))
        self._h = h
        if model != MODEL_COROTATED:
            self.set_constitutive_model(model)
        if any(_is_dynamic(c) for c in colliders):
            self.set_body_mass_properties(colliders)
        self._set_mesh_samples(colliders, cell_width)

    @classmethod
    def new(cls, pipeline, params, particles, colliders, cell_width, grid_capacity, model=MODEL_COROTATED):
        if not isinstance(particles, ParticleSet):
            particles = ParticleSet.from_particles(particles)
        return cls(pipeline, params, particles, colliders, cell_width, grid_capacity, model)

    @classmethod
    def from_scene(cls, pipeline, scene, **overrides):
        sc = {"model": MODEL_COROTATED, **scene, **overrides}
        return cls.new(pipeline, sc["params"], sc["particles"], sc["colliders"], sc["cell_width"], sc["grid_capacity"], sc["model"])

    def set_particle_models(self, models):
        if models is None:
            _ffi.check(self.lib, self.lib.wgs_set_particle_models(self._h, None))
            return
        m = np.ascontiguousarray(models, np.uint8).reshape(-1)
        if m.shape[0] != self.n:
            raise ValueError("set_particle_models: one entry per particle")
        _ffi.check(self.lib, self.lib.wgs_set_particle_models(self._h, m.ctypes.data_as(C.POINTER(C.c_uint8))))

    def read_particle_models(self) -> np.ndarray:
        out = np.zeros(self.n, np.uint8)
        _ffi.check(self.lib, self.lib.wgs_read_particle_models(self._h, out.ctypes.data_as(C.POINTER(C.c_uint8))))
        return out

    def read_positions(self) -> np.ndarray:
        out = np.zeros((self.n, self.dim), F32)
        _ffi.check(self.lib, self.lib.wgs_read_positions(self._h, out.ctypes.data_as(C.POINTER(C.c_float))))
        return out

    def device_ptrs(self):
        v = _ffi.DevicePtrs()
        _ffi.check(self.lib, self.lib.wgs_get_device_ptrs(self._h, C.byref(v)))
        return v

    def read_particles(self) -> ParticleSet:
        T = self.T
        words = C.sizeof(T.Particle) // 4
        raw = np.zeros((self.n, words), F32)
        plastic = np.zeros((self.n, 3), F32)
        _ffi.check(self.lib, self.lib.wgs_read_particles(
            self._h, raw.ctypes.data_as(C.POINTER(T.Particle)), plastic.ctypes.data_as(C.POINTER(T.PlasticState))))
        return _unpack_particles(T, raw, self.dim, plastic)

    def prep_vertex_buffer(self, mode: int = 0, base_color=None) -> np.ndarray:
        inst = np.zeros((self.n, 24), F32)
        inst[:, 16:20] = 1.0 if base_color is None else np.asarray(base_color, F32).reshape(self.n, 4)
        _ffi.check(self.lib, self.lib.wgs_prep_vertex_buffer(self._h, int(mode), inst.ctypes.data_as(C.c_void_p)))
        return inst

    def set_plastic_state(self, dp_state: np.ndarray):
        st = np.ascontiguousarray(dp_state, F32).reshape(self.n, 3)
        _ffi.check(self.lib, self.lib.wgs_set_plastic_state(self._h, st.ctypes.data_as(C.POINTER(self.T.PlasticState))))

    def read_grid(self):
        T, D = self.T, self.dim
        cnt = C.c_size_t(0)
        _ffi.check(self.lib, self.lib.wgs_read_grid(self._h, None, 0, C.byref(cnt)))
        m = cnt.value
        words = C.sizeof(T.NodeRecord) // 4
        raw = np.zeros((max(m, 1), words), np.int32)
        if m:
            _ffi.check(self.lib, self.lib.wgs_read_grid(self._h, raw.ctypes.data_as(C.POINTER(T.NodeRecord)), m, C.byref(cnt)))
        raw = raw[:m]
        cells = raw[:, :D].copy()
        fl = raw.view(F32)
        vm = fl[:, D:2 * D + 1].copy()
        dist = fl[:, 2 * D + 1].copy()
        aff = raw.view(np.uint32)[:, 2 * D + 2].copy()
        closest = raw.view(np.uint32)[:, 2 * D + 3].copy()
        order = np.lexsort(cells.T[::-1]) if m else np.zeros(0, np.int64)
        return cells[order], vm[order], dist[order], aff[order], closest[order]

    def read_blocks(self, with_sorted_ids: bool = True):
        T, D = self.T, self.dim
        cnt = C.c_size_t(0)
        _ffi.check(self.lib, self.lib.wgs_read_blocks(self._h, None, 0, C.byref(cnt), None))
        m = cnt.value
        raw = np.zeros((max(m, 1), D + 2), np.int32)
        ids = np.zeros(max(self.n, 1), np.uint32)
        _ffi.check(self.lib, self.lib.wgs_read_blocks(
            self._h, raw.ctypes.data_as(C.POINTER(T.BlockRecord)), m, C.byref(cnt),
            ids.ctypes.data_as(C.POINTER(C.c_uint32)) if with_sorted_ids else None))
        raw = raw[:m]
        vid = raw[:, :D].copy()
        order = np.lexsort(vid.T[::-1]) if m else np.zeros(0, np.int64)
        u = raw.view(np.uint32)
        return vid[order], u[:, D][order].copy(), u[:, D + 1][order].copy(), ids[:self.n]

    def particle_fields(self) -> ParticleFields:
        words = np.zeros((self.n, C.sizeof(self.T.ParticleField) // 4), np.uint32)
        _ffi.check(self.lib, self.lib.wgs_read_particle_fields(self._h, words.ctypes.data_as(C.POINTER(self.T.ParticleField))))
        return particle_fields_from_words(words, self.dim)

    def particle_fields_device(self, out_ptr: int):
        _ffi.check(self.lib, self.lib.wgs_read_particle_fields_device(self._h, C.c_void_p(int(out_ptr))))

    def sample_grid(self, points) -> GridSamples:
        D = self.dim
        pts = np.ascontiguousarray(points, F32).reshape(-1, D)
        n = pts.shape[0]
        words = np.zeros((n, C.sizeof(self.T.GridSample) // 4), np.uint32)
        _ffi.check(self.lib, self.lib.wgs_sample_grid(self._h, pts.ctypes.data_as(C.POINTER(C.c_float)), n,
                                                      words.ctypes.data_as(C.POINTER(self.T.GridSample))))
        return grid_samples_from_words(words, D)

    def sample_grid_device(self, points_ptr: int, n: int, out_ptr: int):
        _ffi.check(self.lib, self.lib.wgs_sample_grid_device(self._h, C.c_void_p(int(points_ptr)), int(n), C.c_void_p(int(out_ptr))))

    def _window_args(self, lo, dims):
        D = self.dim
        lo = np.ascontiguousarray(lo, np.int32).reshape(D)
        dims = np.ascontiguousarray(dims, np.uint32).reshape(D)
        return lo, dims, lo.ctypes.data_as(C.POINTER(C.c_int32)), dims.ctypes.data_as(C.POINTER(C.c_uint32))

    def grid_window(self, lo, dims):
        D = self.dim
        lo, dims, plo, pdims = self._window_args(lo, dims)
        total = int(np.prod(dims.astype(np.uint64)))
        ok = bool(np.all(dims >= 1)) and total < 2 ** 31
# ... 15 lines not shown
```

Measured before the change: 5.649 billion particle-steps/s.

## Compact P2G work list to particle-bearing blocks and size CPIC workgroups separately

Adds a third prefix-scan channel during block sorting that counts active blocks holding particles, and writes act_info/act_cells compacted by that rank so P2G iterates only over blocks with particles (CTR_NP2G) rather than all active blocks. The plain P2G launch is sized from the bearing-block count, and the CPIC half gets its own workgroup count derived from ncpic instead of mirroring the plain half. This cuts empty-block iterations and idle workgroups, at the cost of extra scan work, extra tagged publishes and buffers, and a split between active-index and p2g-rank indexing.

```diff
diff --git a/wgsparkl_amd/csrc/capi_debug.inc b/wgsparkl_amd/csrc/capi_debug.inc
--- a/wgsparkl_amd/csrc/capi_debug.inc
+++ b/wgsparkl_amd/csrc/capi_debug.inc
@@ -24,14 +24,16 @@
     dev.cap = std::max(1u, n);
     const uint32_t nscan = (dev.cap + SCAN_CHUNK - 1) / SCAN_CHUNK, epoch = 1u;
     Scratch<uint32_t> counters, stamp, acc, active, start;
-    Scratch<unsigned long long> chunk_a, chunk_b, group_a, group_b;
+    Scratch<unsigned long long> chunk_a, chunk_b, group_a, group_b, chunk_c, group_c;
     const size_t ngroup = (size_t)nscan * SORT_THREADS;
     if (counters.alloc(CTR_COUNT, true) != WGS_OK || stamp.alloc(dev.cap, true) != WGS_OK || acc.alloc(dev.cap, true) != WGS_OK ||
         active.alloc(dev.cap, true) != WGS_OK || start.alloc(dev.cap, true) != WGS_OK || chunk_a.alloc(nscan, true) != WGS_OK ||
-        chunk_b.alloc(nscan, true) != WGS_OK || group_a.alloc(ngroup, true) != WGS_OK || group_b.alloc(ngroup, true) != WGS_OK)
+        chunk_b.alloc(nscan, true) != WGS_OK || group_a.alloc(ngroup, true) != WGS_OK || group_b.alloc(ngroup, true) != WGS_OK ||
+        chunk_c.alloc(nscan, true) != WGS_OK || group_c.alloc(ngroup, true) != WGS_OK)
         return fail(WGS_ERR_HIP, "out of device memory");
     dev.counters = counters.ptr; dev.block_stamp = stamp.ptr; dev.block_acc = acc.ptr; dev.active = active.ptr; dev.block_start = start.ptr;
     dev.chunk_a = chunk_a.ptr; dev.chunk_b = chunk_b.ptr; dev.group_a = group_a.ptr; dev.group_b = group_b.ptr;
+    dev.chunk_c = chunk_c.ptr; dev.group_c = group_c.ptr;
     std::vector<uint32_t> ones(dev.cap, epoch);
     uint32_t ctr[CTR_COUNT] = {0};
     ctr[CTR_NPHYS] = n;
@@ -54,6 +56,27 @@
     return WGS_OK;
 }
 
+wgs_status wgs_debug_p2g_list(wgs_data *d, uint32_t *records, uint32_t *active, size_t capacity, size_t *nlist, size_t *nactive) {
+    WGS_TRY(enter(d, nlist && nactive));
+    WGS_TRY(fetch_counters(d));
+    uint32_t np2g = 0;
+    WGS_TRY(download(d, &np2g, d->dev.counters + CTR_NP2G, sizeof(uint32_t)));
+    *nlist = std::min(np2g, d->dev.cap);
+    *nactive = d->seen.sync_nblocks;
+    if (capacity < *nlist || capacity < *nactive) return fail(WGS_ERR_INVALID_ARGUMENT, "capacity too small; *nlist and *nactive hold the required sizes");
+    if (records && *nlist) WGS_TRY(download(d, records, d->dev.act_info, sizeof(uint4) * *nlist));
+    if (active && *nactive) {
+        std::vector<uint32_t> ids(*nactive), counts(d->dev.cap);
+        WGS_TRY(download(d, ids.data(), d->dev.active, sizeof(uint32_t) * *nactive));
+        WGS_TRY(download(d, counts.data(), d->dev.block_count, sizeof(uint32_t) * counts.size()));
+        for (size_t a = 0; a < *nactive; a++) {
+            active[2 * a] = ids[a];
+            active[2 * a + 1] = ids[a] < d->dev.cap ? counts[ids[a]] : 0u;
+        }
+    }
+    return WGS_OK;
+}
+
 #ifdef WGS_ABLATE
 static wgs_status read_and_reset_prof(const void *symbol, unsigned long long *out, size_t rows) {
     const std::vector<unsigned long long> zero(rows * 8, 0ull);
diff --git a/wgsparkl_amd/csrc/host_grid.inc b/wgsparkl_amd/csrc/host_grid.inc
--- a/wgsparkl_amd/csrc/host_grid.inc
+++ b/wgsparkl_amd/csrc/host_grid.inc
@@ -35,6 +35,8 @@
     WGS_TRY(grid_array(&dev.chunk_b, nchunk));
     WGS_TRY(grid_array(&dev.group_a, nchunk * SORT_THREADS));
     WGS_TRY(grid_array(&dev.group_b, nchunk * SORT_THREADS));
+    WGS_TRY(grid_array(&dev.chunk_c, nchunk));
+    WGS_TRY(grid_array(&dev.group_c, nchunk * SORT_THREADS));
     WGS_TRY(grid_array(&dev.cell_start, cap * NPB));
     WGS_TRY(grid_array(&dev.cell_cursor, cap * NPB));
     WGS_TRY(grid_array(&dev.nodes, cap * NPB));
@@ -113,6 +115,7 @@
     if (d->dev.sharded) d->seen.nv_hint = std::max(d->seen.watch[CTR_NV], d->seen.watch[CTR_NV + CTR_SET]);
     const uint32_t rate = nblocks > d->seen.nblocks && d->seen.nblocks != 0u ? nblocks - d->seen.nblocks : 0u;
     d->seen.nblocks = std::min(nblocks, cap);
+    d->seen.nbear = std::min(d->seen.watch[CTR_NP2G], cap);
     const uint64_t ahead = (uint64_t)nblocks + 3ull * rate;
     if (d->auto_grow && (nblocks > cap / 2u || ahead > cap / 4u * 3u) && cap < (1u << 24)) {
         uint32_t new_cap = cap * 2u;
@@ -145,6 +148,7 @@
     HIP_TRY(hipStreamSynchronize(d->stream));
     d->seen.sync_nblocks = host[CTR_NBLOCKS] < d->dev.cap ? host[CTR_NBLOCKS] : d->dev.cap;
     d->seen.nblocks = d->seen.sync_nblocks;
+    d->seen.nbear = std::min(host[CTR_NP2G], d->dev.cap);
     const uint32_t last_epoch = (uint32_t)d->substeps;
     d->seen.ncpic = 0;
     for (uint32_t k = 0; k < 8; k++) d->seen.ncpic += std::min(host[ctr_ncpic(k, last_epoch)], d->dev.cap);
diff --git a/wgsparkl_amd/csrc/host_state.h b/wgsparkl_amd/csrc/host_state.h
--- a/wgsparkl_amd/csrc/host_state.h
+++ b/wgsparkl_amd/csrc/host_state.h
@@ -255,6 +255,7 @@
         uint32_t watch_skips = 0;
         uint32_t errors = 0;
         uint32_t nblocks = 0;
+        uint32_t nbear = 0;
         uint32_t sync_nblocks = 0;
         uint32_t nv_hint = 0;
         uint32_t ncpic = UINT32_MAX;
diff --git a/wgsparkl_amd/csrc/host_substep.inc b/wgsparkl_amd/csrc/host_substep.inc
--- a/wgsparkl_amd/csrc/host_substep.inc
+++ b/wgsparkl_amd/csrc/host_substep.inc
@@ -53,17 +53,18 @@
     bool small_budget;
     int gu;
     uint32_t wgs;
+    uint32_t ncpic_wgs;
     uint32_t ride;
     uint32_t npack, npack_blk, layer_sel;
     uint32_t npro;
 };
 
 template <int DIM, bool TW, int WPE> void launch_p2g_pair(Dev &dev, hipStream_t s, int side, uint32_t epoch, const P2gLaunch &p) {
-    const dim3 g(p.npro + 2u * p.wgs + p.ride), b(P2GCfg<DIM>::NW * 64);
+    const dim3 g(p.npro + p.ncpic_wgs + p.wgs + p.ride), b(P2GCfg<DIM>::NW * 64);
     dev.pcdf_waves = p.npro;
-    if (p.gu == 2) hipLaunchKernelGGL((k_p2g_pair<DIM, TW, WPE, 2>), g, b, 0, s, dev, side, epoch, p.wgs, p.npack, p.npack_blk, p.layer_sel, p.npro);
-    else if (p.gu == 3) hipLaunchKernelGGL((k_p2g_pair<DIM, TW, WPE, 3>), g, b, 0, s, dev, side, epoch, p.wgs, p.npack, p.npack_blk, p.layer_sel, p.npro);
-    else hipLaunchKernelGGL((k_p2g_pair<DIM, TW, WPE, 0>), g, b, 0, s, dev, side, epoch, p.wgs, p.npack, p.npack_blk, p.layer_sel, p.npro);
+    if (p.gu == 2) hipLaunchKernelGGL((k_p2g_pair<DIM, TW, WPE, 2>), g, b, 0, s, dev, side, epoch, p.ncpic_wgs, p.wgs, p.npack, p.npack_blk, p.layer_sel, p.npro);
+    else if (p.gu == 3) hipLaunchKernelGGL((k_p2g_pair<DIM, TW, WPE, 3>), g, b, 0, s, dev, side, epoch, p.ncpic_wgs, p.wgs, p.npack, p.npack_blk, p.layer_sel, p.npro);
+    else hipLaunchKernelGGL((k_p2g_pair<DIM, TW, WPE, 0>), g, b, 0, s, dev, side, epoch, p.ncpic_wgs, p.wgs, p.npack, p.npack_blk, p.layer_sel, p.npro);
     dev.pcdf_waves = 0u;
 }
 
@@ -223,7 +224,8 @@
     P2gLaunch p{};
     p.two_way = d->two_way;
     p.layer_sel = layers == P2gLayers::boundary ? 1u : layers == P2gLayers::others ? 2u : 0u;
-    p.wgs = std::min((uint32_t)grid_for(d, 32), std::max((uint32_t)grid_for(d, 8), (d->seen.nblocks / 2u + 255u) & ~255u));
+    p.wgs = std::min((uint32_t)grid_for(d, 32), std::max((uint32_t)grid_for(d, 8), (d->seen.nbear / 2u + 255u) & ~255u));
+    p.ncpic_wgs = d->seen.ncpic == UINT32_MAX ? p.wgs : std::min(p.wgs, std::max(256u, (2u * d->seen.ncpic + 7u) & ~7u));
     p.gu = d->sub.gu_fused ? 2 : d->sub.shard_fused ? 3 : 0;
     const uint32_t gu_wgs = (p.gu == 0 || layers == P2gLayers::boundary) ? 0u : std::min((uint32_t)grid_for(d, 8), std::max((uint32_t)grid_for(d, 1), ((d->seen.nblocks + NW - 1u) / NW + 7u) & ~7u));
     if (d->sub.shard_fused && (d->link->has_lower || d->link->has_upper) && layers != P2gLayers::others) {
@@ -362,6 +364,7 @@
         launch_regroup<DIM>(dev, s, dim3(p.nscan + p.nreg), side, epoch, p.nscan, p.have_old, p.cdf, p.summ);
     } else {
         HIP_TRY(hipMemsetAsync(dev.counters + CTR_NBLOCKS, 0, sizeof(uint32_t), s));
+        HIP_TRY(hipMemsetAsync(dev.counters + CTR_NP2G, 0, sizeof(uint32_t), s));
     }
     mark(1);
     if (dev.n_rigid > 0 && n > 0)
diff --git a/wgsparkl_amd/csrc/kernels_sort.h b/wgsparkl_amd/csrc/kernels_sort.h
--- a/wgsparkl_amd/csrc/kernels_sort.h
+++ b/wgsparkl_amd/csrc/kernels_sort.h
@@ -247,6 +247,9 @@
     if (tid == 0 && k == 0) g_prof[WGS_PROF_ROWS - 1][1] = wall_clock64();
 #endif
     unsigned long long sum = 0ull;
+    __shared__ uint32_t s_bear[SORT_THREADS / 64], s_bear_before;
+    const bool full_list = SHARD || (d.dbg & DBG_P2G_FULL_LIST) != 0u;
+    uint32_t bear = 0u;
     const uint32_t first = k * SCAN_CHUNK + (uint32_t)tid * SCAN_ITEMS;
     uint32_t stamp[SCAN_ITEMS], acc[SCAN_ITEMS];
 #pragma unroll
@@ -259,16 +262,24 @@
     for (int j = 0; j < SCAN_ITEMS; j++) {
         const bool act = first + j < nphys && stamp[j] == epoch;
         sum += act ? ((1ull << 32) | (unsigned long long)acc[j]) : 0ull;
+        bear += (act && (full_list || acc[j] != 0u)) ? 1u : 0u;
     }
     const unsigned long long inc = ((unsigned long long)wave_scan_incl_u32((uint32_t)(sum >> 32)) << 32) | (unsigned long long)wave_scan_incl_u32((uint32_t)sum);
-    if (lane == 63) s_wave[wave] = inc;
+    const uint32_t bear_inc = wave_scan_incl_u32(bear);
+    if (lane == 63) {
+        s_wave[wave] = inc;
+        s_bear[wave] = bear_inc;
+    }
     __syncthreads();
     unsigned long long wave_off = 0ull, total = 0ull;
+    uint32_t bear_off = 0u, bear_total = 0u;
 #pragma unroll
     for (int w = 0; w < SORT_THREADS / 64; w++) {
         const unsigned long long t = s_wave[w];
-        if (w < wave) wave_off += t;
+        const uint32_t tb = s_bear[w];
+        if (w < wave) { wave_off += t; bear_off += tb; }
         total += t;
+        bear_total += tb;
     }
 #ifdef WGS_ABLATE
     if (tid == 0 && k == 0) g_prof[WGS_PROF_ROWS - 1][2] = wall_clock64();
@@ -276,27 +287,43 @@
     if (tid == 0) {
         publish_tagged(&d.chunk_a[k], epoch, (uint32_t)(total >> 32));
         publish_tagged(&d.chunk_b[k], epoch, (uint32_t)total);
+        publish_tagged(&d.chunk_c[k], epoch, bear_total);
     }
     unsigned long long part = 0ull;
-    for (uint32_t p = (uint32_t)tid; p < k; p += SORT_THREADS)
+    uint32_t part_c = 0u;
+    for (uint32_t p = (uint32_t)tid; p < k; p += SORT_THREADS) {
         part += ((unsigned long long)wait_tagged(&d.chunk_a[p], epoch) << 32) + wait_tagged(&d.chunk_b[p], epoch);
+        part_c += wait_tagged(&d.chunk_c[p], epoch);
+    }
     part = ((unsigned long long)wave_sum_u32((uint32_t)(part >> 32)) << 32) + (unsigned long long)wave_sum_u32((uint32_t)part);
+    part_c = wave_sum_u32(part_c);
     __syncthreads();
-    if (lane == 0) s_wave[wave] = part;
+    if (lane == 0) {
+        s_wave[wave] = part;
+        s_bear[wave] = part_c;
+    }
     __syncthreads();
     if (tid == 0) {
         unsigned long long b = 0ull;
-        for (int w = 0; w < SORT_THREADS / 64; w++) b += s_wave[w];
+        uint32_t bc = 0u;
+        for (int w = 0; w < SORT_THREADS / 64; w++) {
+            b += s_wave[w];
+            bc += s_bear[w];
+        }
         *s_bcast = b;
+        s_bear_before = bc;
     }
     __syncthreads();
     const unsigned long long base = *s_bcast;
+    const uint32_t base_c = s_bear_before;
     const unsigned long long run = base + wave_off + inc - sum;
     publish_tagged(&d.group_a[k * SORT_THREADS + tid], epoch, (uint32_t)(run >> 32));
     publish_tagged(&d.group_b[k * SORT_THREADS + tid], epoch, (uint32_t)run);
+    publish_tagged(&d.group_c[k * SORT_THREADS + tid], epoch, base_c + bear_off + bear_inc - bear);
     if (tid == 0 && k + 1 == nchunks) {
         d.counters[CTR_NBLOCKS] = (uint32_t)((base + total) >> 32);
         d.counters[CTR_NSORTED] = (uint32_t)(base + total);
+        d.counters[CTR_NP2G] = base_c + bear_total;
     }
 #ifdef WGS_ABLATE
     if (tid == 0) g_prof[WGS_PROF_ROWS - 1][0] = wall_clock64();
@@ -321,15 +348,17 @@
     }
     return g;
 }
-__device__ inline void block_prefix(const Dev &d, uint32_t epoch, uint32_t id, int lane, const GroupLoads &g, uint32_t nphys, uint32_t &start, uint32_t &aidx) {
+__device__ inline void block_prefix(const Dev &d, uint32_t epoch, uint32_t id, int lane, const GroupLoads &g, uint32_t nphys, bool full_list, uint32_t &start, uint32_t &aidx, uint32_t &p2g_rank) {
     const uint32_t gbase = id & ~(uint32_t)(SCAN_ITEMS - 1), j = id & (uint32_t)(SCAN_ITEMS - 1);
     const bool before = lane < (int)j && gbase + (uint32_t)lane < nphys && g.stamp == epoch;
     const uint32_t cnt = (uint32_t)__popcll(__ballot(before));
+    const uint32_t cnt_c = (uint32_t)__popcll(__ballot(before && (full_list || g.acc != 0u)));
     uint32_t psum = before ? g.acc : 0u;
     psum = wave_sum_u32(psum);
     const uint32_t grp = id / SCAN_ITEMS;
     aidx = wait_tagged(&d.group_a[grp], epoch) + cnt;
     start = wait_tagged(&d.group_b[grp], epoch) + psum;
+    p2g_rank = wait_tagged(&d.group_c[grp], epoch) + cnt_c;
 }
 
 constexpr uint32_t OUT_CELL_SHIFT = 26, OUT_SRC_MASK = 0x03ffffffu;
@@ -746,8 +775,10 @@
     const uint32_t lstart = inc - total;
     WGS_PROF(2)
     const bool out_lds = btotal <= (uint32_t)RUNCAP;
-    uint32_t bstart = 0, aidx = 0;
-    auto fetch_bstart = [&]() { block_prefix(d, epoch, id, lane, grp, nphys, bstart, aidx); };
+    const bool full_list = SHARD || (d.dbg & DBG_P2G_FULL_LIST) != 0u;
+    const bool p2g_listed = full_list || bcount > 0u;
+    uint32_t bstart = 0, aidx = 0, p2g_rank = 0;
+    auto fetch_bstart = [&]() { block_prefix(d, epoch, id, lane, grp, nphys, full_list, bstart, aidx, p2g_rank); };
     if (!out_lds) fetch_bstart();
     const bool fast_clean = old_ok && clean && !any_arr;
     bool keep_perm = false;
@@ -998,7 +1029,7 @@
     d.cell_start[idx] = bstart + lstart;
     d.cell_cursor[idx] = bstart + lstart + total;
     const bool direct = fast_clean && !(d.dbg & DBG_NO_DIRECT_RUNS);
-    d.act_cells[(size_t)aidx * NPB + lane] = direct ? make_uint2(cs_old, ce_old) : make_uint2(bstart + lstart, bstart + lstart + total);
+    if (p2g_listed) d.act_cells[(size_t)p2g_rank * NPB + lane] = direct ? make_uint2(cs_old, ce_old) : make_uint2(bstart + lstart, bstart + lstart + total);
     if (head != 0u) d.cell_head[idx] = 0u;
     if (lane == 0 && narr != 0u) d.blk_narr[id] = 0u;
     if (d.n_rigid != 0u) {
@@ -1008,7 +1039,7 @@
     if (lane >= 8 && lane < 16) d.act_src[aidx * 8u + (uint32_t)(lane & 7)] = link_cnt > 0u ? res : NONE;
     if (lane == 63) {
         d.active[aidx] = id;
-        d.act_info[aidx] = make_uint4(id, bkey, btotal, pc_flag | (direct ? CELL_DIRECT : 0u));
+        if (p2g_listed) d.act_info[p2g_rank] = make_uint4(id, bkey, btotal, pc_flag | (direct ? CELL_DIRECT : 0u));
         d.block_start[id] = bstart;
         d.block_count[id] = btotal;
         d.links_epoch[id] = epoch;
@@ -1106,8 +1137,8 @@
     const uint32_t nwaves = ((gridDim.x - nscan) * SORT_THREADS) >> 6;
     for (uint32_t id = wave; id < nphys; id += nwaves) {
         const GroupLoads g = block_prefix_loads(d, id, lane);
-        uint32_t start = 0, aidx = 0;
-        block_prefix(d, epoch, id, lane, g, nphys, start, aidx);
+        uint32_t start = 0, aidx = 0, rank = 0;
+        block_prefix(d, epoch, id, lane, g, nphys, false, start, aidx, rank);
         if (lane == 0) {
             d.block_start[id] = start;
             d.active[aidx] = id;
diff --git a/wgsparkl_amd/csrc/kernels_transfer.h b/wgsparkl_amd/csrc/kernels_transfer.h
--- a/wgsparkl_amd/csrc/kernels_transfer.h
+++ b/wgsparkl_amd/csrc/kernels_transfer.h
@@ -233,7 +233,7 @@
 }
 
 template <int D, bool TWOWAY, int WPE = 1, int GU = 0>
-__global__ __launch_bounds__(P2GCfg<D>::NW * 64, WPE) void k_p2g_pair(Dev d, int side, uint32_t epoch, uint32_t half, uint32_t npack, uint32_t npack_blk, uint32_t layer_sel, uint32_t npro) {
+__global__ __launch_bounds__(P2GCfg<D>::NW * 64, WPE) void k_p2g_pair(Dev d, int side, uint32_t epoch, uint32_t ncw, uint32_t half, uint32_t npack, uint32_t npack_blk, uint32_t layer_sel, uint32_t npro) {
     using Cfg = P2GCfg<D>;
     constexpr int TILE = Dim<D>::TILE;
     __shared__ float4 s_tile[Cfg::NW][TILE];
@@ -245,18 +245,19 @@
         return;
     }
     const uint32_t wg = blockIdx.x - npro, nwg = gridDim.x - npro;
+    const uint32_t nbody = ncw + half;
     if constexpr (GU == 2) {
-        if (wg >= 2u * half) {
-            gu_waves<D, TWOWAY>(d, epoch, (wg - 2u * half) * Cfg::NW + (threadIdx.x >> 6), (nwg - 2u * half) * Cfg::NW, (int)(threadIdx.x & 63u));
+        if (wg >= nbody) {
+            gu_waves<D, TWOWAY>(d, epoch, (wg - nbody) * Cfg::NW + (threadIdx.x >> 6), (nwg - nbody) * Cfg::NW, (int)(threadIdx.x & 63u));
             return;
         }
     }
     if constexpr (GU == 3) {
-        if (wg >= 2u * half) {
-            const uint32_t t = wg - 2u * half, w = threadIdx.x >> 6;
+        if (wg >= nbody) {
+            const uint32_t t = wg - nbody, w = threadIdx.x >> 6;
             const int lane = (int)(threadIdx.x & 63u);
             if (t < npack) pack_face_body<D, true>(d, side, epoch, t * Cfg::NW + w, npack_blk, npack * Cfg::NW, lane);
-            else gu_waves<D, TWOWAY, true>(d, epoch, (t - npack) * Cfg::NW + w, (nwg - 2u * half - npack) * Cfg::NW, lane);
+            else gu_waves<D, TWOWAY, true>(d, epoch, (t - npack) * Cfg::NW + w, (nwg - nbody - npack) * Cfg::NW, lane);
             return;
         }
     }
@@ -276,31 +277,33 @@
     __shared__ ColliderMotion s_colm[TWOWAY ? 16 : 1];
 #define P2G_HANDOVER (GU != 0)
 #define P2G_GUESTS_INLAUNCH (GU == 3)
-#define P2G_NBLK half
-    if (wg >= half) {
+    if (wg >= ncw) {
         const int filter = 1;
 #define P2G_CPIC false
 #define P2G_TWOWAY false
 #define P2G_PCDF false
-#define P2G_BLK (wg - half)
+#define P2G_BLK (wg - ncw)
+#define P2G_NBLK half
 #include "p2g_body.inc"
 #undef P2G_CPIC
 #undef P2G_TWOWAY
 #undef P2G_PCDF
 #undef P2G_BLK
+#undef P2G_NBLK
     } else {
         const int filter = 2;
 #define P2G_CPIC true
 #define P2G_TWOWAY TWOWAY
 #define P2G_PCDF true
 #define P2G_BLK wg
+#define P2G_NBLK ncw
 #include "p2g_body.inc"
 #undef P2G_CPIC
 #undef P2G_TWOWAY
 #undef P2G_PCDF
 #undef P2G_BLK
-    }
 #undef P2G_NBLK
+    }
 #undef P2G_HANDOVER
 #undef P2G_GUESTS_INLAUNCH
 }
diff --git a/wgsparkl_amd/csrc/layout.h b/wgsparkl_amd/csrc/layout.h
--- a/wgsparkl_amd/csrc/layout.h
+++ b/wgsparkl_amd/csrc/layout.h
@@ -106,6 +106,7 @@
        CTR_NFREE = 11,
        CTR_NINSERT = 12,
        CTR_NTOMB = 13,
+       CTR_NP2G = 14,
        CTR_NPHYS_SEEN = 8,
        CTR_NVISIT = 64,
        CTR_NCPIC = 320,
@@ -219,6 +220,7 @@
     uint32_t dbg;
     float fluid_gamma;
     uint8_t *pmodel[2];
+    unsigned long long *chunk_c, *group_c;
 };
 
 enum DebugSwitch : uint32_t {
@@ -245,6 +247,7 @@
     DBG_CELL_INSERTION_SORT = 1u << 24,
     DBG_NO_DIRECT_RUNS = 1u << 25,
     DBG_PLAIN_P2G_FIRST = 1u << 26,
+    DBG_P2G_FULL_LIST = 1u << 27,
 };
 
 constexpr uint32_t or_of_distinct_bits(std::initializer_list<uint32_t> bits) {
@@ -259,7 +262,7 @@
     DBG_CDF_SUMM_NO_WAIT, DBG_NO_PCDF_WAVES, DBG_PCDF_WAVES_UNSIZED, DBG_NO_REBIN, DBG_NO_EVICTION, DBG_NO_CDF_SUMM,
     DBG_G2P_TWO_LAUNCHES, DBG_P2G_TWO_LAUNCHES, DBG_NO_G2P_DENSE, DBG_NO_P2G_SMALL_BUDGET, DBG_NO_UNIFORM, DBG_G2P_TWO_PASSES,
     DBG_GU_OWN_LAUNCH, DBG_BODIES_OWN_LAUNCH, DBG_REBIN_LAUNCH, DBG_SHARD_SPLIT_LAYERS, DBG_CELL_INSERTION_SORT,
-    DBG_NO_DIRECT_RUNS, DBG_PLAIN_P2G_FIRST});
+    DBG_NO_DIRECT_RUNS, DBG_PLAIN_P2G_FIRST, DBG_P2G_FULL_LIST});
 constexpr uint32_t WGS_ABLATION_SWITCHES = or_of_distinct_bits({
     DBG_ABLATE_G2P_BYTES_ONLY, DBG_ABLATE_P2G_NO_ACCUM, DBG_ABLATE_P2G_NO_LOADS, DBG_ABLATE_NO_BLOCK_CDF});
 static_assert(WGS_LAUNCH_SHAPE_SWITCHES != 0u && WGS_ABLATION_SWITCHES != 0u && (WGS_LAUNCH_SHAPE_SWITCHES & WGS_ABLATION_SWITCHES) == 0u,
diff --git a/wgsparkl_amd/csrc/p2g_body.inc b/wgsparkl_amd/csrc/p2g_body.inc
--- a/wgsparkl_amd/csrc/p2g_body.inc
+++ b/wgsparkl_amd/csrc/p2g_body.inc
@@ -15,7 +15,7 @@
 #pragma unroll
     for (int kk = 0; kk < (TILE + NT - 1) / NT; kk++) tmap[kk] = tid0 + kk * NT < TILE ? (int)g_slab_tile_map.t[tid0 + kk * NT] : 0;
     uint32_t pending = NONE;
-    const uint32_t B = min(d.counters[filter == 2 ? ctr_ncpic(P2G_BLK & 7u, epoch) : (uint32_t)CTR_NBLOCKS], d.cap);
+    const uint32_t B = min(d.counters[filter == 2 ? ctr_ncpic(P2G_BLK & 7u, epoch) : (uint32_t)CTR_NP2G], d.cap);
     for (uint32_t a = filter == 2 ? P2G_BLK >> 3 : P2G_BLK; a < B; a += filter == 2 ? P2G_NBLK >> 3 : P2G_NBLK) {
         int tid = tid0;
         asm volatile("" : "+v"(tid));
diff --git a/wgsparkl_amd/pipeline.py b/wgsparkl_amd/pipeline.py
--- a/wgsparkl_amd/pipeline.py
+++ b/wgsparkl_amd/pipeline.py
@@ -329,6 +329,16 @@
         _ffi.check(self.lib, self.lib.wgs_get_stats(self._h, C.byref(s)))
         return {k: int(getattr(s, k)) for k, _ in s._fields_}
 
+    def debug_p2g_list(self):
+        fn = self.lib.wgs_debug_p2g_list
+        u32p, size = C.POINTER(C.c_uint32), C.c_size_t
+        fn.restype, fn.argtypes = C.c_int32, [C.c_void_p, u32p, u32p, size, C.POINTER(size), C.POINTER(size)]
+        cap = self.stats()["grid_capacity"]
+        rec, act = np.zeros((cap, 4), np.uint32), np.zeros((cap, 2), np.uint32)
+        n, m = size(0), size(0)
+        _ffi.check(self.lib, fn(self._h, rec.ctypes.data_as(u32p), act.ctypes.data_as(u32p), cap, C.byref(n), C.byref(m)))
+        return rec[:n.value].copy(), act[:m.value].copy()
+
     def close(self):
         if getattr(self, "_h", None):
             self.lib.wgs_data_destroy(self._h)
```

Result: no change. 5.615 billion particle-steps/s, median of 2 (-0.6%).
